# megaease/easevoice-trainer

Hardware: AMD Instinct MI355X
Metric: audio-seconds/sec trained (s2) (higher is better)
Workload: dtype bf16; 1 GPU; s2 SoVITS generator+discriminator GAN step, batch=16/GPU, 4 s 32 kHz clips (T=200 frames), configs/s2.json, random-init weights; global_batch=16, parallelism=dp1, launch=hip-graph replay (3 graphs/step)

## Files before the change

### easevoice_trainer_amd/csrc/conv1d.hip

```cpp
#include "evt_common.h"
#include "../../include/evt.h"
#include "conv_p.h"
#include "wgrad_epi.h"

extern "C" int evt_grouped_supported(const evt_conv1d_params* c);
extern "C" int evt_grouped_fwd(const evt_conv1d_params* c, const void* x, const void* w_reg, const float* bias, void* y,
                               void* stream);
extern "C" int evt_grouped_bwd_data(const evt_conv1d_params* c, const void* dy, const void* y, const void* w_reg,
                                    void* dx, void* stream);
extern "C" int evt_grouped_bwd_weight(const evt_conv1d_params* c, const void* x, const void* dy, const void* y,
                                      float* dw, void* stream);

extern "C" int evt_small_kind(const evt_conv1d_params* c);
extern "C" int evt_cout1_fwd(const evt_conv1d_params* c, const void* x, const void* w_reg, const float* bias, void* y,
                             void* stream);
extern "C" int evt_cout1_bwd_weight(const evt_conv1d_params* c, const void* x, const void* dy, const void* y, float* dw,
                                    float* dbias, float* ws, long ws_floats, void* stream);
extern "C" int evt_cin1_bwd_weight(const evt_conv1d_params* c, const void* x, const void* dy, const void* y, float* dw,
                                   float* dbias, float* ws, long ws_floats, void* stream);
extern "C" int evt_cin1_fwd(const evt_conv1d_params* c, const void* x, const void* w_reg, const float* bias, void* y,
                            void* stream);
extern "C" int evt_cin1_bwd_data(const evt_conv1d_params* c, const void* dy, const void* y, const void* w_reg,
                                 const void* gate, const void* dx_add, void* dx, void* stream);
extern "C" int evt_cout1_bwd_data(const evt_conv1d_params* c, const void* dy, const void* y, const void* w_reg,
                                  const void* gate, const void* dx_add, void* dx, void* stream);

namespace {

using evt_conv::ConvP;

template <typename T> struct Frag;
template <> struct Frag<float> {
  static constexpr int EPL = 1, KS = 4;
  typedef float type;
  static __device__ __forceinline__ f32x4 mma(float a, float b, f32x4 c) {
    return __builtin_amdgcn_mfma_f32_16x16x4f32(a, b, c, 0, 0, 0);
  }
};
template <> struct Frag<h16_t> {
  static constexpr int EPL = 8, KS = 32;
  typedef h16x8 type;
  static __device__ __forceinline__ f32x4 mma(h16x8 a, h16x8 b, f32x4 c) {
    return EVT_MFMA_16x16x32(a, b, c, 0, 0, 0);
  }
};

template <typename T, int MODE>
__device__ __forceinline__ uint4 fuse16(uint4 v, uint4 va, float act_slope, float in_slope, int act_kind) {
  if (MODE == 0) return v;
  constexpr int V = 16 / sizeof(T);
  T* h = reinterpret_cast<T*>(&v);
  const T* a = reinterpret_cast<const T*>(&va);
#pragma unroll
  for (int i = 0; i < V; ++i) {
    float t = to_f<T>(h[i]);
    if (MODE == 1) t = t > 0.f ? t : t * in_slope;
    else if (MODE == 2) t = to_f<T>(a[i]) > 0.f ? t : t * act_slope;
    else if (MODE == 3) { const float y = to_f<T>(a[i]); t *= 1.f - y * y; }
    else { t *= dact_from_out(act_kind, to_f<T>(a[i]), act_slope); t = t > 0.f ? t : t * in_slope; }
    h[i] = from_f<T>(t);
  }
  return v;
}

__device__ __forceinline__ int fuse_mode(bool has_act, int act_kind, float in_slope) {
  if (!has_act) return in_slope == 1.f ? 0 : 1;
  if (in_slope != 1.f) return 4;
  return act_kind == EVT_ACT_LRELU ? 2 : (act_kind == EVT_ACT_TANH ? 3 : 0);
}

template <typename T>
__device__ __forceinline__ uint4 fuse_load16(uint4 v, bool has_act, uint4 va, int act_kind, float act_slope,
                                             float in_slope) {
  switch (fuse_mode(has_act, act_kind, in_slope)) {
    case 0: return v;
    case 1: return fuse16<T, 1>(v, va, act_slope, in_slope, act_kind);
    case 2: return fuse16<T, 2>(v, va, act_slope, in_slope, act_kind);
    case 3: return fuse16<T, 3>(v, va, act_slope, in_slope, act_kind);
    default: return fuse16<T, 4>(v, va, act_slope, in_slope, act_kind);
  }
}

template <typename T, int CK, int WPT, int TPR>
__device__ __forceinline__ void igemm_load_w(uint4 (&wr)[WPT], const T* wg, const ConvP& p, int ch, int tg, int TG,
                                             int wrow, int wsub) {
  constexpr int SZ = sizeof(T);
  const int t0 = tg * TG;
  const int ppr = min(TG, p.KHp - t0) * CK * SZ / 16;
  const T* src = wg + ((long)(wrow * p.nchunk + ch) * p.KHp + t0) * CK;
#pragma unroll
  for (int i = 0; i < WPT; ++i) {
    const int piece = wsub + i * TPR;
    wr[i] = piece < ppr ? *reinterpret_cast<const uint4*>(src + piece * (16 / SZ)) : make_uint4(0, 0, 0, 0);
  }
}

template <typename T, int CK, int WPT, int TPR>
__device__ __forceinline__ void igemm_store_w(const uint4 (&wr)[WPT], unsigned char* ws, const ConvP& p, int tg, int TG,
                                              int WROW, int wrow, int wsub) {
  constexpr int SZ = sizeof(T);
  const int ppr = min(TG, p.KHp - tg * TG) * CK * SZ / 16;
#pragma unroll
  for (int i = 0; i < WPT; ++i) {
    const int piece = wsub + i * TPR;
    if (piece < ppr) *reinterpret_cast<uint4*>(ws + wrow * WROW + piece * 16) = wr[i];
  }
}

template <typename T, int CK, int XPT, int I0, int XPR>
__device__ __forceinline__ void igemm_load_x(uint4 (&xr)[XPT], uint4 (&ar)[XPT], const T* xg, const T* ag,
                                             const ConvP& p, int ch, int R, int row0, int lane) {
  constexpr int SZ = sizeof(T), LPR = CK * SZ / 16;
#pragma unroll
  for (int i = 0; i < XPR; ++i) {
    const int idx = lane + i * 64;
    const int r = idx / LPR, part = idx - r * LPR;
    const int in_row = row0 + r;
    const bool ok = idx < R * LPR && in_row >= 0 && in_row < p.Lin;
    const long off = ok ? (long)in_row * p.Cin + ch * CK + part * (16 / SZ) : 0;
    xr[I0 + i] = ok ? *reinterpret_cast<const uint4*>(xg + off) : make_uint4(0, 0, 0, 0);
    ar[I0 + i] = (ok && ag) ? *reinterpret_cast<const uint4*>(ag + off) : make_uint4(0, 0, 0, 0);
  }
}

template <typename T, int CK, int XPT, int I0, int XPR, int MODE>
__device__ __forceinline__ void igemm_store_x_m(const uint4 (&xr)[XPT], const uint4 (&ar)[XPT], unsigned char* xs,
                                                const ConvP& p, int R, int row0, int lane, int XROW) {
  constexpr int SZ = sizeof(T), LPR = CK * SZ / 16;
#pragma unroll
  for (int i = 0; i < XPR; ++i) {
    const int idx = lane + i * 64;
    const int r = idx / LPR, part = idx - r * LPR;
    const int in_row = row0 + r;
    if (idx < R * LPR) {
      const bool ok = in_row >= 0 && in_row < p.Lin;
      uint4 v = fuse16<T, MODE>(xr[I0 + i], ar[I0 + i], p.xact_slope, p.in_slope, p.xact_kind);
      if (!ok) v = make_uint4(0, 0, 0, 0);
      *reinterpret_cast<uint4*>(xs + r * XROW + part * 16) = v;
    }
  }
}

template <typename T, int CK, int XPT, int I0, int XPR>
__device__ __forceinline__ void igemm_store_x(const uint4 (&xr)[XPT], const uint4 (&ar)[XPT], unsigned char* xs,
                                              int mode, const ConvP& p, int R, int row0, int lane, int XROW) {
  switch (mode) {
    case 0: igemm_store_x_m<T, CK, XPT, I0, XPR, 0>(xr, ar, xs, p, R, row0, lane, XROW); break;
    case 1: igemm_store_x_m<T, CK, XPT, I0, XPR, 1>(xr, ar, xs, p, R, row0, lane, XROW); break;
    case 2: igemm_store_x_m<T, CK, XPT, I0, XPR, 2>(xr, ar, xs, p, R, row0, lane, XROW); break;
    case 3: igemm_store_x_m<T, CK, XPT, I0, XPR, 3>(xr, ar, xs, p, R, row0, lane, XROW); break;
    default: igemm_store_x_m<T, CK, XPT, I0, XPR, 4>(xr, ar, xs, p, R, row0, lane, XROW); break;
  }
}

template <typename T, int CK, int MODE>
__device__ __forceinline__ void igemm_stage_x_sync_m(unsigned char* xs, const T* xg, const T* ag, const ConvP& p, int ch,
                                                     int R, int row0, int lane, int XROW, int first_idx) {
  constexpr int SZ = sizeof(T), LPR = CK * SZ / 16;
  for (int idx = first_idx + lane; idx < R * LPR; idx += 64) {
    const int r = idx / LPR, part = idx - r * LPR;
    const int in_row = row0 + r;
    uint4 v = make_uint4(0, 0, 0, 0);
    if (in_row >= 0 && in_row < p.Lin) {
      const long off = (long)in_row * p.Cin + ch * CK + part * (16 / SZ);
      v = *reinterpret_cast<const uint4*>(xg + off);
      uint4 va = make_uint4(0, 0, 0, 0);
      if (MODE >= 2) va = *reinterpret_cast<const uint4*>(ag + off);
      v = fuse16<T, MODE>(v, va, p.xact_slope, p.in_slope, p.xact_kind);
    }
    *reinterpret_cast<uint4*>(xs + r * XROW + part * 16) = v;
  }
}

template <typename T, int CK>
__device__ __forceinline__ void igemm_stage_x_sync(unsigned char* xs, const T* xg, const T* ag, int mode, const ConvP& p,
                                                   int ch, int R, int row0, int lane, int XROW, int first_idx) {
  switch (mode) {
    case 0: igemm_stage_x_sync_m<T, CK, 0>(xs, xg, ag, p, ch, R, row0, lane, XROW, first_idx); break;
// ... 879 lines not shown
  if (c->cin % 16 || c->cout % 16) return false;
  if (c->stride > 1 && c->dil != 1) return false;
  return true;
}

int valid(const evt_conv1d_params* c) {
  if (!c || c->nseq <= 0 || c->lin <= 0 || c->cin <= 0 || c->cout <= 0 || c->k <= 0 || c->stride <= 0 ||
      c->dil <= 0 || c->groups <= 0 || c->pad < 0)
    return EVT_EINVAL;
  if (c->dtype != EVT_DT_F32 && c->dtype != EVT_DT_HALF) return EVT_EINVAL;
  if (c->cin % c->groups || c->cout % c->groups) return EVT_EINVAL;
  if (c->transposed && (c->groups != 1 || c->dil != 1)) return EVT_ENOTSUP;
  if (evt_conv1d_lout(c) <= 0) return EVT_EINVAL;
  return EVT_OK;
}

}

extern "C" {

int32_t evt_conv1d_lout(const evt_conv1d_params* c) {
  if (!c->transposed) return (c->lin + 2 * c->pad - c->dil * (c->k - 1) - 1) / c->stride + 1;
  return (c->lin - 1) * c->stride - 2 * c->pad + c->dil * (c->k - 1) + 1;
}

int32_t evt_conv1d_wants_plain_dy(const evt_conv1d_params* c) {
  if (!c || valid(c) != EVT_OK) return 0;
  if (c->impl != EVT_IMPL_AUTO || c->dtype != EVT_DT_HALF || c->transposed || !igemm_ok(c)) return 0;
  if (c->out_act == EVT_ACT_NONE || c->in_slope != 1.f) return 0;
  ConvP p{};
  p.in_slope = 1.f;
  p.nseq = c->nseq;
  p.nchunk = c->cout / 32;
  int nphase = 1;
  if (c->stride == 1) p.Q = c->lin;
  else { nphase = c->stride; p.Q = (c->lin - 1 + c->pad) / c->stride + 1; }
  if (evt_conv::deep_eligible(p, c->dtype, c->cin, c->cout, nphase)) return 1;
  {
    evt_wlayout l; evt_conv1d_layout(c, &l);
    ConvP q = p;
    q.s_in = q.s_out = 1; q.off_out = 0; q.KHp = l.alt_kp; q.nchunk = l.alt_nchunk;
    if (c->stride == 1 && evt_conv::narrow_eligible(q, c->dtype, c->cin, c->cout, 1)) return 1;
  }
  WgP w{};
  w.nseq = c->nseq; w.KH = w.KHp = c->k; w.Q = w.LA = evt_conv1d_lout(c); w.CA = c->cout; w.CB = c->cin;
  w.s = c->stride; w.dil = c->dil; w.LB = c->lin;
  w.a_slope = w.b_slope = 1.f;
  return (evt_conv::wgrad_deep_eligible(w, c->dtype) || evt_conv::wgrad_halo_eligible(w, c->dtype)) ? 1 : 0;
}

int32_t evt_conv1d_wants_plain_x(const evt_conv1d_params* c) {
  if (!c || valid(c) != EVT_OK) return 0;
  if (c->impl != EVT_IMPL_AUTO || c->dtype != EVT_DT_HALF || c->in_slope == 1.f || !igemm_ok(c)) return 0;
  if (evt_grouped_supported(c) || evt_small_kind(c) != 0) return 0;
  evt_wlayout l; evt_conv1d_layout(c, &l);
  const int lout = evt_conv1d_lout(c);
  ConvP p{};
  p.in_slope = 1.f;
  p.nseq = c->nseq;
  int nphase = 1;
  if (!c->transposed) { p.nchunk = l.reg_nchunk; p.KHp = l.reg_kp; p.Q = lout; }
  else {
    p.nchunk = l.alt_nchunk; p.KHp = l.alt_kp;
    if (c->stride == 1) p.Q = lout;
    else { nphase = c->stride; p.Q = (lout - 1 + c->pad) / c->stride + 1; }
  }
  return evt_conv::deep_eligible(p, c->dtype, c->cout, c->cin, nphase) ? 1 : 0;
}

int evt_conv1d_layout(const evt_conv1d_params* c, evt_wlayout* o) {
  if (!c || !o) return EVT_EINVAL;
  const int d0 = c->transposed ? c->cin : c->cout;
  const int d1 = c->transposed ? c->cout : c->cin / c->groups;
  o->d0 = d0; o->d1 = d1; o->k = c->k; o->stride = c->stride;
  pick_ck(c->dtype, d1, c->k, 1, &o->reg_ck, &o->reg_nchunk, &o->reg_kp);
  o->reg_elems = (int64_t)d0 * o->reg_nchunk * o->reg_kp * o->reg_ck;
  if (c->stride == 1) {
    pick_ck(c->dtype, d0, c->k, 1, &o->alt_ck, &o->alt_nchunk, &o->alt_kp);
    o->alt_nphase = 1;
  } else {
    const int J = (c->k + c->stride - 1) / c->stride;
    pick_ck(c->dtype, d0, J, 1, &o->alt_ck, &o->alt_nchunk, &o->alt_kp);
    o->alt_nphase = c->stride;
  }
  o->alt_elems = (int64_t)o->alt_nphase * d1 * o->alt_nchunk * o->alt_kp * o->alt_ck;
  return EVT_OK;
}

int evt_conv1d_fwd(const evt_conv1d_params* c, const void* x, const void* w_reg, const void* w_alt,
                   const float* bias, const void* res, void* y, void* stream) {
  int rc = valid(c);
  if (rc) return rc;
  if (!x || !y) return EVT_EINVAL;
  hipStream_t st = (hipStream_t)stream;
  const bool use_igemm = c->impl != EVT_IMPL_NAIVE && igemm_ok(c);
  if (c->impl == EVT_IMPL_IGEMM && !use_igemm) return EVT_ENOTSUP;
  const int lout = evt_conv1d_lout(c);
  evt_wlayout l; evt_conv1d_layout(c, &l);
  if (w_reg && evt_conv::rows16_eligible(c, c->nseq * c->lin, c->cout, c->cin,
                                         res || c->in_slope != 1.f || c->out_act != EVT_ACT_NONE))
    return evt_conv::launch_rows16(x, w_reg, bias, y, c->nseq * c->lin, c->cout, c->cin, st);
  evt_set_last_tag("conv_naive_fwd");
  if (c->impl != EVT_IMPL_NAIVE && !res && evt_grouped_supported(c)) {
    if (!w_reg) return EVT_EINVAL;
    evt_set_last_tag("grouped_fwd");
    return evt_grouped_fwd(c, x, w_reg, bias, y, stream);
  }
  if (c->impl != EVT_IMPL_NAIVE && !res && evt_small_kind(c) == 1) {
    if (!w_reg) return EVT_EINVAL;
    return evt_cout1_fwd(c, x, w_reg, bias, y, stream);
  }
  if (c->impl != EVT_IMPL_NAIVE && !res && evt_small_kind(c) == 2) {
    if (!w_reg) return EVT_EINVAL;
    return evt_cin1_fwd(c, x, w_reg, bias, y, stream);
  }
  if (!use_igemm) {
    if (!w_reg) return EVT_EINVAL;
    NvP p = make_nvp(c);
    p.x = x; p.w = w_reg; p.bias = bias; p.res = res; p.y = y;
    const long total = (long)c->nseq * lout * c->cout;
    const int blocks = (int)((total + 255) / 256 > 65535 * 8 ? 65535 * 8 : (total + 255) / 256);
    if (c->dtype == EVT_DT_HALF) hipLaunchKernelGGL(conv_naive_fwd<h16_t>, dim3(blocks), dim3(256), 0, st, p);
    else hipLaunchKernelGGL(conv_naive_fwd<float>, dim3(blocks), dim3(256), 0, st, p);
    return evt_check_launch();
  }
  const void* w = c->transposed ? w_alt : w_reg;
  if (!w) return EVT_EINVAL;
  ConvP p{};
  p.x = x; p.xact = nullptr; p.w = w; p.bias = bias; p.res = res; p.gate = nullptr; p.y = y;
  p.nseq = c->nseq; p.Lin = c->lin; p.Lout = lout; p.Cin = c->cin; p.Cout = c->cout;
  p.in_slope = c->in_slope; p.xact_kind = 0; p.xact_slope = 1.f; p.out_act = c->out_act; p.out_slope = c->out_slope;
  p.gate_slope = 1.f;
  int nphase = 1;
  if (!c->transposed) {
    p.KHp = l.reg_kp; p.nchunk = l.reg_nchunk;
    p.s_in = c->stride; p.dil = c->dil; p.off_in = -c->pad;
    p.s_out = 1; p.off_out = 0; p.off_out_phase = 0; p.Q = lout; p.w_phase_stride = 0;
  } else {
    p.KHp = l.alt_kp; p.nchunk = l.alt_nchunk; p.dil = 1; p.s_in = 1;
    if (c->stride == 1) {
      p.off_in = c->pad - (c->k - 1); p.s_out = 1; p.off_out = 0; p.off_out_phase = 0; p.Q = lout;
      p.w_phase_stride = 0;
    } else {
      const int J = (c->k + c->stride - 1) / c->stride;
      nphase = c->stride;
      p.off_in = -(J - 1); p.s_out = c->stride; p.off_out = -c->pad; p.off_out_phase = 1;
      p.Q = (lout - 1 + c->pad) / c->stride + 1;
      p.w_phase_stride = (long)c->cout * l.alt_nchunk * l.alt_kp * l.alt_ck;
    }
  }
  return launch_igemm(c->dtype, p, c->cout, c->cin, nphase, st, c->impl == EVT_IMPL_AUTO);
}

int evt_conv1d_bwd_data(const evt_conv1d_params* c, const void* dy, const void* y, const void* w_reg,
                        const void* w_alt, const void* x, const void* dx_add, void* dx, void* stream) {
  int rc = valid(c);
  if (rc) return rc;
  if (!dy || !dx) return EVT_EINVAL;
  if (c->out_act != EVT_ACT_NONE && !y) return EVT_EINVAL;
  if (c->in_slope != 1.f && !x) return EVT_EINVAL;
  hipStream_t st = (hipStream_t)stream;
  const bool use_igemm = c->impl != EVT_IMPL_NAIVE && igemm_ok(c);
  if (c->impl == EVT_IMPL_IGEMM && !use_igemm) return EVT_ENOTSUP;
  const int lout = evt_conv1d_lout(c);
  evt_wlayout l; evt_conv1d_layout(c, &l);
  const void* ysv = c->out_act != EVT_ACT_NONE ? y : nullptr;
  const void* gate = c->in_slope != 1.f ? x : nullptr;
  if (w_alt && evt_conv::rows16_eligible(c, c->nseq * c->lin, c->cin, c->cout, ysv || gate || dx_add))
    return evt_conv::launch_rows16(dy, w_alt, nullptr, dx, c->nseq * c->lin, c->cin, c->cout, st);
  evt_set_last_tag("conv_naive_bwd_data");
  if (c->impl != EVT_IMPL_NAIVE && !gate && !dx_add && evt_grouped_supported(c)) {
    if (!w_reg) return EVT_EINVAL;
    evt_set_last_tag("grouped_bwd_data");
    return evt_grouped_bwd_data(c, dy, y, w_reg, dx, stream);
  }
  if (c->impl != EVT_IMPL_NAIVE && evt_small_kind(c) != 0) {
    if (!w_reg) return EVT_EINVAL;
    rc = evt_small_kind(c) == 1 ? evt_cout1_bwd_data(c, dy, y, w_reg, gate, dx_add, dx, stream)
                                : evt_cin1_bwd_data(c, dy, y, w_reg, gate, dx_add, dx, stream);
    if (rc != EVT_ENOTSUP) return rc;
  }
  if (!use_igemm) {
    if (!w_reg) return EVT_EINVAL;
    NvP p = make_nvp(c);
    p.x = dy; p.y_in = ysv; p.w = w_reg; p.gate = gate; p.res = dx_add; p.y = dx;
    const long total = (long)c->nseq * c->lin * c->cin;
    const int blocks = (int)((total + 255) / 256 > 65535 * 8 ? 65535 * 8 : (total + 255) / 256);
    if (c->dtype == EVT_DT_HALF) hipLaunchKernelGGL(conv_naive_bwd_data<h16_t>, dim3(blocks), dim3(256), 0, st, p);
    else hipLaunchKernelGGL(conv_naive_bwd_data<float>, dim3(blocks), dim3(256), 0, st, p);
    return evt_check_launch();
  }
  const void* w = c->transposed ? w_reg : w_alt;
  if (!w) return EVT_EINVAL;
  ConvP p{};
  p.x = dy; p.xact = ysv; p.w = w; p.bias = nullptr; p.res = dx_add; p.gate = gate; p.y = dx;
  p.nseq = c->nseq; p.Lin = lout; p.Lout = c->lin; p.Cin = c->cout; p.Cout = c->cin;
  p.in_slope = 1.f; p.xact_kind = c->out_act; p.xact_slope = c->out_slope; p.out_act = EVT_ACT_NONE;
  p.out_slope = 1.f; p.gate_slope = c->in_slope;
  int nphase = 1;
  if (!c->transposed) {
    p.KHp = l.alt_kp; p.nchunk = l.alt_nchunk;
    if (c->stride == 1) {
      p.s_in = 1; p.dil = c->dil; p.off_in = c->pad - (c->k - 1) * c->dil;
      p.s_out = 1; p.off_out = 0; p.off_out_phase = 0; p.Q = c->lin; p.w_phase_stride = 0;
    } else {
      const int J = (c->k + c->stride - 1) / c->stride;
      nphase = c->stride;
      p.s_in = 1; p.dil = 1; p.off_in = -(J - 1);
      p.s_out = c->stride; p.off_out = -c->pad; p.off_out_phase = 1;
      p.Q = (c->lin - 1 + c->pad) / c->stride + 1;
      p.w_phase_stride = (long)c->cin * l.alt_nchunk * l.alt_kp * l.alt_ck;
    }
  } else {
    p.KHp = l.reg_kp; p.nchunk = l.reg_nchunk;
    p.s_in = c->stride; p.dil = 1; p.off_in = -c->pad;
    p.s_out = 1; p.off_out = 0; p.off_out_phase = 0; p.Q = c->lin; p.w_phase_stride = 0;
  }
  return launch_igemm(c->dtype, p, c->cin, c->cout, nphase, st, c->impl == EVT_IMPL_AUTO);
}

int evt_conv1d_bwd_weight(const evt_conv1d_params* c, const void* x, const void* dy, const void* y, float* dw,
                          float* dbias, void* stream) {
  return evt_conv1d_bwd_weight_parts(c, x, dy, y, dw, dbias, nullptr, stream);
}

int evt_conv1d_bwd_weight_parts(const evt_conv1d_params* c, const void* x, const void* dy, const void* y, float* dw,
                                float* dbias, evt_wgrad_parts* sp, void* stream) {
  int rc = valid(c);
  if (rc) return rc;
  if (!x || !dy || !dw) return EVT_EINVAL;
  int used_host = 0;
  if (sp) {
    sp->used = 0;
    if (sp->parts < 1 || !sp->used_dev || sp->prev_used < 0 || sp->prev_used > sp->parts) return EVT_EINVAL;
    if (sp->parts > 1 && (!sp->dw_extra || sp->part_stride <= 0)) return EVT_EINVAL;
    if (sp->ws && sp->ws_floats <= 0) return EVT_EINVAL;
  }
  if (c->out_act != EVT_ACT_NONE && !y) return EVT_EINVAL;
  hipStream_t st = (hipStream_t)stream;
  const int lout = evt_conv1d_lout(c);
  const void* ysv = c->out_act != EVT_ACT_NONE ? y : nullptr;
  evt_wlayout l; evt_conv1d_layout(c, &l);
  const bool grouped = c->impl != EVT_IMPL_NAIVE && evt_grouped_supported(c);
  const bool igemm_path = !grouped && c->impl != EVT_IMPL_NAIVE && igemm_ok(c) && l.reg_kp <= 64;
  WgP p{};
  p.dw = dw; p.nseq = c->nseq; p.KH = c->k; p.KHp = l.reg_kp; p.s = c->stride; p.dil = c->dil; p.off = -c->pad;
  if (!c->transposed) {
    p.A = dy; p.Aact = ysv; p.aact_kind = c->out_act; p.aact_slope = c->out_slope; p.a_slope = 1.f;
    p.B = x; p.Bact = nullptr; p.bact_kind = 0; p.bact_slope = 1.f; p.b_slope = c->in_slope;
    p.LA = lout; p.CA = c->cout; p.LB = c->lin; p.CB = c->cin; p.Q = lout;
  } else {
    p.A = x; p.Aact = nullptr; p.aact_kind = 0; p.aact_slope = 1.f; p.a_slope = c->in_slope;
    p.B = dy; p.Bact = ysv; p.bact_kind = c->out_act; p.bact_slope = c->out_slope; p.b_slope = 1.f;
    p.LA = c->lin; p.CA = c->cin; p.LB = lout; p.CB = c->cout; p.Q = c->lin;
  }
  p.dbias = nullptr;
  if (sp) {
    p.dw_extra = sp->dw_extra; p.part_stride = sp->part_stride; p.parts = sp->parts; p.prev_used = sp->prev_used;
    p.db_part = sp->db_part; p.used = sp->used_dev; p.used_host = &used_host; p.dirty0 = sp->dirty0 || sp->prev_used > 0;
  }
  const bool gemm_w = igemm_path && c->impl == EVT_IMPL_AUTO && !c->transposed && evt_conv::wgrad_gemm_eligible(p, c->dtype);
  const bool halo_w = !gemm_w && igemm_path && c->impl == EVT_IMPL_AUTO && evt_conv::wgrad_halo_eligible(p, c->dtype);
  const bool deep_w = !gemm_w && !halo_w && igemm_path && c->impl == EVT_IMPL_AUTO && evt_conv::wgrad_deep_eligible(p, c->dtype);
  const bool ring_w = !deep_w && !halo_w && igemm_path && c->impl == EVT_IMPL_AUTO && evt_conv::wgrad_ring_eligible(p, c->dtype);
  const bool cin1 = !grouped && c->impl != EVT_IMPL_NAIVE && evt_small_kind(c) == 2;
  const bool cout1 = !grouped && c->impl != EVT_IMPL_NAIVE && evt_small_kind(c) == 1;
  const bool fuse_bias = dbias && ((igemm_path && c->dtype == EVT_DT_HALF && !c->transposed) || cin1 || cout1);
  float* ws = sp ? sp->ws : nullptr;
  const long ws_floats = sp ? (long)sp->ws_floats : 0;
  if (dbias && !fuse_bias) {
    const long rows = (long)c->nseq * lout;
    const int V = c->dtype == EVT_DT_HALF ? 8 : 4;
    int blocks;
    float* wsb = nullptr;
    if (c->cout % V == 0 && c->cout / V <= 256) {
      long rpb = (rows + 255) / 256;
      if (rpb < 16) rpb = 16;
      blocks = (int)((rows + rpb - 1) / rpb);
      if (ws && blocks >= 2 && (long)blocks * c->cout <= ws_floats) wsb = ws;
      if (c->dtype == EVT_DT_HALF)
        hipLaunchKernelGGL(colsum_act2<h16_t>, dim3(blocks), dim3(256), 0, st, (const h16_t*)dy, (const h16_t*)ysv,
                           dbias, rows, c->cout, c->out_act, c->out_slope, (int)rpb, wsb);
      else
        hipLaunchKernelGGL(colsum_act2<float>, dim3(blocks), dim3(256), 0, st, (const float*)dy, (const float*)ysv,
                           dbias, rows, c->cout, c->out_act, c->out_slope, (int)rpb, wsb);
    } else {
      const int rpb = 64;
      blocks = (int)((rows + rpb - 1) / rpb);
      if (ws && blocks >= 2 && (long)blocks * c->cout <= ws_floats) wsb = ws;
      if (c->dtype == EVT_DT_HALF)
        hipLaunchKernelGGL(colsum_act<h16_t>, dim3(blocks), dim3(256), 0, st, (const h16_t*)dy, (const h16_t*)ysv,
                           dbias, rows, c->cout, c->out_act, c->out_slope, rpb, wsb);
      else
        hipLaunchKernelGGL(colsum_act<float>, dim3(blocks), dim3(256), 0, st, (const float*)dy, (const float*)ysv,
                           dbias, rows, c->cout, c->out_act, c->out_slope, rpb, wsb);
    }
    rc = evt_check_launch();
    if (rc) return rc;
    if (wsb) {
      rc = evt_conv::launch_fold_partials(wsb, c->cout, blocks, dbias, c->cout, st);
      if (rc) return rc;
    }
  }
  evt_set_last_tag("conv_naive_bwd_weight");
  if (grouped) {
    evt_set_last_tag("grouped_bwd_weight");
    return evt_grouped_bwd_weight(c, x, dy, y, dw, stream);
  }
  if (cout1) return evt_cout1_bwd_weight(c, x, dy, y, dw, dbias, ws, ws_floats, stream);
  if (cin1) return evt_cin1_bwd_weight(c, x, dy, y, dw, dbias, ws, ws_floats, stream);
  const bool use_igemm = igemm_path;
  if (c->impl == EVT_IMPL_IGEMM && !use_igemm) return EVT_ENOTSUP;
  if (!use_igemm) {
    NvP p = make_nvp(c);
    p.x = x; p.res = dy; p.y_in = ysv; p.dw = dw;
    const int d1n = c->transposed ? c->cout : c->cin / c->groups;
    const int d0n = c->transposed ? c->cin : c->cout;
    const long elems = (long)d0n * d1n * c->k;
    const long pos = (long)c->nseq * (c->transposed ? c->lin : lout);
    long split = (4096 + elems - 1) / elems;
    const long maxsplit = (pos + 2047) / 2048;
    if (split > maxsplit) split = maxsplit;
    if (split < 1) split = 1;
    p.nsplit = (int)split;
    if (c->dtype == EVT_DT_HALF)
      hipLaunchKernelGGL(conv_naive_bwd_weight<h16_t>, dim3((unsigned)elems, p.nsplit), dim3(256), 0, st, p);
    else
      hipLaunchKernelGGL(conv_naive_bwd_weight<float>, dim3((unsigned)elems, p.nsplit), dim3(256), 0, st, p);
    return evt_check_launch();
  }
  if (gemm_w) {
    p.dbias = fuse_bias ? dbias : nullptr;
    p.parts = 0;
    return evt_conv::launch_wgrad_gemm(p, st);
  }
  if (halo_w || deep_w || ring_w) {
    p.dbias = fuse_bias ? dbias : nullptr;
    if (!p.dbias) p.db_part = nullptr;
    rc = halo_w ? evt_conv::launch_wgrad_halo(p, st) : (deep_w ? evt_conv::launch_wgrad_deep(p, st) : evt_conv::launch_wgrad_ring(p, st));
    if (sp) sp->used = used_host;
    return rc;
  }
  if (c->dtype == EVT_DT_HALF) {
    p.dbias = fuse_bias ? dbias : nullptr;
    p.ws = ws; p.ws_floats = ws_floats;
    if (p.parts < 2) p.parts = 0;
    rc = launch_wgrad_tr(p, st);
    if (sp && rc != EVT_ENOTSUP) sp->used = used_host;
    if (rc != EVT_ENOTSUP) return rc;
    p.parts = 0;
    if (fuse_bias) {
      const long rows = (long)c->nseq * lout;
      hipLaunchKernelGGL(colsum_act<h16_t>, dim3((int)((rows + 63) / 64)), dim3(256), 0, st, (const h16_t*)dy,
                         (const h16_t*)ysv, dbias, rows, c->cout, c->out_act, c->out_slope, 64, (float*)nullptr);
      rc = evt_check_launch();
      if (rc) return rc;
    }
  }
  p.dbias = nullptr;
  return launch_wgrad(c->dtype, p, st);
}

}
```

### easevoice_trainer_amd/csrc/conv_deep.hip

```cpp
#include "conv_p.h"
#include "wgrad_epi.h"

namespace evt_conv {
namespace {

__device__ __attribute__((aligned(256))) unsigned int g_zero_page[64];

typedef __attribute__((address_space(1))) const void* gptr_t;
typedef __attribute__((address_space(3))) void* lptr_t;

__device__ __forceinline__ void glds16(const void* g, void* l) {
  __builtin_amdgcn_global_load_lds((gptr_t)g, (lptr_t)l, 16, 0, 0);
}

constexpr int BM = 128, BN = 128, BK = 64;

template <int TM, int TN, int MI, int NJ>
__device__ __forceinline__ void store_tile_staged(const ConvP& p, unsigned char* smem, const f32x4 (&acc)[MI][NJ], int wr,
                                                  int wc, int n, int g, int yi, int pb, int phase, int total_units) {
  constexpr int PITCH = TM * 2 + 16;
  constexpr int CPR = TM / 8;
  constexpr int RPP = 256 / CPR;
  f32x4 bv[MI];
#pragma unroll
  for (int i = 0; i < MI; ++i)
    bv[i] = p.bias ? *reinterpret_cast<const f32x4*>(p.bias + yi * TM + wr * 16 * MI + i * 16 + g * 4) : f32x4{0.f, 0.f, 0.f, 0.f};
  asm volatile("s_waitcnt lgkmcnt(0)" ::: "memory");
  __builtin_amdgcn_s_barrier();
  asm volatile("" ::: "memory");
#pragma unroll
  for (int j = 0; j < NJ; ++j) {
    const int pl = wc * 16 * NJ + j * 16 + n;
#pragma unroll
    for (int i = 0; i < MI; ++i) {
      const int cl = wr * 16 * MI + i * 16 + g * 4;
      h16_t outv[4];
#pragma unroll
      for (int r = 0; r < 4; ++r) {
        float v = acc[i][j][r] + bv[i][r];
        if (p.out_act == EVT_ACT_LRELU) v = lrelu_f(v, p.out_slope);
        else if (p.out_act == EVT_ACT_TANH) v = tanhf(v);
        outv[r] = f2h(v);
      }
      *reinterpret_cast<uint2*>(smem + pl * PITCH + cl * 2) = *reinterpret_cast<uint2*>(outv);
    }
  }
  __syncthreads();
  h16_t* Y = reinterpret_cast<h16_t*>(p.y);
  const h16_t* R = reinterpret_cast<const h16_t*>(p.res);
  const h16_t* G = reinterpret_cast<const h16_t*>(p.gate);
  const int tid = threadIdx.x;
  const int c16 = tid % CPR, r0 = tid / CPR;
#pragma unroll
  for (int pass = 0; pass * RPP < TN; ++pass) {
    const int pl = pass * RPP + r0;
    const int u = pb * TN + pl;
    if (pl >= TN || u >= total_units) continue;
    const int seq = u / p.Q;
    const int q = u - seq * p.Q;
    const int orow = q * p.s_out + p.off_out + phase * p.off_out_phase;
    if (orow < 0 || orow >= p.Lout) continue;
    const long off = ((long)seq * p.Lout + orow) * p.Cout + yi * TM + c16 * 8;
    uint4 v = *reinterpret_cast<const uint4*>(smem + pl * PITCH + c16 * 16);
    if (G || R) {
      uint4 gv = make_uint4(0, 0, 0, 0), rv = make_uint4(0, 0, 0, 0);
      if (G) gv = *reinterpret_cast<const uint4*>(G + off);
      if (R) rv = *reinterpret_cast<const uint4*>(R + off);
      h16_t* vp = reinterpret_cast<h16_t*>(&v);
      const h16_t* gp = reinterpret_cast<const h16_t*>(&gv);
      const h16_t* rp = reinterpret_cast<const h16_t*>(&rv);
#pragma unroll
      for (int e = 0; e < 8; ++e) {
        float f = h2f(vp[e]);
        if (G) f *= (h2f(gp[e]) > 0.f ? 1.f : p.gate_slope);
        if (R) f += h2f(rp[e]);
        vp[e] = f2h(f);
      }
    }
    *reinterpret_cast<uint4*>(Y + off) = v;
  }
}


constexpr int STAGE_BYTES = (BM + BN) * BK * 2;

__global__ __launch_bounds__(256, 2) void conv_deep(ConvP p) {
  extern __shared__ __attribute__((aligned(1024))) unsigned char smem[];
  const int tid = threadIdx.x, lane = tid & 63;
  const int wave = __builtin_amdgcn_readfirstlane(tid >> 6);
  const int n = lane & 15, g = lane >> 4;
  const int wr = wave >> 1, wc = wave & 1;

  const int lin = blockIdx.x;
  const int xcd = lin & 7, slot = lin >> 3;
  const int yi = slot % p.Y;
  const int pb = xcd + 8 * (slot / p.Y);
  if (pb >= p.P) return;
  const int phase = blockIdx.y;

  const h16_t* X = reinterpret_cast<const h16_t*>(p.x);
  const h16_t* W = reinterpret_cast<const h16_t*>(p.w) + (long)phase * p.w_phase_stride;
  const int total_units = p.nseq * p.Q;

  const int rsub = lane >> 3, pslot = lane & 7;
  long aoff[4], boff[4];
  int brow[4];
#pragma unroll
  for (int i = 0; i < 4; ++i) {
    const int row = wave * 32 + i * 8 + rsub;
    const int c = pslot ^ (row & 7);
    const int co = yi * BM + row;
    aoff[i] = ((long)co * p.nchunk + (c >> 2)) * p.KHp * 32 + (c & 3) * 8;
    const int u = pb * BN + row;
    const bool ok = u < total_units;
    const int seq = ok ? u / p.Q : 0;
    const int q = ok ? u - seq * p.Q : 0;
    brow[i] = ok ? q * p.s_in + p.off_in : -(1 << 28);
    boff[i] = ((long)seq * p.Lin + brow[i]) * p.Cin + c * 8;
  }
  const h16_t* zsrc = reinterpret_cast<const h16_t*>(g_zero_page) + pslot * 8;
  unsigned char* my_a = smem + wave * 32 * 128;
  unsigned char* my_b = smem + BM * 128 + wave * 32 * 128;

  const int nch2 = p.nchunk >> 1;
  const int nst = nch2 * p.KHp;

  auto issue = [&](int st, int buf) {
    const int ch2 = st / p.KHp, tap = st - ch2 * p.KHp;
    const long wsoff = ((long)(2 * ch2) * p.KHp + tap) * 32;
    const int rshift = tap * p.dil;
    const long xsoff = (long)rshift * p.Cin + ch2 * 64;
#pragma unroll
    for (int i = 0; i < 4; ++i) glds16(W + aoff[i] + wsoff, my_a + buf * STAGE_BYTES + i * 1024);
#pragma unroll
    for (int i = 0; i < 4; ++i) {
      const bool ok = (unsigned)(brow[i] + rshift) < (unsigned)p.Lin;
      const h16_t* src = ok ? X + boff[i] + xsoff : zsrc;
      glds16(src, my_b + buf * STAGE_BYTES + i * 1024);
    }
  };

  f32x4 acc[4][4];
#pragma unroll
  for (int i = 0; i < 4; ++i)
#pragma unroll
    for (int j = 0; j < 4; ++j) acc[i][j] = f32x4{0.f, 0.f, 0.f, 0.f};

  const int sw = n & 7;
  const int a_base = (wr * 64 + n) * 128;
  const int b_base = BM * 128 + (wc * 64 + n) * 128;
  const int so0 = ((0 + g) ^ sw) * 16, so1 = ((4 + g) ^ sw) * 16;

  issue(0, 0);
  for (int st = 0; st < nst; ++st) {
    const int buf = st & 1;
    __syncthreads();
    if (st + 1 < nst) issue(st + 1, buf ^ 1);
    const unsigned char* sa = smem + buf * STAGE_BYTES + a_base;
    const unsigned char* sb = smem + buf * STAGE_BYTES + b_base;
#pragma unroll
    for (int ks = 0; ks < 2; ++ks) {
      const int so = ks ? so1 : so0;
      h16x8 a[4], b[4];
#pragma unroll
      for (int i = 0; i < 4; ++i) a[i] = *reinterpret_cast<const h16x8*>(sa + i * 16 * 128 + so);
#pragma unroll
      for (int j = 0; j < 4; ++j) b[j] = *reinterpret_cast<const h16x8*>(sb + j * 16 * 128 + so);
#pragma unroll
      for (int i = 0; i < 4; ++i)
#pragma unroll
        for (int j = 0; j < 4; ++j) acc[i][j] = EVT_MFMA_16x16x32(a[i], b[j], acc[i][j], 0, 0, 0);
    }
  }

  store_tile_staged<BM, BN, 4, 4>(p, smem, acc, wr, wc, n, g, yi, pb, phase, total_units);
}

constexpr int STAGE32 = (BM + BN) * 64;

__global__ __launch_bounds__(256, 4) void conv_deep32(ConvP p) {
  extern __shared__ __attribute__((aligned(1024))) unsigned char smem[];
  const int tid = threadIdx.x, lane = tid & 63;
  const int wave = __builtin_amdgcn_readfirstlane(tid >> 6);
  const int n = lane & 15, g = lane >> 4;
  const int wr = wave >> 1, wc = wave & 1;
  const int lin = blockIdx.x;
  const int xcd = lin & 7, slot = lin >> 3;
  const int yi = slot % p.Y;
  const int pb = xcd + 8 * (slot / p.Y);
  if (pb >= p.P) return;
  const int phase = blockIdx.y;
  const h16_t* X = reinterpret_cast<const h16_t*>(p.x);
  const h16_t* W = reinterpret_cast<const h16_t*>(p.w) + (long)phase * p.w_phase_stride;
  const int total_units = p.nseq * p.Q;

  const int rsub = lane >> 2, pslot = lane & 3;
  long aoff[2], boff[2];
  int brow[2];
#pragma unroll
  for (int i = 0; i < 2; ++i) {
    const int row = wave * 32 + i * 16 + rsub;
    const int c = pslot ^ (2 * ((row >> 3) & 1));
    aoff[i] = (long)(yi * BM + row) * p.nchunk * p.KHp * 32 + c * 8;
    const int u = pb * BN + row;
    const bool ok = u < total_units;
    const int seq = ok ? u / p.Q : 0;
    const int q = ok ? u - seq * p.Q : 0;
    brow[i] = ok ? q * p.s_in + p.off_in : -(1 << 28);
    boff[i] = ((long)seq * p.Lin + brow[i]) * p.Cin + c * 8;
  }
  const h16_t* zsrc = reinterpret_cast<const h16_t*>(g_zero_page) + pslot * 8;
  unsigned char* my_a = smem + wave * 32 * 64;
  unsigned char* my_b = smem + BM * 64 + wave * 32 * 64;
  const int nst = p.nchunk * p.KHp;

  auto issue = [&](int st, int buf) {
    const int ch = st / p.KHp, tap = st - ch * p.KHp;
    const long wsoff = ((long)ch * p.KHp + tap) * 32;
    const int rshift = tap * p.dil;
    const long xsoff = (long)rshift * p.Cin + ch * 32;
#pragma unroll
    for (int i = 0; i < 2; ++i) glds16(W + aoff[i] + wsoff, my_a + buf * STAGE32 + i * 1024);
#pragma unroll
    for (int i = 0; i < 2; ++i) {
      const bool ok = (unsigned)(brow[i] + rshift) < (unsigned)p.Lin;
      glds16(ok ? X + boff[i] + xsoff : zsrc, my_b + buf * STAGE32 + i * 1024);
    }
  };

// ... 1173 lines not shown
```

### easevoice_trainer_amd/csrc/conv_p.h

```cpp
#pragma once
#include "evt_common.h"
#include "../../include/evt.h"
#include <cstdlib>

namespace evt_conv {

struct ConvP {
  const void* x;
  const void* xact;
  const void* w;
  const float* bias;
  const void* res;
  const void* gate;
  void* y;
  int nseq, Lin, Lout, Cin, Cout;
  int KHp;
  int s_in, dil, off_in;
  int s_out, off_out, off_out_phase;
  int Q, U;
  int nchunk;
  long w_phase_stride;
  float in_slope;
  int xact_kind;
  float xact_slope;
  int out_act;
  float out_slope;
  float gate_slope;
  int P, Y;
};

struct WgP {
  const void* A;
  const void* Aact;
  const void* B;
  const void* Bact;
  float* dw;
  int nseq, LA, LB, CA, CB;
  int KH, KHp, s, dil, off, Q;
  int nchunk;
  float a_slope, b_slope;
  int aact_kind, bact_kind;
  float aact_slope, bact_slope;
  int nsplit;
  int ntapgrp;
  int xcd_order;
  float* dbias;
  float* dw_extra;
  long part_stride;
  int parts;
  int prev_used;
  int now_used;
  int dirty0;
  float* db_part;
  int* used;
  int* used_host;
  float* ws;
  long ws_floats;
};

bool deep_eligible(const ConvP& p, int dtype, int out_ch, int k_ch, int nphase);
int launch_conv_deep(const ConvP& p, int out_ch, int k_ch, int nphase, hipStream_t st);
bool narrow_eligible(const ConvP& p, int dtype, int out_ch, int k_ch, int nphase);
int launch_conv_narrow(const ConvP& p, int out_ch, int k_ch, int nphase, hipStream_t st);
bool wgrad_deep_eligible(const WgP& p, int dtype);
int launch_wgrad_deep(const WgP& p, hipStream_t st);
bool wgrad_gemm_eligible(const WgP& p, int dtype);
int launch_wgrad_gemm(const WgP& p, hipStream_t st);
bool wgrad_ring_eligible(const WgP& p, int dtype);
int launch_wgrad_ring(const WgP& p, hipStream_t st);
bool wgrad_halo_eligible(const WgP& p, int dtype);
int launch_wgrad_halo(const WgP& p, hipStream_t st);
int launch_fold_partials(const float* part, long stride, int nb, float* out, long n, hipStream_t st);
int launch_fold_partials2(const float* part, long stride, int nb, float* out, long n, float* out2, long n2, hipStream_t st);
void wgrad_pick_split(const WgP& p, long tiles, int nstages, long target, int min_stages, int* nsplit, int* per);

bool rows16_eligible(const struct evt_conv1d_params* c, int rows, int n_out, int k_red, bool fused);
int launch_rows16(const void* x, const void* w, const float* bias, void* y, int M, int N, int K, hipStream_t st);

}
```

### easevoice_trainer_amd/csrc/conv_small.hip

```cpp
#include "evt_common.h"
#include "../../include/evt.h"
#include "conv_p.h"

namespace {

struct SP {
  const void* x; const void* w; const float* bias; const void* y_in; const void* dy; void* y; float* dw;
  int nseq, lin, lout, cin, cout, k, stride, pad, dil;
  int ck, nchunk, kp;
  float in_slope; int out_act; float out_slope;
  int G;
  int pos_per_block;
  float* ws;
  long ws_row;
  float* dbias;
  int tile;
  int step_q, step_r;
};

__device__ __forceinline__ long sreg_index(const SP& p, int d0, int d1, int t) {
  const int chunk = d1 / p.ck, cc = d1 - chunk * p.ck;
  return (((long)d0 * p.nchunk + chunk) * p.kp + t) * p.ck + cc;
}

struct Walk { int seq, i; };
__device__ __forceinline__ Walk walk_at(long r, int len) {
  Walk w;
  w.seq = (int)(r / len);
  w.i = (int)(r - (long)w.seq * len);
  return w;
}
__device__ __forceinline__ void walk_add(Walk& w, int dq, int dr, int len) {
  w.seq += dq; w.i += dr;
  if (w.i >= len) { w.i -= len; ++w.seq; }
}

template <typename T> struct Raw8 { uint4 q[sizeof(T) / 2]; };
template <typename T> __device__ __forceinline__ Raw8<T> ld8(const T* s) {
  Raw8<T> r;
#pragma unroll
  for (int i = 0; i < (int)sizeof(T) / 2; ++i) r.q[i] = reinterpret_cast<const uint4*>(s)[i];
  return r;
}
template <typename T> __device__ __forceinline__ void cvt8(const Raw8<T>& r, float* f) {
  const T* pv = reinterpret_cast<const T*>(&r);
#pragma unroll
  for (int e = 0; e < 8; ++e) f[e] = to_f<T>(pv[e]);
}

template <typename T>
__global__ __launch_bounds__(256) void cout1_fwd(SP p) {
  constexpr int V = 16 / sizeof(T);
  extern __shared__ __attribute__((aligned(16))) unsigned char smem[];
  float* wl = reinterpret_cast<float*>(smem);
  const T* w = reinterpret_cast<const T*>(p.w);
  for (int i = threadIdx.x; i < p.k * p.cin; i += 256) {
    const int t = i / p.cin, c = i - t * p.cin;
    wl[i] = to_f<T>(w[sreg_index(p, 0, c, t)]);
  }
  __syncthreads();
  const int G = p.G;
  const int sub = threadIdx.x % G;
  const long gid = ((long)blockIdx.x * 256 + threadIdx.x) / G;
  const long ngroups = (long)gridDim.x * 256 / G;
  const long total = (long)p.nseq * p.lout;
  const int ppr = p.cin / V;
  const int pieces = p.k * ppr;
  const T* x = reinterpret_cast<const T*>(p.x);
  const long rounds = (total + ngroups - 1) / ngroups;
  for (long rd = 0; rd < rounds; ++rd) {
    const long o = rd * ngroups + gid;
    const bool live = o < total;
    const int q = live ? (int)(o % p.lout) : 0;
    const int seq = live ? (int)(o / p.lout) : 0;
    float acc = 0.f;
    if (live) {
      for (int pc = sub; pc < pieces; pc += G) {
        const int t = pc / ppr, c0 = (pc - t * ppr) * V;
        const int row = q * p.stride + t * p.dil - p.pad;
        if (row < 0 || row >= p.lin) continue;
        const uint4 v = *reinterpret_cast<const uint4*>(x + ((long)seq * p.lin + row) * p.cin + c0);
        const T* pv = reinterpret_cast<const T*>(&v);
        const float* wr = wl + t * p.cin + c0;
#pragma unroll
        for (int e = 0; e < V; ++e) acc += lrelu_f(to_f<T>(pv[e]), p.in_slope) * wr[e];
      }
    }
    for (int off = G >> 1; off > 0; off >>= 1) acc += __shfl_xor(acc, off, 64);
    if (live && sub == 0) {
      if (p.bias) acc += p.bias[0];
      if (p.out_act == EVT_ACT_LRELU) acc = lrelu_f(acc, p.out_slope);
      else if (p.out_act == EVT_ACT_TANH) acc = tanhf(acc);
      reinterpret_cast<T*>(p.y)[o] = from_f<T>(acc);
    }
  }
}

template <typename T>
__device__ __forceinline__ float cout1_dy_sum(const SP& p, long o0, long o1) {
  __shared__ float redb[4];
  const T* dy = reinterpret_cast<const T*>(p.dy);
  const T* ys = reinterpret_cast<const T*>(p.y_in);
  float s = 0.f;
  for (long o = o0 + threadIdx.x; o < o1; o += 256) {
    float d = to_f<T>(dy[o]);
    if (ys) d *= dact_from_out(p.out_act, to_f<T>(ys[o]), p.out_slope);
    s += d;
  }
  return block_reduce_sum_256(s, redb);
}

__device__ __forceinline__ void cout1_store_partial(const SP& p, const float* red, int npl, float bsum) {
  const int kc = p.k * p.cin;
  const int img = p.nchunk * p.kp * p.ck;
  for (int i = threadIdx.x; i < img; i += 256) {
    const int run = i / p.ck, cc = i - run * p.ck;
    const int chunk = run / p.kp, t = run - chunk * p.kp;
    const int c = chunk * p.ck + cc;
    const bool real = t < p.k && c < p.cin;
    float v = 0.f;
    if (real) {
      v = red[t * p.cin + c];
      for (int l = 1; l < npl; ++l) v += red[l * kc + t * p.cin + c];
    }
    if (p.ws) p.ws[(long)blockIdx.x * p.ws_row + i] = v;
    else if (real) atomicAdd(p.dw + i, v);
  }
  if (threadIdx.x == 0 && p.dbias) {
    if (p.ws) p.ws[(long)blockIdx.x * p.ws_row + img] = bsum;
    else atomicAdd(p.dbias, bsum);
  }
}

template <typename T>
__global__ __launch_bounds__(256) void cout1_bwd_weight(SP p) {
  constexpr int V = 16 / sizeof(T);
  extern __shared__ __attribute__((aligned(16))) unsigned char smem[];
  float* red = reinterpret_cast<float*>(smem);
  const int ppr = p.cin / V;
  const int pieces = p.k * ppr;
  int pp = 1;
  while (pp < pieces && pp < 256) pp <<= 1;
  const int npl = 256 / pp;
  const int pl = threadIdx.x / pp, pc0 = threadIdx.x % pp;
  constexpr int NA = 4;
  float acc[NA][V];
#pragma unroll
  for (int a = 0; a < NA; ++a)
#pragma unroll
    for (int e = 0; e < V; ++e) acc[a][e] = 0.f;
  const T* x = reinterpret_cast<const T*>(p.x);
  const T* dy = reinterpret_cast<const T*>(p.dy);
  const T* ys = reinterpret_cast<const T*>(p.y_in);
  const long total = (long)p.nseq * p.lout;
  const long p0 = (long)blockIdx.x * p.pos_per_block;
  const long p1 = min(total, p0 + p.pos_per_block);
  constexpr int UP = 4;
  for (long ob = p0 + pl; ob < p1; ob += (long)npl * UP) {
    uint4 v[UP][NA];
    float d[UP];
#pragma unroll
    for (int u = 0; u < UP; ++u) {
      const long o = ob + (long)u * npl;
      const bool live = o < p1;
      const int q = live ? (int)(o % p.lout) : 0, seq = live ? (int)(o / p.lout) : 0;
      d[u] = live ? to_f<T>(dy[o]) : 0.f;
      if (live && ys) d[u] *= dact_from_out(p.out_act, to_f<T>(ys[o]), p.out_slope);
#pragma unroll
      for (int a = 0; a < NA; ++a) {
        const int pc = pc0 + a * pp;
// ... 162 lines not shown
        }
      }
    }
  }
  __syncthreads();
  T* dx = reinterpret_cast<T*>(p.y) + (long)seq * p.lin;
  const T* gt = gate ? reinterpret_cast<const T*>(gate) + (long)seq * p.lin : nullptr;
  const T* ad = dx_add ? reinterpret_cast<const T*>(dx_add) + (long)seq * p.lin : nullptr;
  for (int ii = threadIdx.x; ii < ni; ii += 256) {
    const int i = i0 + ii;
    float acc = 0.f;
    for (int t = 0; t < p.k; ++t) {
      const int j = i + p.pad - t * p.dil;
      if (j < 0) break;
      const int q = j / p.stride;
      if (q * p.stride != j || q > qhi || q < qlo) continue;
      const float* pr = pl + (long)(q - qlo) * CG * p.k + t;
      float s = pr[0];
      for (int g = 1; g < CG; ++g) s += pr[g * p.k];
      acc += s;
    }
    if (gt) acc *= (to_f<T>(gt[i]) > 0.f ? 1.f : p.in_slope);
    if (ad) acc += to_f<T>(ad[i]);
    dx[i] = from_f<T>(acc);
  }
}

constexpr int C1_TQ = 256;

template <typename T, int KM>
__global__ __launch_bounds__(256) void cin1_bwd_weight(SP p, float* dbias) {
  extern __shared__ __attribute__((aligned(16))) unsigned char smem[];
  float* xl = reinterpret_cast<float*>(smem);
  __shared__ float red[4][4][(KM + 1) * 8];
  const int CG = p.cout >> 3, ppp = 256 / CG;
  const int cg = threadIdx.x & (CG - 1), c0 = cg * 8, ql = threadIdx.x / CG;
  const int lane = threadIdx.x & 63, wave = threadIdx.x >> 6;
  const int tiles = (p.lout + C1_TQ - 1) / C1_TQ;
  const long ntiles = (long)p.nseq * tiles;
  constexpr int UP = KM <= 8 ? 4 : 2;
  for (int t0 = 0; t0 < p.k; t0 += KM) {
    float acc[KM][8], bacc[8];
#pragma unroll
    for (int e = 0; e < 8; ++e) {
      bacc[e] = 0.f;
#pragma unroll
      for (int t = 0; t < KM; ++t) acc[t][e] = 0.f;
    }
    Walk wk = walk_at(blockIdx.x, tiles);
    for (long tile = blockIdx.x; tile < ntiles; tile += gridDim.x) {
      const int q0 = wk.i * C1_TQ;
      const int nq = min(C1_TQ, p.lout - q0);
      const int seg = (nq - 1) * p.stride + (p.k - 1) * p.dil + 1;
      const int r0 = q0 * p.stride - p.pad;
      const T* x = reinterpret_cast<const T*>(p.x) + (long)wk.seq * p.lin;
      const T* dy = reinterpret_cast<const T*>(p.dy) + ((long)wk.seq * p.lout + q0) * p.cout + c0;
      const T* ys = p.y_in ? reinterpret_cast<const T*>(p.y_in) + ((long)wk.seq * p.lout + q0) * p.cout + c0 : nullptr;
      __syncthreads();
      for (int i = threadIdx.x; i < seg; i += 256) {
        const int r = r0 + i;
        xl[i] = (r >= 0 && r < p.lin) ? lrelu_f(to_f<T>(x[r]), p.in_slope) : 0.f;
      }
      __syncthreads();
      for (int qb = ql; qb < nq; qb += ppp * UP) {
        Raw8<T> v[UP], va[UP];
#pragma unroll
        for (int u = 0; u < UP; ++u) {
          const int q = qb + u * ppp;
          if (q < nq) {
            v[u] = ld8<T>(dy + (long)q * p.cout);
            if (ys) va[u] = ld8<T>(ys + (long)q * p.cout);
          }
        }
#pragma unroll
        for (int u = 0; u < UP; ++u) {
          const int q = qb + u * ppp;
          if (q < nq) {
            float d[8], a[8];
            cvt8<T>(v[u], d);
            if (ys) {
              cvt8<T>(va[u], a);
#pragma unroll
              for (int e = 0; e < 8; ++e) d[e] *= dact_from_out(p.out_act, a[e], p.out_slope);
            }
            if (t0 == 0) {
#pragma unroll
              for (int e = 0; e < 8; ++e) bacc[e] += d[e];
            }
            const float* xr = xl + q * p.stride + t0 * p.dil;
#pragma unroll
            for (int t = 0; t < KM; ++t) {
              if (t0 + t < p.k) {
                const float xv = xr[t * p.dil];
#pragma unroll
                for (int e = 0; e < 8; ++e) acc[t][e] += d[e] * xv;
              }
            }
          }
        }
      }
      walk_add(wk, p.step_q, p.step_r, tiles);
    }
    for (int off = CG; off < 64; off <<= 1) {
#pragma unroll
      for (int e = 0; e < 8; ++e) {
        bacc[e] += __shfl_xor(bacc[e], off, 64);
#pragma unroll
        for (int t = 0; t < KM; ++t) acc[t][e] += __shfl_xor(acc[t][e], off, 64);
      }
    }
    __syncthreads();
    if (lane < CG) {
#pragma unroll
      for (int e = 0; e < 8; ++e) {
        red[wave][cg][KM * 8 + e] = bacc[e];
#pragma unroll
        for (int t = 0; t < KM; ++t) red[wave][cg][t * 8 + e] = acc[t][e];
      }
    }
    __syncthreads();
    for (int i = threadIdx.x; i < (KM + 1) * p.cout; i += 256) {
      const int t = i / p.cout, co = i - t * p.cout;
      const int g = co >> 3, e = co & 7;
      const float v = ((red[0][g][t * 8 + e] + red[1][g][t * 8 + e]) + red[2][g][t * 8 + e]) + red[3][g][t * 8 + e];
      if (t < KM) {
        if (t0 + t < p.k) {
          const long idx = (long)co * p.kp + t0 + t;
          if (p.ws) p.ws[(long)blockIdx.x * p.ws_row + idx] = v;
          else atomicAdd(p.dw + idx, v);
        }
      } else if (t0 == 0) {
        if (p.ws) p.ws[(long)blockIdx.x * p.ws_row + (p.ws_row - p.cout) + co] = v;
        else if (dbias) atomicAdd(dbias + co, v);
      }
    }
  }
}

template <typename T>
__global__ __launch_bounds__(256) void cout1_bwd_data(SP p, const void* gate, const void* dx_add) {
  constexpr int V = 16 / sizeof(T);
  extern __shared__ __attribute__((aligned(16))) unsigned char smem[];
  float* wl = reinterpret_cast<float*>(smem);
  const T* w = reinterpret_cast<const T*>(p.w);
  for (int i = threadIdx.x; i < p.k * p.cin; i += 256) {
    const int t = i / p.cin, c = i - t * p.cin;
    wl[i] = to_f<T>(w[sreg_index(p, 0, c, t)]);
  }
  __syncthreads();
  const int ppr = p.cin / V;
  const long total = (long)p.nseq * p.lin * ppr;
  const T* dy = reinterpret_cast<const T*>(p.dy);
  const T* ys = reinterpret_cast<const T*>(p.y_in);
  for (long idx = (long)blockIdx.x * 256 + threadIdx.x; idx < total; idx += (long)gridDim.x * 256) {
    const long row = idx / ppr;
    const int c0 = (int)(idx - row * ppr) * V;
    const int seq = (int)(row / p.lin), i = (int)(row - (long)seq * p.lin);
    float acc[V];
#pragma unroll
    for (int e = 0; e < V; ++e) acc[e] = 0.f;
    for (int t = 0; t < p.k; ++t) {
      const int j = i + p.pad - t * p.dil;
      if (j < 0) break;
      const int q = j / p.stride;
      if (q * p.stride != j || q >= p.lout) continue;
      const long o = (long)seq * p.lout + q;
      float d = to_f<T>(dy[o]);
      if (ys) d *= dact_from_out(p.out_act, to_f<T>(ys[o]), p.out_slope);
      const float* wr = wl + t * p.cin + c0;
#pragma unroll
      for (int e = 0; e < V; ++e) acc[e] += d * wr[e];
    }
    const long off = row * p.cin + c0;
    T outv[V];
    uint4 gv = make_uint4(0, 0, 0, 0), av = make_uint4(0, 0, 0, 0);
    if (gate) gv = *reinterpret_cast<const uint4*>(reinterpret_cast<const T*>(gate) + off);
    if (dx_add) av = *reinterpret_cast<const uint4*>(reinterpret_cast<const T*>(dx_add) + off);
    const T* pg = reinterpret_cast<const T*>(&gv);
    const T* pa = reinterpret_cast<const T*>(&av);
#pragma unroll
    for (int e = 0; e < V; ++e) {
      float v = acc[e];
      if (gate) v *= (to_f<T>(pg[e]) > 0.f ? 1.f : p.in_slope);
      if (dx_add) v += to_f<T>(pa[e]);
      outv[e] = from_f<T>(v);
    }
    *reinterpret_cast<uint4*>(reinterpret_cast<T*>(p.y) + off) = *reinterpret_cast<uint4*>(outv);
  }
}

SP make_sp(const evt_conv1d_params* c) {
  SP p{};
  p.nseq = c->nseq; p.lin = c->lin; p.lout = evt_conv1d_lout(c); p.cin = c->cin; p.cout = c->cout; p.k = c->k;
  p.stride = c->stride; p.pad = c->pad; p.dil = c->dil; p.in_slope = c->in_slope; p.out_act = c->out_act;
  p.out_slope = c->out_slope;
  evt_wlayout l; evt_conv1d_layout(c, &l);
  p.ck = l.reg_ck; p.nchunk = l.reg_nchunk; p.kp = l.reg_kp;
  return p;
}

inline void set_step(SP& p, long step, int len) {
  p.step_q = (int)(step / len);
  p.step_r = (int)(step - (long)p.step_q * len);
}

constexpr int CI1_WG_BLOCKS = 512;

template <typename T, int K>
__global__ __launch_bounds__(256) void cout1_bwd_weight_xs(SP p, int rows_per_block) {
  constexpr int V = 16 / sizeof(T);
  extern __shared__ __attribute__((aligned(16))) unsigned char smem[];
  float* red = reinterpret_cast<float*>(smem);
  const int ppr = p.cin / V;
  int pp = 1;
  while (pp < ppr) pp <<= 1;
  const int npl = 256 / pp;
  const int rl = threadIdx.x / pp, pc = threadIdx.x % pp;
  float acc[K][V];
#pragma unroll
  for (int t = 0; t < K; ++t)
#pragma unroll
    for (int e = 0; e < V; ++e) acc[t][e] = 0.f;
  const T* x = reinterpret_cast<const T*>(p.x);
  const T* dy = reinterpret_cast<const T*>(p.dy);
  const T* ys = reinterpret_cast<const T*>(p.y_in);
  const long total = (long)p.nseq * p.lin;
  const long r0 = (long)blockIdx.x * rows_per_block;
  const long r1 = min(total, r0 + rows_per_block);
  constexpr int UP = 4;
  if (pc < ppr) {
    for (long rb = r0 + rl; rb < r1; rb += (long)npl * UP) {
      uint4 v[UP];
      float d[UP][K];
#pragma unroll
      for (int u = 0; u < UP; ++u) {
        const long r = rb + (long)u * npl;
        const bool live = r < r1;
        const long seq = live ? r / p.lin : 0;
        const int i = live ? (int)(r - seq * p.lin) : 0;
        v[u] = live ? *reinterpret_cast<const uint4*>(x + r * p.cin + pc * V) : make_uint4(0, 0, 0, 0);
#pragma unroll
        for (int t = 0; t < K; ++t) {
          const int q = i + p.pad - t;
          const bool ok = live && q >= 0 && q < p.lout;
          const long o = seq * p.lout + (ok ? q : 0);
          float dv = ok ? to_f<T>(dy[o]) : 0.f;
          if (ok && ys) dv *= dact_from_out(p.out_act, to_f<T>(ys[o]), p.out_slope);
          d[u][t] = dv;
        }
      }
#pragma unroll
      for (int u = 0; u < UP; ++u) {
        const T* pv = reinterpret_cast<const T*>(&v[u]);
#pragma unroll
        for (int e = 0; e < V; ++e) {
          const float xv = lrelu_f(to_f<T>(pv[e]), p.in_slope);
#pragma unroll
          for (int t = 0; t < K; ++t) acc[t][e] += d[u][t] * xv;
        }
      }
    }
  }
  const int kc = K * p.cin;
  if (pc < ppr) {
#pragma unroll
    for (int t = 0; t < K; ++t)
#pragma unroll
      for (int e = 0; e < V; ++e) red[rl * kc + t * p.cin + pc * V + e] = acc[t][e];
  }
  const long nout = (long)p.nseq * p.lout;
  const long o0 = min(nout, (long)blockIdx.x * p.pos_per_block);
  const float bsum = p.dbias ? cout1_dy_sum<T>(p, o0, min(nout, o0 + p.pos_per_block)) : 0.f;
  __syncthreads();
  cout1_store_partial(p, red, npl, bsum);
}

}

extern "C" int evt_small_kind(const evt_conv1d_params* c) {
  if (c->transposed || c->groups != 1) return 0;
  const int V = c->dtype == EVT_DT_HALF ? 8 : 4;
  if (c->cout == 1 && c->cin % V == 0 && (long)c->k * c->cin <= 4096) return 1;
  if (c->cin == 1 && c->cout % 8 == 0 && c->cout <= 32 && 256 % c->cout == 0 && c->cout * (c->k + 1) <= 256)
    return 2;
  return 0;
}

extern "C" int evt_cout1_fwd(const evt_conv1d_params* c, const void* x, const void* w_reg, const float* bias, void* y,
                             void* stream) {
  SP p = make_sp(c);
  p.x = x; p.w = w_reg; p.bias = bias; p.y = y;
  const int V = c->dtype == EVT_DT_HALF ? 8 : 4;
  const int pieces = c->k * (c->cin / V);
  int G = 1;
  while (G < pieces && G < 64) G <<= 1;
  p.G = G;
  const long total = (long)p.nseq * p.lout;
  long blocks = (total * G + 255) / 256;
  constexpr long cap = 4096;
  if (blocks > cap) blocks = cap;
  const size_t lds = (size_t)c->k * c->cin * sizeof(float);
  hipStream_t st = (hipStream_t)stream;
  evt_set_last_tag("cout1_fwd");
  if (c->dtype == EVT_DT_HALF) hipLaunchKernelGGL(cout1_fwd<h16_t>, dim3((int)blocks), dim3(256), lds, st, p);
  else hipLaunchKernelGGL(cout1_fwd<float>, dim3((int)blocks), dim3(256), lds, st, p);
  return evt_check_launch();
}

extern "C" int evt_cout1_bwd_weight(const evt_conv1d_params* c, const void* x, const void* dy, const void* y, float* dw,
                                    float* dbias, float* ws, long ws_floats, void* stream) {
  SP p = make_sp(c);
  p.x = x; p.dy = dy; p.y_in = c->out_act != EVT_ACT_NONE ? y : nullptr; p.dw = dw; p.dbias = dbias;
  const long total = (long)p.nseq * p.lout;
  long ppb = (total + 255) / 256;
  if (ppb < 16) ppb = 16;
  const long img = (long)p.nchunk * p.kp * p.ck;
  const long row = img + 1;
  if (ws && row * 2 <= ws_floats) {
    constexpr long tgt = 1024, minp = 16;
    ppb = (total + tgt - 1) / tgt;
    if (ppb < minp) ppb = minp;
    const long maxb = ws_floats / row;
    if ((total + ppb - 1) / ppb > maxb) ppb = (total + maxb - 1) / maxb;
    p.ws = ws; p.ws_row = row;
  }
  p.pos_per_block = (int)ppb;
  int blocks = (int)((total + ppb - 1) / ppb);
  const int V = c->dtype == EVT_DT_HALF ? 8 : 4;
  hipStream_t st = (hipStream_t)stream;
  int ppr2 = 1;
  while (ppr2 < c->cin / V) ppr2 <<= 1;
  const size_t lds_xs = (size_t)(256 / ppr2) * c->k * c->cin * sizeof(float);
  if (p.stride == 1 && p.dil == 1 && (c->k == 3 || c->k == 7) && ppr2 <= 256 && lds_xs <= (60u << 10)) {
    const long rows = (long)p.nseq * p.lin;
    long rpb = (rows + blocks - 1) / blocks;
    if (rpb < 16) rpb = 16;
    blocks = (int)((rows + rpb - 1) / rpb);
    p.pos_per_block = (int)((total + blocks - 1) / blocks);
    evt_set_last_tag("cout1_bwd_weight_xs<k%d>", c->k);
#define XS(T, K_) hipLaunchKernelGGL((cout1_bwd_weight_xs<T, K_>), dim3(blocks), dim3(256), lds_xs, st, p, (int)rpb)
    if (c->dtype == EVT_DT_HALF) { if (c->k == 3) XS(h16_t, 3); else XS(h16_t, 7); }
    else { if (c->k == 3) XS(float, 3); else XS(float, 7); }
#undef XS
  } else {
    int pp = 1;
    while (pp < c->k * (c->cin / V) && pp < 256) pp <<= 1;
    const size_t lds = (size_t)(256 / pp) * c->k * c->cin * sizeof(float);
    evt_set_last_tag("cout1_bwd_weight");
    if (c->dtype == EVT_DT_HALF) hipLaunchKernelGGL(cout1_bwd_weight<h16_t>, dim3(blocks), dim3(256), lds, st, p);
    else hipLaunchKernelGGL(cout1_bwd_weight<float>, dim3(blocks), dim3(256), lds, st, p);
  }
  int rc = evt_check_launch();
  if (rc || !p.ws) return rc;
  return evt_conv::launch_fold_partials2(p.ws, row, blocks, dw, img, dbias, dbias ? 1 : 0, st);
}

extern "C" int evt_cin1_bwd_weight(const evt_conv1d_params* c, const void* x, const void* dy, const void* y, float* dw,
                                   float* dbias, float* ws, long ws_floats, void* stream) {
  if (c->cout != 8 && c->cout != 16 && c->cout != 32) return EVT_ENOTSUP;
  SP p = make_sp(c);
  p.x = x; p.dy = dy; p.y_in = c->out_act != EVT_ACT_NONE ? y : nullptr; p.dw = dw;
  const int tiles = (p.lout + C1_TQ - 1) / C1_TQ;
  const long ntiles = (long)p.nseq * tiles;
  const long img = (long)p.cout * p.nchunk * p.kp * p.ck;
  const long row = img + p.cout;
  int blocks = (int)(ntiles < 256 ? ntiles : 256);
  if (ws && ntiles >= 2 && row * 2 <= ws_floats) {
    const long maxb = ws_floats / row < CI1_WG_BLOCKS ? ws_floats / row : CI1_WG_BLOCKS;
    blocks = (int)(ntiles < maxb ? ntiles : maxb);
    p.ws = ws; p.ws_row = row;
  }
  set_step(p, blocks, tiles);
  const int seg = (C1_TQ - 1) * c->stride + (c->k - 1) * c->dil + 1;
  const size_t lds = (size_t)seg * sizeof(float);
  hipStream_t st = (hipStream_t)stream;
  evt_set_last_tag("cin1_bwd_weight");
#define WG(T) do { if (c->k <= 8) hipLaunchKernelGGL((cin1_bwd_weight<T, 8>), dim3(blocks), dim3(256), lds, st, p, dbias); \
                   else hipLaunchKernelGGL((cin1_bwd_weight<T, 16>), dim3(blocks), dim3(256), lds, st, p, dbias); } while (0)
  if (c->dtype == EVT_DT_HALF) WG(h16_t); else WG(float);
#undef WG
  int rc = evt_check_launch();
  if (rc || !p.ws) return rc;
  return evt_conv::launch_fold_partials2(p.ws, row, blocks, dw, img, dbias, dbias ? p.cout : 0, st);
}

extern "C" int evt_cin1_fwd(const evt_conv1d_params* c, const void* x, const void* w_reg, const float* bias, void* y,
                            void* stream) {
  SP p = make_sp(c);
  p.x = x; p.w = w_reg; p.bias = bias; p.y = y;
  const int blocks = p.nseq * ((p.lout + C1_TP - 1) / C1_TP);
  const int seg = (C1_TP - 1) * c->stride + (c->k - 1) * c->dil + 1;
  const size_t lds = ((size_t)c->k * c->cout + seg) * sizeof(float);
  hipStream_t st = (hipStream_t)stream;
  evt_set_last_tag("cin1_fwd");
  if (c->dtype == EVT_DT_HALF) hipLaunchKernelGGL(cin1_fwd<h16_t>, dim3(blocks), dim3(256), lds, st, p);
  else hipLaunchKernelGGL(cin1_fwd<float>, dim3(blocks), dim3(256), lds, st, p);
  return evt_check_launch();
}

extern "C" int evt_cin1_bwd_data(const evt_conv1d_params* c, const void* dy, const void* y, const void* w_reg,
                                 const void* gate, const void* dx_add, void* dx, void* stream) {
  if (c->cout != 8 && c->cout != 16 && c->cout != 32) return EVT_ENOTSUP;
  SP p = make_sp(c);
  p.dy = dy; p.y_in = c->out_act != EVT_ACT_NONE ? y : nullptr; p.w = w_reg; p.y = dx;
  const int CG = c->cout >> 3;
  int TI = C1_TI;
  size_t lds;
  for (;; TI >>= 1) {
    const int rows = (TI + (c->k - 1) * c->dil) / c->stride + 2;
    lds = ((size_t)c->k * c->cout + (size_t)rows * CG * c->k) * sizeof(float);
    if (lds <= 48 * 1024 || TI <= 32) break;
  }
  if (lds > 64 * 1024) return EVT_ENOTSUP;
  p.tile = TI;
  const int blocks = p.nseq * ((p.lin + TI - 1) / TI);
  hipStream_t st = (hipStream_t)stream;
  evt_set_last_tag("cin1_bwd_data");
#define BWD(T) do { if (c->k <= 8) hipLaunchKernelGGL((cin1_bwd_data<T, 8>), dim3(blocks), dim3(256), lds, st, p, gate, dx_add); \
                    else hipLaunchKernelGGL((cin1_bwd_data<T, 16>), dim3(blocks), dim3(256), lds, st, p, gate, dx_add); } while (0)
  if (c->dtype == EVT_DT_HALF) BWD(h16_t); else BWD(float);
#undef BWD
  return evt_check_launch();
}

extern "C" int evt_cout1_bwd_data(const evt_conv1d_params* c, const void* dy, const void* y, const void* w_reg,
                                  const void* gate, const void* dx_add, void* dx, void* stream) {
  SP p = make_sp(c);
  p.dy = dy; p.y_in = c->out_act != EVT_ACT_NONE ? y : nullptr; p.w = w_reg; p.y = dx;
  const int V = c->dtype == EVT_DT_HALF ? 8 : 4;
  const long total = (long)p.nseq * p.lin * (p.cin / V);
  long blocks = (total + 255) / 256;
  if (blocks > 2048) blocks = 2048;
  const size_t lds = (size_t)c->k * c->cin * sizeof(float);
  hipStream_t st = (hipStream_t)stream;
  evt_set_last_tag("cout1_bwd_data");
  if (c->dtype == EVT_DT_HALF) hipLaunchKernelGGL(cout1_bwd_data<h16_t>, dim3((int)blocks), dim3(256), lds, st, p, gate, dx_add);
  else hipLaunchKernelGGL(cout1_bwd_data<float>, dim3((int)blocks), dim3(256), lds, st, p, gate, dx_add);
  return evt_check_launch();
}
```

### easevoice_trainer_amd/csrc/elementwise.hip

```cpp
#include "evt_common.h"
#include "../../include/evt.h"

namespace {

__device__ __forceinline__ void store_w(void* base, long idx, float w, int dtype) {
  if (dtype == EVT_DT_HALF) reinterpret_cast<h16_t*>(base)[idx] = f2h(w);
  else reinterpret_cast<float*>(base)[idx] = w;
}

__device__ __forceinline__ long reg_idx(const evt_wlayout& L, int d0, int d1, int kk) {
  const int chunk = d1 / L.reg_ck, cc = d1 - chunk * L.reg_ck;
  return (((long)d0 * L.reg_nchunk + chunk) * L.reg_kp + kk) * L.reg_ck + cc;
}

__device__ __forceinline__ long alt_idx(const evt_wlayout& L, int d0, int d1, int kk) {
  const int chunk = d0 / L.alt_ck, cc = d0 - chunk * L.alt_ck;
  if (L.stride == 1) {
    const int t = L.k - 1 - kk;
    return (((long)d1 * L.alt_nchunk + chunk) * L.alt_kp + t) * L.alt_ck + cc;
  }
  const int J = (L.k + L.stride - 1) / L.stride;
  const int ph = kk % L.stride, j = kk / L.stride;
  const int jp = J - 1 - j;
  return ((((long)ph * L.d1 + d1) * L.alt_nchunk + chunk) * L.alt_kp + jp) * L.alt_ck + cc;
// ... 184 lines not shown
      const int row_floats = L.reg_nchunk * L.reg_kp * L.reg_ck;
      const long ro = (long)d0 * row_floats;
      fold_slabs_row(const_cast<float*>(it.dw) + ro, it.dw_extra + ro, it.dw_part_stride, nu, row_floats);
    }
    if (nb > 0 && it.db_part && it.db && threadIdx.x == 0) {
      float s = 0.f;
      for (int k = 0; k < nb; ++k) s += it.db_part[(long)k * L.d0 + d0];
      it.db[d0] += s;
    }
  }
  if (!it.g) {
    for (int e = threadIdx.x; e < n; e += 256) {
      const int d1 = e / L.k, kk = e - d1 * L.k;
      dv[e] += it.dw[reg_idx(L, d0, d1, kk)];
    }
    return;
  }
  float ss = 0.f, dot = 0.f;
  for (int e = threadIdx.x; e < n; e += 256) {
    const int d1 = e / L.k, kk = e - d1 * L.k;
    const float x = v[e];
    ss += x * x;
    dot += x * it.dw[reg_idx(L, d0, d1, kk)];
  }
  ss = block_reduce_sum_256(ss, red);
  dot = block_reduce_sum_256(dot, red);
  const float norm = sqrtf(ss);
  const float gval = it.g[d0];
  if (threadIdx.x == 0) it.dg[d0] += dot / norm;
  const float s1 = gval / norm, s2 = dot / ss;
  for (int e = threadIdx.x; e < n; e += 256) {
    const int d1 = e / L.k, kk = e - d1 * L.k;
    dv[e] += s1 * (it.dw[reg_idx(L, d0, d1, kk)] - v[e] * s2);
  }
}

template <typename T>
__global__ void add3_scale_kernel(const T* a, const T* b, const T* c, float scale, T* out, long n) {
  for (long i = blockIdx.x * (long)blockDim.x + threadIdx.x; i < n; i += (long)gridDim.x * blockDim.x) {
    float v = to_f<T>(a[i]);
    if (b) v += to_f<T>(b[i]);
    if (c) v += to_f<T>(c[i]);
    out[i] = from_f<T>(v * scale);
  }
}

template <typename T>
__global__ void dact_mul_kernel(const T* dy, const T* y, int kind, float slope, T* out, long n) {
  constexpr int V = 16 / sizeof(T);
  const long nv = n / V;
  for (long i = blockIdx.x * (long)blockDim.x + threadIdx.x; i < nv; i += (long)gridDim.x * blockDim.x) {
    uint4 d = reinterpret_cast<const uint4*>(dy)[i];
    const uint4 a = reinterpret_cast<const uint4*>(y)[i];
    T* dh = reinterpret_cast<T*>(&d);
    const T* ah = reinterpret_cast<const T*>(&a);
#pragma unroll
    for (int e = 0; e < V; ++e) dh[e] = from_f<T>(to_f<T>(dh[e]) * dact_from_out(kind, to_f<T>(ah[e]), slope));
    reinterpret_cast<uint4*>(out)[i] = d;
  }
  if (blockIdx.x == 0 && threadIdx.x < n - nv * V) {
    const long i = nv * V + threadIdx.x;
    out[i] = from_f<T>(to_f<T>(dy[i]) * dact_from_out(kind, to_f<T>(y[i]), slope));
  }
}

template <typename T>
__global__ void lrelu_kernel(const T* x, float slope, T* out, long n) {
  constexpr int V = 16 / sizeof(T);
  const long nv = n / V;
  for (long i = blockIdx.x * (long)blockDim.x + threadIdx.x; i < nv; i += (long)gridDim.x * blockDim.x) {
    uint4 v = reinterpret_cast<const uint4*>(x)[i];
    T* h = reinterpret_cast<T*>(&v);
#pragma unroll
    for (int e = 0; e < V; ++e) h[e] = from_f<T>(lrelu_f(to_f<T>(h[e]), slope));
    reinterpret_cast<uint4*>(out)[i] = v;
  }
  if (blockIdx.x == 0 && threadIdx.x < n - nv * V) {
    const long i = nv * V + threadIdx.x;
    out[i] = from_f<T>(lrelu_f(to_f<T>(x[i]), slope));
  }
}

__device__ __forceinline__ float sigmoid_f(float x) { return 1.f / (1.f + __expf(-x)); }

template <typename T>
__global__ void gated_fwd_kernel(const T* xin, const T* g, T* acts, int nseq, int len, int H) {
  const long total = (long)nseq * len * H;
  for (long i = blockIdx.x * (long)blockDim.x + threadIdx.x; i < total; i += (long)gridDim.x * blockDim.x) {
    const int h = (int)(i % H);
    const long nt = i / H;
    const int s = (int)(nt / len);
    float a = to_f<T>(xin[nt * 2 * H + h]), b = to_f<T>(xin[nt * 2 * H + H + h]);
    if (g) { a += to_f<T>(g[(long)s * 2 * H + h]); b += to_f<T>(g[(long)s * 2 * H + H + h]); }
    acts[i] = from_f<T>(tanhf(a) * sigmoid_f(b));
  }
}

template <typename T>
__global__ void gated_bwd_kernel(const T* xin, const T* g, const T* dacts, T* dxin, float* dg, int nseq, int len,
                                 int H) {
  const long total = (long)nseq * len * H;
  for (long i = blockIdx.x * (long)blockDim.x + threadIdx.x; i < total; i += (long)gridDim.x * blockDim.x) {
    const int h = (int)(i % H);
    const long nt = i / H;
    const int s = (int)(nt / len);
    float a = to_f<T>(xin[nt * 2 * H + h]), b = to_f<T>(xin[nt * 2 * H + H + h]);
    if (g) { a += to_f<T>(g[(long)s * 2 * H + h]); b += to_f<T>(g[(long)s * 2 * H + H + h]); }
    const float t = tanhf(a), sg = sigmoid_f(b), d = to_f<T>(dacts[i]);
    const float da = d * sg * (1.f - t * t), db = d * t * sg * (1.f - sg);
    dxin[nt * 2 * H + h] = from_f<T>(da);
    dxin[nt * 2 * H + H + h] = from_f<T>(db);
    if (dg) { atomicAdd(dg + (long)s * 2 * H + h, da); atomicAdd(dg + (long)s * 2 * H + H + h, db); }
  }
}

template <typename T>
__global__ __launch_bounds__(256) void gated_bwd_dg_kernel(const T* xin, const T* g, const T* dacts, T* dxin, float* dg,
                                                           int nseq, int len, int H, int tch) {
  const int per_seq = (len + tch - 1) / tch;
  const int s = blockIdx.x / per_seq;
  const int t0 = (blockIdx.x - s * per_seq) * tch, t1 = min(len, t0 + tch);
  for (int h = threadIdx.x; h < H; h += 256) {
    const float ga = to_f<T>(g[(long)s * 2 * H + h]), gb = to_f<T>(g[(long)s * 2 * H + H + h]);
    float sa = 0.f, sb = 0.f;
    for (int t = t0; t < t1; ++t) {
      const long nt = (long)s * len + t;
      const float a = to_f<T>(xin[nt * 2 * H + h]) + ga, b = to_f<T>(xin[nt * 2 * H + H + h]) + gb;
      const float th = tanhf(a), sg = sigmoid_f(b), d = to_f<T>(dacts[nt * H + h]);
      const float da = d * sg * (1.f - th * th), db = d * th * sg * (1.f - sg);
      dxin[nt * 2 * H + h] = from_f<T>(da);
      dxin[nt * 2 * H + H + h] = from_f<T>(db);
      sa += da;
      sb += db;
    }
    atomicAdd(dg + (long)s * 2 * H + h, sa);
    atomicAdd(dg + (long)s * 2 * H + H + h, sb);
  }
}

constexpr int SEG_MAX = 64;

template <typename T, int MODE>
__device__ __forceinline__ float seg_term(float a, float b, float target) {
  if (MODE == 0) return fabsf(a - b);
  const float d = target - a;
  return d * d;
}
template <typename T, int MODE>
__device__ __forceinline__ float seg_grad(float a, float b, float target, float dl) {
  if (MODE == 0) { const float d = a - b; return d > 0.f ? dl : (d < 0.f ? -dl : 0.f); }
  return -2.f * (target - a) * dl;
}

template <typename T, int MODE, bool BWD>
__global__ __launch_bounds__(256) void seg_flat_kernel(const evt_seg* segs, int nseg, float target, float* out,
                                                       const float* dloss) {
  constexpr int V = 16 / sizeof(T);
  __shared__ float red[4];
  __shared__ long pre[SEG_MAX + 1];
  if (threadIdx.x == 0) {
    long acc = 0;
    for (int i = 0; i < nseg; ++i) { pre[i] = acc; acc += segs[i].n; }
    pre[nseg] = acc;
  }
  __syncthreads();
  const long total = pre[nseg];
  long chunk = (total + gridDim.x - 1) / gridDim.x;
  chunk = (chunk + 2047) / 2048 * 2048;
  const long lo = (long)blockIdx.x * chunk, hi = min(total, lo + chunk);
  float acc = 0.f;
  for (int si = 0; si < nseg; ++si) {
    const long s0 = pre[si], s1 = pre[si + 1];
    if (s1 <= lo || s0 >= hi) continue;
    const evt_seg s = segs[si];
    if (BWD && !s.da) continue;
    const T* a = reinterpret_cast<const T*>(s.a);
    const T* b = reinterpret_cast<const T*>(s.b);
    T* da = reinterpret_cast<T*>(s.da);
    const long i0 = max(lo, s0) - s0, i1 = min(hi, s1) - s0;
    const float dl = BWD ? dloss[0] * s.scale : 0.f;
    float part = 0.f;
    const long v0 = min(i1, (i0 + V - 1) / V * V), v1 = v0 + (i1 - v0) / V * V;
    const bool vec_ok = ((((uintptr_t)a) | (MODE == 0 ? (uintptr_t)b : 0) | (BWD ? (uintptr_t)da : 0)) & 15) == 0;
    if (vec_ok) {
      for (long i = i0 + threadIdx.x; i < v0; i += 256) {
        const float av = to_f<T>(a[i]), bv = MODE == 0 ? to_f<T>(b[i]) : 0.f;
        if (BWD) da[i] = from_f<T>(seg_grad<T, MODE>(av, bv, target, dl)); else part += seg_term<T, MODE>(av, bv, target);
      }
      for (long i = v0 + (long)threadIdx.x * V; i < v1; i += 256L * V) {
        const uint4 va = *reinterpret_cast<const uint4*>(a + i);
        uint4 vb = make_uint4(0, 0, 0, 0);
        if (MODE == 0) vb = *reinterpret_cast<const uint4*>(b + i);
        const T* pa = reinterpret_cast<const T*>(&va);
        const T* pb = reinterpret_cast<const T*>(&vb);
        uint4 vo;
        T* po = reinterpret_cast<T*>(&vo);
#pragma unroll
        for (int e = 0; e < V; ++e) {
          const float av = to_f<T>(pa[e]), bv = MODE == 0 ? to_f<T>(pb[e]) : 0.f;
          if (BWD) po[e] = from_f<T>(seg_grad<T, MODE>(av, bv, target, dl)); else part += seg_term<T, MODE>(av, bv, target);
        }
        if (BWD) *reinterpret_cast<uint4*>(da + i) = vo;
      }
      for (long i = v1 + threadIdx.x; i < i1; i += 256) {
        const float av = to_f<T>(a[i]), bv = MODE == 0 ? to_f<T>(b[i]) : 0.f;
        if (BWD) da[i] = from_f<T>(seg_grad<T, MODE>(av, bv, target, dl)); else part += seg_term<T, MODE>(av, bv, target);
      }
    } else {
      for (long i = i0 + threadIdx.x; i < i1; i += 256) {
        const float av = to_f<T>(a[i]), bv = MODE == 0 ? to_f<T>(b[i]) : 0.f;
        if (BWD) da[i] = from_f<T>(seg_grad<T, MODE>(av, bv, target, dl)); else part += seg_term<T, MODE>(av, bv, target);
      }
    }
    acc += part * s.scale;
  }
  if (!BWD) {
    acc = block_reduce_sum_256(acc, red);
    if (threadIdx.x == 0 && acc != 0.f) atomicAdd(out, acc);
  }
}

__global__ void adamw_flat_kernel(float* p, const float* g, float* m, float* v, const evt_adamw_seg* segs, int nseg,
                                  float b1, float b2, float eps, float bc1, float bc2_sqrt, float gscale,
                                  long lo, long hi) {
  for (long i = lo + blockIdx.x * (long)blockDim.x + threadIdx.x; i < hi; i += (long)gridDim.x * blockDim.x) {
    int si = -1;
    for (int s = 0; s < nseg; ++s)
      if (i >= segs[s].begin && i < segs[s].end) { si = s; break; }
    if (si < 0) continue;
    const float lr = segs[si].lr, wd = segs[si].weight_decay;
    const float gr = g[i] * gscale;
    float pv = p[i];
    pv *= 1.f - lr * wd;
    const float mv = b1 * m[i] + (1.f - b1) * gr;
    const float vv = b2 * v[i] + (1.f - b2) * gr * gr;
    m[i] = mv; v[i] = vv;
    const float denom = sqrtf(vv) / bc2_sqrt + eps;
    pv -= (lr / bc1) * (mv / denom);
    p[i] = pv;
  }
}

__global__ void counter_inc_kernel(int* c, const float* skip) {
  if (skip && *skip != 0.f) return;
  *c += 1;
}

__global__ void adamw_flat_dev_kernel(float* p, const float* g, float* m, float* v, const evt_adamw_seg* segs, int nseg,
                                      float b1, float b2, float eps, const int* stepp, float gscale, long lo, long hi,
                                      const float* skip) {
  if (skip && *skip != 0.f) return;
  const float stepf = (float)*stepp;
  const float bc1 = 1.f - powf(b1, stepf);
  const float bc2_sqrt = sqrtf(1.f - powf(b2, stepf));
  for (long i = lo + blockIdx.x * (long)blockDim.x + threadIdx.x; i < hi; i += (long)gridDim.x * blockDim.x) {
    int si = -1;
    for (int s = 0; s < nseg; ++s)
      if (i >= segs[s].begin && i < segs[s].end) { si = s; break; }
    if (si < 0) continue;
    const float lr = segs[si].lr, wd = segs[si].weight_decay;
    const float gr = g[i] * gscale;
    float pv = p[i];
    pv *= 1.f - lr * wd;
    const float mv = b1 * m[i] + (1.f - b1) * gr;
    const float vv = b2 * v[i] + (1.f - b2) * gr * gr;
    m[i] = mv; v[i] = vv;
    const float denom = sqrtf(vv) / bc2_sqrt + eps;
    pv -= (lr / bc1) * (mv / denom);
    p[i] = pv;
  }
}

__global__ __launch_bounds__(256) void unscale_check_kernel(float* g, long n, const float* scale, float* found) {
  const float inv = (float)(1.0 / (double)*scale);
  bool bad = false;
  const long n4 = n >> 2;
  float4* g4 = reinterpret_cast<float4*>(g);
  for (long i = blockIdx.x * 256L + threadIdx.x; i < n4; i += (long)gridDim.x * 256) {
    float4 v = g4[i];
    bad |= !(isfinite(v.x) && isfinite(v.y) && isfinite(v.z) && isfinite(v.w));
    v.x *= inv; v.y *= inv; v.z *= inv; v.w *= inv;
    g4[i] = v;
  }
  for (long i = (n4 << 2) + blockIdx.x * 256L + threadIdx.x; i < n; i += (long)gridDim.x * 256) {
    const float v = g[i];
    bad |= !isfinite(v);
    g[i] = v * inv;
  }
  if (bad) *found = 1.f;
}

struct ScalerFlags { float* f[4]; };
__global__ void scaler_update_kernel(float* scale, int* tracker, ScalerFlags fl, int nflags, float growth, float backoff,
                                     int interval) {
  bool found = false;
  for (int i = 0; i < nflags; ++i) {
    found |= *fl.f[i] != 0.f;
    *fl.f[i] = 0.f;
  }
  if (found) {
    *scale = *scale * backoff;
    *tracker = 0;
  } else {
    const int ok = *tracker + 1;
    if (ok == interval) {
      const float ns = *scale * growth;
      if (isfinite(ns)) *scale = ns;
      *tracker = 0;
    } else {
      *tracker = ok;
    }
  }
}

__global__ __launch_bounds__(256) void sumsq_kernel(const float* x, long n, float* out) {
  __shared__ float red[4];
  float acc = 0.f;
  for (long i = blockIdx.x * 256L + threadIdx.x; i < n; i += (long)gridDim.x * 256) acc += x[i] * x[i];
  acc = block_reduce_sum_256(acc, red);
  if (threadIdx.x == 0) atomicAdd(out, acc);
}

inline int grid_for(long n, int cap = 8192) {
  long b = (n + 255) / 256;
  if (b > cap) b = cap;
  if (b < 1) b = 1;
  return (int)b;
}

}

#include <stdarg.h>
#include <stdio.h>
static bool g_tags_on = false;
static thread_local char g_last_tag[128] = "";
extern "C" void evt_set_last_tag(const char* fmt, ...) {
  if (!g_tags_on) return;
  va_list ap;
  va_start(ap, fmt);
  vsnprintf(g_last_tag, sizeof(g_last_tag), fmt, ap);
  va_end(ap);
}

extern "C" {

const char* evt_last_kernel_tag(void) { return g_last_tag; }
void evt_debug_kernel_tags(int32_t enable) { g_tags_on = enable != 0; }

#ifndef EVT_SRC_HASH
#define EVT_SRC_HASH "unknown"
#endif
const char* evt_version(void) { return "evt-hip 0.3 (gfx950, half = " EVT_HALF_NAME ") src=" EVT_SRC_HASH; }
int32_t evt_half_dtype(void) { return EVT_DT_HALF; }

int evt_wn_fold_multi(const evt_wprep_item* items, const int32_t* row_index, int32_t nrows, void* stream) {
  if (!items || !row_index || nrows <= 0) return EVT_EINVAL;
  const int nblocks = ((nrows + 255) / 256) * 256;
  hipLaunchKernelGGL(wn_fold_kernel, dim3(nblocks), dim3(256), 0, (hipStream_t)stream, items, row_index, nrows);
  return evt_check_launch();
}

int evt_wn_fold_groups(const evt_wprep_item* items, const int32_t* group_index, int32_t ngroups, void* stream) {
  if (!items || !group_index || ngroups <= 0) return EVT_EINVAL;
  const int nblocks = ((ngroups + 31) / 32) * 32;
// ... 208 lines not shown
```

### easevoice_trainer_amd/hip/conv.py

```python
import ctypes as C
import os
import math

import torch
from torch import nn

from . import lib as L


class ConvSlot:

    __slots__ = ("module", "layout", "reg", "alt", "dw", "bank", "_pcache", "packed_member", "parts", "dw_extra",
                 "db_part", "used", "wg_used", "wg_dirty", "_wgp")

    def __init__(self, module, layout, bank):
        self.module, self.layout, self.bank = module, layout, bank
        self.reg = self.alt = self.dw = None
        self._pcache = {}
        self.packed_member = False
        self.parts, self.dw_extra, self.db_part, self.used, self.wg_used, self._wgp = 1, None, None, None, 0, None
        self.wg_dirty = False

    def params(self, nseq, lin, in_slope, out_act, out_slope):
        key = (nseq, lin, in_slope, out_act, out_slope, self.bank.impl)
# ... 355 lines not shown

class FrozenConv:
    weight_norm, kdims, transposed, groups, dil = False, 1, False, 1, 1

    def __init__(self, weight_fn, bias_fn, cin, cout, k=1, stride=1, padding=0):
        self.weight_fn, self.bias_fn = weight_fn, bias_fn
        self.cin, self.cout, self.k, self.stride, self.pad = cin, cout, k, stride, padding
        self._slot = None

    @property
    def v(self):
        w = self.weight_fn()
        return w if w.dim() == 3 else w.unsqueeze(-1)

    @property
    def bias(self):
        return self.bias_fn() if self.bias_fn is not None else None

    def lout(self, lin):
        return (lin + 2 * self.pad - (self.k - 1) - 1) // self.stride + 1


class FrozenBank:
    weight_grads = False

    def __init__(self, convs, device, impl=L.IMPL_AUTO):
        self.dt, self.dtype, self.device, self.impl = L.DT_F32, torch.float32, torch.device(device), impl
        self.slots, offs, reg_n, alt_n = [], [], 0, 0
        for m in convs:
            lay = conv_layout(self.dt, m.cin, m.cout, m.k, m.stride, m.pad, m.dil, m.groups, m.transposed)
            s = ConvSlot(m, lay, self)
            m._slot = s
            self.slots.append(s)
            offs.append((reg_n, alt_n))
            reg_n += (lay.reg_elems + 127) // 128 * 128
            alt_n += (lay.alt_elems + 127) // 128 * 128
        self.reg_arena = torch.zeros(max(reg_n, 1), dtype=torch.float32, device=device)
        self.alt_arena = torch.zeros(max(alt_n, 1), dtype=torch.float32, device=device)
        for s, (ro, ao) in zip(self.slots, offs):
            s.reg = self.reg_arena[ro: ro + s.layout.reg_elems]
            s.alt = self.alt_arena[ao: ao + s.layout.alt_elems]
        self._stamp = self._items = None

    def prepare(self):
        vs = [s.module.v for s in self.slots]
        stamp = tuple((v.data_ptr(), v._version) for v in vs)
        if stamp == self._stamp:
            return
        items, rows = [], []
        for i, (s, v) in enumerate(zip(self.slots, vs)):
            if v.dtype != torch.float32 or not v.is_contiguous() or v.device != self.device:
                raise L.EvtError("FrozenBank: contiguous fp32 weights on the bank's device expected")
            it = L.WPrepItem()
            it.v, it.g, it.reg, it.alt = v.data_ptr(), None, s.reg.data_ptr(), s.alt.data_ptr()
            it.dw = it.dv = it.dg = None
            it.lay, it.dtype = s.layout, self.dt
            items.append(it)
            rows.extend((i, r) for r in range(s.layout.d0))
        self._items = L.struct_to_device(items, self.device)
        self._rows = torch.tensor(rows, dtype=torch.int32, device=self.device).contiguous()
        L.check(L.lib().evt_wn_fold_multi(L.ptr(self._items), L.ptr(self._rows), len(rows), L.stream_ptr()),
                "evt_wn_fold_multi")
        self._stamp = stamp


PLAIN_X = os.environ.get("EVT_CONV_PLAIN_X", "1") != "0"
TRACE = None


TRACE_RANGES = False


def set_trace(rec, ranges=False):
    global TRACE, TRACE_RANGES
    TRACE = rec
    TRACE_RANGES = bool(ranges) and rec is not None
    L.lib().evt_debug_kernel_tags(1 if rec is not None else 0)


def _t0():
    if TRACE is None:
        return None
    rf = None
    if TRACE_RANGES:
        rf = torch.profiler.record_function(f"evt#{len(TRACE)}")
        rf.__enter__()
    e = torch.cuda.Event(enable_timing=True)
    e.record()
    return e, rf


def _t1(e0, kind, m, nseq, lin, extra_elems):
    e0, rf = e0
    e1 = torch.cuda.Event(enable_timing=True)
    e1.record()
    if rf is not None:
        rf.__exit__(None, None, None)
    lq = lin if m.transposed else m.lout(lin)
    macs = nseq * lq * m.cin * m.cout * m.k // m.groups
    sz = 2 if L.is_half(m._slot.bank.dtype) else 4
    act = nseq * (lin * m.cin + m.lout(lin) * m.cout) + extra_elems
    wbytes = m.v.numel() * (4 if kind == "bwd_weight" else sz)
    shape = (f"{'T' if m.transposed else ''}{m.cin}>{m.cout} k{m.k} s{m.stride} d{m.dil} g{m.groups} "
             f"n{nseq} L{lin}")
    TRACE.append((L.lib().evt_last_kernel_tag().decode(), kind, 2 * macs, act * sz + wbytes, e0, e1, shape, m))


def _t1_elt(e0, name, nbytes, owner):
    e0, rf = e0
    e1 = torch.cuda.Event(enable_timing=True)
    e1.record()
    if rf is not None:
        rf.__exit__(None, None, None)
    TRACE.append((name, "elt", 0, nbytes, e0, e1, name, owner))


def _fwd(slot, x, res, in_slope, out_act, out_slope, out=None):
    m = slot.module
    if x.dim() != 3 or x.size(2) != m.cin or x.dtype != slot.bank.dtype or not x.is_contiguous():
        raise L.EvtError(f"conv input must be contiguous [nseq, L, {m.cin}] {slot.bank.dtype}, got "
                         f"{tuple(x.shape)} {x.dtype} contiguous={x.is_contiguous()}")
    nseq, lin = x.size(0), x.size(1)
    y = out if out is not None else torch.empty((nseq, m.lout(lin), m.cout), dtype=x.dtype, device=x.device)
    if y.shape != (nseq, m.lout(lin), m.cout) or y.dtype != x.dtype or not y.is_contiguous():
        raise L.EvtError("conv output buffer must be contiguous [nseq, Lout, Cout] in the compute dtype")
    if res is not None and (res.shape != y.shape or not res.is_contiguous() or res.dtype != x.dtype):
        raise L.EvtError("residual must match the output")
    p = slot.params(nseq, lin, in_slope, out_act, out_slope)
    bias = m.bias
    e0 = _t0()
    L.check(L.lib().evt_conv1d_fwd(C.byref(p), L.ptr(x), L.ptr(slot.reg), L.ptr(slot.alt),
                                   L.ptr(bias.data if bias is not None else None), L.ptr(res), L.ptr(y),
                                   L.stream_ptr()), "evt_conv1d_fwd")
    if e0 is not None:
        _t1(e0, "fwd", m, nseq, lin, y.numel() if res is not None else 0)
    return y


def _bwd_data(slot, dy, y, x, dx_add, nseq, lin, in_slope, out_act, out_slope):
    m = slot.module
    dx = torch.empty((nseq, lin, m.cin), dtype=dy.dtype, device=dy.device)
    p = slot.params(nseq, lin, in_slope, out_act, out_slope)
    e0 = _t0()
    L.check(L.lib().evt_conv1d_bwd_data(C.byref(p), L.ptr(dy), L.ptr(y if out_act != L.ACT_NONE else None),
                                        L.ptr(slot.reg), L.ptr(slot.alt), L.ptr(x if in_slope != 1.0 else None),
                                        L.ptr(dx_add), L.ptr(dx), L.stream_ptr()), "evt_conv1d_bwd_data")
    if e0 is not None:
        extra = (dy.numel() if out_act != L.ACT_NONE else 0) + (dx.numel() if in_slope != 1.0 else 0) + \
                (dx.numel() if dx_add is not None else 0)
        _t1(e0, "bwd_data", m, nseq, lin, extra)
    return dx


def _bwd_weight(slot, x, dy, y, nseq, lin, in_slope, out_act, out_slope):
    bank = slot.bank
    if slot.packed_member:
        raise L.EvtError("weight gradient of a packed projection member requested on its own: inside a bf16 runtime the "
                         "q / k / v projections of a windowed attention layer run (and are differentiated) as one pack")
    if bank.defer_n > 0 and TRACE is None:
        bank._deferred.append((slot, x, dy, y, nseq, lin, in_slope, out_act, out_slope))
        bank._deferred_on.add(torch.cuda.current_stream(bank.device))
        bank._deferred_bytes += x.numel() * x.element_size() + dy.numel() * dy.element_size()
        if len(bank._deferred) >= bank.defer_n or bank._deferred_bytes >= bank.defer_bytes:
            bank.flush_deferred()
        return
    _bwd_weight_now(slot, x, dy, y, nseq, lin, in_slope, out_act, out_slope)


def _bwd_weight_now(slot, x, dy, y, nseq, lin, in_slope, out_act, out_slope):
    m = slot.module
    p = slot.params(nseq, lin, in_slope, out_act, out_slope)
    dbias = None
    if m.bias is not None:
        if m.bias.grad is None:
            m.bias.grad = torch.zeros_like(m.bias)
        dbias = m.bias.grad
    e0 = _t0()
    if slot.bank.parts_on:
        sp = slot._wgp
        if sp is None:
            sp = slot._wgp = L.WgradParts()
            sp.dw_extra = slot.dw_extra.data_ptr() if slot.parts > 1 else None
            sp.part_stride = (slot.layout.reg_elems + 127) // 128 * 128
            sp.db_part = slot.db_part.data_ptr() if (dbias is not None and not m.transposed) else None
            sp.used_dev = slot.used.data_ptr()
            sp.parts = slot.parts
        sp.prev_used, sp.dirty0 = slot.wg_used, int(slot.wg_dirty)
        ws = slot.bank.scratch()
        sp.ws, sp.ws_floats = ws.data_ptr(), ws.numel()
        L.check(L.lib().evt_conv1d_bwd_weight_parts(C.byref(p), L.ptr(x), L.ptr(dy),
                                                    L.ptr(y if out_act != L.ACT_NONE else None), L.ptr(slot.dw),
                                                    L.ptr(dbias), C.byref(sp), L.stream_ptr()),
                "evt_conv1d_bwd_weight_parts")
        slot.wg_used, slot.wg_dirty = max(slot.wg_used, int(sp.used)), True
    else:
        L.check(L.lib().evt_conv1d_bwd_weight(C.byref(p), L.ptr(x), L.ptr(dy),
                                              L.ptr(y if out_act != L.ACT_NONE else None), L.ptr(slot.dw), L.ptr(dbias),
                                              L.stream_ptr()), "evt_conv1d_bwd_weight")
    if e0 is not None:
        _t1(e0, "bwd_weight", m, nseq, lin, dy.numel() if out_act != L.ACT_NONE else 0)


class ConvFn(torch.autograd.Function):

    @staticmethod
    def forward(ctx, x, anchor, res, slot, in_slope, out_act, out_slope):
        ctx.pre = False
        if in_slope != 1.0 and x.is_cuda and x.dim() == 3 and PLAIN_X and L.lib().evt_conv1d_wants_plain_x(
                C.byref(slot.params(x.size(0), x.size(1), in_slope, out_act, out_slope))):
            xa = torch.empty_like(x)
            e0 = _t0()
            L.check(L.lib().evt_leaky_relu(L.dt_of(x), L.ptr(x), C.c_float(in_slope), L.ptr(xa), C.c_int64(x.numel()),
                                           L.stream_ptr()), "evt_leaky_relu")
            if e0 is not None:
                _t1_elt(e0, "lrelu_kernel", 2 * x.numel() * x.element_size(), slot.module)
            y = _fwd(slot, xa, res, 1.0, out_act, out_slope)
            x, ctx.pre = xa, True
        else:
            y = _fwd(slot, x, res, in_slope, out_act, out_slope)
        ctx.slot, ctx.cfg = slot, (in_slope, out_act, out_slope)
        ctx.has_res = res is not None
        ctx.save_for_backward(x, y if out_act != L.ACT_NONE else None)
        return y

    @staticmethod
    def backward(ctx, dy):
        x, y = ctx.saved_tensors
        slot = ctx.slot
        in_slope, out_act, out_slope = ctx.cfg
        dy = dy.contiguous()
        nseq, lin = x.size(0), x.size(1)
        if out_act != L.ACT_NONE and L.lib().evt_conv1d_wants_plain_dy(
                C.byref(slot.params(nseq, lin, in_slope, out_act, out_slope))):
            dy_eff = torch.empty_like(dy)
            e0 = _t0()
            L.check(L.lib().evt_dact_mul(L.dt_of(dy), L.ptr(dy), L.ptr(y), int(out_act), C.c_float(out_slope),
                                         L.ptr(dy_eff), C.c_int64(dy.numel()), L.stream_ptr()), "evt_dact_mul")
            if e0 is not None:
                _t1_elt(e0, "dact_mul_kernel", 3 * dy.numel() * dy.element_size(), slot.module)
            dy, y, out_act, out_slope = dy_eff, None, L.ACT_NONE, 1.0
        if slot.bank.weight_grads:
            _bwd_weight(slot, x, dy, y, nseq, lin, 1.0 if ctx.pre else in_slope, out_act, out_slope)
        dx = None
        if ctx.needs_input_grad[0]:
            dx = _bwd_data(slot, dy, y, x, None, nseq, lin, in_slope, out_act, out_slope)
        dres = dy if (ctx.has_res and ctx.needs_input_grad[2]) else None
        if dres is not None and out_act != L.ACT_NONE:
            raise L.EvtError("residual + output activation: residual is added after the activation, "
                             "its gradient is dy (supported), but was not expected here")
        return dx, None, dres, None, None, None, None


def _resunit_params(s1, s2, x, slope):
    m1, m2 = s1.module, s2.module
    if (not L.is_half(x.dtype) or not x.is_cuda or not x.is_contiguous() or x.dim() != 3 or m1.cin != m1.cout
            or m2.cin != m2.cout or m1.cin != m2.cin or m1.k != m2.k or m2.dil != 1 or m1.stride != 1 or m2.stride != 1
            or m1.groups != 1 or m2.groups != 1 or m1.transposed or m2.transposed
            or m1.pad != m1.dil * (m1.k - 1) // 2 or m2.pad != (m2.k - 1) // 2 or s1.bank.impl != L.IMPL_AUTO):
        return None
    p = L.ResUnitParams(L.dt_code(x.dtype), x.size(0), x.size(1), m1.cin, m1.k, m1.dil, float(slope))
    return p if L.lib().evt_resunit_supported(C.byref(p)) else None


def _resunit_wide_params(s1, s2, x, slope):
    m1, m2 = s1.module, s2.module
    if (not L.is_half(x.dtype) or not x.is_cuda or not x.is_contiguous() or x.dim() != 3 or m1.cin != m1.cout
            or m2.cin != m2.cout or m1.cin != m2.cin or m1.k != m2.k or m2.dil != 1 or m1.stride != 1 or m2.stride != 1
            or m1.groups != 1 or m2.groups != 1 or m1.transposed or m2.transposed
            or m1.pad != m1.dil * (m1.k - 1) // 2 or m2.pad != (m2.k - 1) // 2 or s1.bank.impl != L.IMPL_AUTO):
        return None
    p = L.ResUnitParams(L.dt_code(x.dtype), x.size(0), x.size(1), m1.cin, m1.k, m1.dil, float(slope))
    return p if L.lib().evt_resunit_wide_supported(C.byref(p)) else None


def _t1_unit(e0, m1, m2, x):
    e0, rf = e0
    e1 = torch.cuda.Event(enable_timing=True)
    e1.record()
    if rf is not None:
        rf.__exit__(None, None, None)
    n, ln, c = x.shape
    macs = n * ln * c * c * (m1.k + m2.k)
    TRACE.append((L.lib().evt_last_kernel_tag().decode(), "fwd", 2 * macs, 4 * x.numel() * 2 + (m1.v.numel() + m2.v.numel()) * 2,
                  e0, e1, f"unit {c}>{c} k{m1.k} d{m1.dil} n{n} L{ln}", m1))


def _lrelu(x, slope, owner=None):
    out = torch.empty_like(x)
    e0 = _t0()
    L.check(L.lib().evt_leaky_relu(L.dt_of(x), L.ptr(x), C.c_float(slope), L.ptr(out), C.c_int64(x.numel()),
                                   L.stream_ptr()), "evt_leaky_relu")
    if e0 is not None:
        _t1_elt(e0, "lrelu_kernel", 2 * x.numel() * x.element_size(), owner)
    return out


def _add3(a, b, c, scale, out, owner):
    e0 = _t0()
    L.check(L.lib().evt_add3_scale(L.dt_of(a), L.ptr(a), L.ptr(b), L.ptr(c), C.c_float(scale), L.ptr(out),
                                   C.c_int64(a.numel()), L.stream_ptr()), "evt_add3_scale")
    if e0 is not None:
        _t1_elt(e0, "add3_scale_kernel", (2 + (b is not None) + (c is not None)) * a.numel() * a.element_size(), owner)
    return out


class ResUnitFn(torch.autograd.Function):

    @staticmethod
    def forward(ctx, x, anchor, s1, s2, slope):
        fused = _resunit_params(s1, s2, x, slope)
        if fused is not None:
            m1, m2 = s1.module, s2.module
            xa, mid_a, y = torch.empty_like(x), torch.empty_like(x), torch.empty_like(x)
            e0 = _t0()
            L.check(L.lib().evt_resunit_fwd(C.byref(fused), L.ptr(x), L.ptr(s1.reg), L.ptr(s2.reg),
                                            L.ptr(m1.bias.data if m1.bias is not None else None),
                                            L.ptr(m2.bias.data if m2.bias is not None else None), L.ptr(xa), L.ptr(mid_a),
                                            L.ptr(y), L.stream_ptr()), "evt_resunit_fwd")
            if e0 is not None:
                _t1_unit(e0, m1, m2, x)
            ctx.s1, ctx.s2, ctx.slope = s1, s2, slope
            ctx.save_for_backward(xa, mid_a)
            return y
        wide = _resunit_wide_params(s1, s2, x, slope)
        if wide is not None:
            m1, m2 = s1.module, s2.module
            xa, mid_a, y = torch.empty_like(x), torch.empty_like(x), torch.empty_like(x)
            e0 = _t0()
            L.check(L.lib().evt_resunit_wide_fwd(C.byref(wide), L.ptr(x), L.ptr(s1.reg), L.ptr(s2.reg),
                                                 L.ptr(m1.bias.data if m1.bias is not None else None),
                                                 L.ptr(m2.bias.data if m2.bias is not None else None), L.ptr(xa),
                                                 L.ptr(mid_a), L.ptr(y), L.stream_ptr()), "evt_resunit_wide_fwd")
            if e0 is not None:
                _t1_unit(e0, m1, m2, x)
            ctx.s1, ctx.s2, ctx.slope = s1, s2, slope
            ctx.save_for_backward(xa, mid_a)
            return y
        xa = _lrelu(x, slope, s1.module)
        mid_a = _fwd(s1, xa, None, 1.0, L.ACT_LRELU, slope)
        y = _fwd(s2, mid_a, x, 1.0, L.ACT_NONE, 1.0)
        ctx.s1, ctx.s2, ctx.slope = s1, s2, slope
        ctx.save_for_backward(xa, mid_a)
        return y

    @staticmethod
    def backward(ctx, dy):
        xa, mid_a = ctx.saved_tensors
        s1, s2, slope = ctx.s1, ctx.s2, ctx.slope
        dy = dy.contiguous()
        nseq, lin = xa.size(0), xa.size(1)
        if ctx.needs_input_grad[0]:
            dx = resunit_bwd(s1, s2, dy, xa, mid_a, slope, 1.0)
            if dx is not None:
                return dx, None, None, None, None
            wide = _resunit_wide_params(s1, s2, xa, slope)
            if wide is not None:
                m1, m2 = s1.module, s2.module
                dmid, dx = torch.empty_like(dy), torch.empty_like(dy)
                e0 = _t0()
                L.check(L.lib().evt_resunit_wide_bwd_data(C.byref(wide), L.ptr(dy), C.c_float(1.0), L.ptr(xa), L.ptr(mid_a),
                                                          L.ptr(s1.alt), L.ptr(s2.alt), L.ptr(dmid), L.ptr(dx),
                                                          L.stream_ptr()), "evt_resunit_wide_bwd_data")
                if e0 is not None:
                    _t1_unit_bwd(e0, m1, m2, xa, False)
                if s2.bank.weight_grads:
                    _bwd_weight(s2, mid_a, dy, None, nseq, lin, 1.0, L.ACT_NONE, 1.0)
                    _bwd_weight(s1, xa, dmid, None, nseq, lin, 1.0, L.ACT_NONE, 1.0)
                return dx, None, None, None, None
        if s2.bank.weight_grads:
            _bwd_weight(s2, mid_a, dy, None, nseq, lin, 1.0, L.ACT_NONE, 1.0)
        dmid = _bwd_data(s2, dy, None, mid_a, None, nseq, lin, slope, L.ACT_NONE, 1.0)
        if s1.bank.weight_grads:
            _bwd_weight(s1, xa, dmid, None, nseq, lin, 1.0, L.ACT_NONE, 1.0)
        dx = None
        if ctx.needs_input_grad[0]:
            dx = _bwd_data(s1, dmid, None, xa, dy, nseq, lin, slope, L.ACT_NONE, 1.0)
        return dx, None, None, None, None


def _t1_unit_bwd(e0, m1, m2, xa, wg):
    e0, rf = e0
    e1 = torch.cuda.Event(enable_timing=True)
    e1.record()
    if rf is not None:
        rf.__exit__(None, None, None)
    n, ln, c = xa.shape
    macs = n * ln * c * c * (m1.k + m2.k) * (2 if wg else 1)
    wb = (m1.v.numel() + m2.v.numel()) * (2 + (4 if wg else 0))
    TRACE.append((L.lib().evt_last_kernel_tag().decode(), "bwd_unit", 2 * macs, 4 * xa.numel() * 2 + wb, e0, e1,
                  f"unit {c}>{c} k{m1.k} d{m1.dil} n{n} L{ln}", m1))


def resunit_bwd(s1, s2, dy, xa, mid_a, slope, dy_scale=1.0):
# ... 232 lines not shown
```

### easevoice_trainer_amd/hip/disc.py

```python
import ctypes as C
import os

import torch

from . import conv as HC
from . import lib as L

_ALL = os.environ.get("EVT_BRANCH_STREAMS", "1") != "0"
MPD_STREAMS = int(os.environ.get("EVT_MPD_STREAMS", "2")) if _ALL else 1
_side = {}


def _new_stream(dev, k):
    return L.role_stream(dev, f"lane{k}", ring=1)


def _branches(dev, n_items):
    n = MPD_STREAMS if (dev.type == "cuda" and HC.TRACE is None) else 1
    if n <= 1:
        return [None] * n_items, []
    pool = _side.setdefault(dev, [])
    while len(pool) < n - 1:
        pool.append(_new_stream(dev, len(pool)))
    lanes = [None] + pool[: n - 1]
    per = [lanes[i % n] for i in range(n_items)]
    return per, pool[: n - 1]


ENC_STREAM = _ALL and os.environ.get("EVT_ENC_STREAM", "1") != "0"


def enc_lane(dev):
    if not ENC_STREAM or dev.type != "cuda" or HC.TRACE is not None:
        return None
    pool = _side.setdefault(dev, [])
    if not pool:
        pool.append(_new_stream(dev, 0))
    return pool[0]


DEC_STREAM = _ALL and os.environ.get("EVT_DEC_STREAM", "1") != "0"


def dec_lane(dev):
    if not DEC_STREAM or dev.type != "cuda" or HC.TRACE is not None:
        return None
    pool = _side.setdefault(dev, [])
    while len(pool) < 2:
        pool.append(_new_stream(dev, len(pool)))
    return pool[1]


class _On:

    def __init__(self, s):
        self.cm = torch.cuda.stream(s) if s is not None else None

    def __enter__(self):
        if self.cm is not None:
            self.cm.__enter__()

    def __exit__(self, *a):
        if self.cm is not None:
            self.cm.__exit__(*a)


def mpd_fold(periods, cd, src0, src1=None):
    src0 = src0.contiguous()
    n0, T = src0.shape
    n1, dt1 = 0, L.dt_of(src0)
    if src1 is not None:
        src1 = src1.contiguous()
        n1, dt1 = src1.size(0), L.dt_of(src1)
    outs = [torch.empty(((n0 + n1) * p, (T + p - 1) // p, 1), dtype=cd, device=src0.device) for p in periods]
    per = (C.c_int32 * len(periods))(*periods)
    ptrs = (C.c_void_p * len(periods))(*[o.data_ptr() for o in outs])
    L.check(L.lib().evt_mpd_fold(L.dt_of(src0), L.ptr(src0), n0, dt1, L.ptr(src1), n1, T, per, len(periods), ptrs,
                                 L.dt_of(outs[0]), L.stream_ptr()), "evt_mpd_fold")
    return outs


def mpd_unfold(periods, grads, b0, n, T, dtype):
    grads = [g.contiguous() for g in grads]
    out = torch.empty((n, T), dtype=dtype, device=grads[0].device)
    per = (C.c_int32 * len(periods))(*periods)
    ptrs = (C.c_void_p * len(periods))(*[g.data_ptr() for g in grads])
    L.check(L.lib().evt_mpd_unfold(L.dt_of(grads[0]), ptrs, per, len(periods), b0, n, T, L.dt_of(out), L.ptr(out),
                                   L.stream_ptr()), "evt_mpd_unfold")
    return out


class MPDFoldFn(torch.autograd.Function):

    @staticmethod
    def forward(ctx, x, periods, cd):
        ctx.periods, ctx.shape, ctx.dtype = periods, tuple(x.shape), x.dtype
        return tuple(mpd_fold(periods, cd, x))

    @staticmethod
    def backward(ctx, *grads):
        n, T = ctx.shape
        gs = []
        for g, p in zip(grads, ctx.periods):
            gs.append(g if g is not None else torch.zeros((n * p, (T + p - 1) // p, 1), dtype=grads[0].dtype,
                                                          device=grads[0].device))
        return mpd_unfold(ctx.periods, gs, 0, n, T, ctx.dtype), None, None


def _seg_table(a, b, da, scales, device):
    segs = [L.Seg(x.data_ptr(), y.data_ptr() if y is not None else None, g.data_ptr() if g is not None else None,
                  x.numel(), sc, 0) for x, y, g, sc in zip(a, b, da, scales)]
    return L.struct_to_device(segs, device)


class MPDGenLossFn(torch.autograd.Function):
    @staticmethod
    def forward(ctx, anchor, plan, periods, y_hat, y_real):
        nd = len(plan)
        n_items, T = y_hat.shape
        dev = y_hat.device
        cd = plan[0][0][0].bank.dtype
        dt = L.dt_code(cd)
        both = mpd_fold(periods, cd, y_real, y_hat)
        maps, saved = [], []
        lanes, sides = _branches(dev, nd)
        main = torch.cuda.current_stream(dev) if sides else None
        for st in sides:
            st.wait_stream(main)
        for (slots, acts), x, lane in zip(plan, both, lanes):
            ys = []
            with _On(lane):
                for s, (act, slope) in zip(slots, acts):
                    x = HC._fwd(s, x, None, 1.0, act, slope)
                    ys.append(x)
            if lane is not None:
                for y in ys:
                    y.record_stream(main)
            maps.append(ys)
        for st in sides:
            main.wait_stream(st)
        fa, fb, fs, la, ls = [], [], [], [], []
        for ys in maps:
            for y in ys:
                h = y.size(0) // 2
                fa.append(y[h:])
                fb.append(y[:h])
                fs.append(2.0 / y[h:].numel())
            lg = ys[-1][ys[-1].size(0) // 2:]
            la.append(lg)
            ls.append(1.0 / lg.numel())
        out = torch.zeros(2, dtype=torch.float32, device=dev)
        L.check(L.lib().evt_l1_multi_fwd(dt, L.ptr(_seg_table(fa, fb, [None] * len(fa), fs, dev)), len(fa),
                                         L.ptr(out[1:]), L.stream_ptr()), "evt_l1_multi_fwd")
        L.check(L.lib().evt_lsgan_multi_fwd(dt, L.ptr(_seg_table(la, [None] * nd, [None] * nd, ls, dev)), nd,
                                            C.c_float(1.0), L.ptr(out[:1]), L.stream_ptr()), "evt_lsgan_multi_fwd")
        ctx.plan, ctx.dt = plan, dt
        ctx.counts = [len(ys) for ys in maps]
        ctx.in_shapes = [(x.size(0) // 2, x.size(1), 1) for x in both]
        ctx.periods, ctx.wav = periods, (n_items, T, y_hat.dtype)
        ctx.save_for_backward(*[y for ys in maps for y in ys])
        logits = [lg.reshape(n_items, -1).detach() for lg in la]
        ctx.mark_non_differentiable(*logits)
        return (out[0], out[1], *logits)

    @staticmethod
    def backward(ctx, dgen, dfm, *_unused):
        plan, dt = ctx.plan, ctx.dt
        flat = list(ctx.saved_tensors)
        maps, at = [], 0
        for c in ctx.counts:
            maps.append(flat[at: at + c])
            at += c
        dev = flat[0].device
        nd = len(plan)
        fa, fb, fs, fg, la, ls, lgr = [], [], [], [], [], [], []
        for ys in maps:
            for y in ys:
                h = y.size(0) // 2
                fa.append(y[h:])
                fb.append(y[:h])
                fs.append(2.0 / y[h:].numel())
                fg.append(torch.empty_like(y[h:]))
            lg = ys[-1][ys[-1].size(0) // 2:]
            la.append(lg)
            ls.append(1.0 / lg.numel())
            lgr.append(torch.empty_like(lg))
        dl = torch.stack([dgen.reshape(()).float(), dfm.reshape(()).float()]).contiguous()
        L.check(L.lib().evt_l1_multi_bwd(dt, L.ptr(_seg_table(fa, fb, fg, fs, dev)), len(fa), L.ptr(dl[1:]),
                                         L.stream_ptr()), "evt_l1_multi_bwd")
        L.check(L.lib().evt_lsgan_multi_bwd(dt, L.ptr(_seg_table(la, [None] * nd, lgr, ls, dev)), nd, C.c_float(1.0),
                                            L.ptr(dl[:1]), L.stream_ptr()), "evt_lsgan_multi_bwd")
        grads, gi = [], 0
        lanes, sides = _branches(dev, nd)
        main = torch.cuda.current_stream(dev) if sides else None
        for st in sides:
            st.wait_stream(main)
        for (slots, acts), ys, lg_grad, in_shape, lane in zip(plan, maps, lgr, ctx.in_shapes, lanes):
            nl = len(slots)
            mg = fg[gi: gi + nl]
            gi += nl
            with _On(lane):
                dy = _branch_bwd(slots, acts, ys, mg, lg_grad, in_shape, dt)
            if lane is not None:
                dy.record_stream(main)
            grads.append(dy)
        for st in sides:
            main.wait_stream(st)
        n_items, T, wdt = ctx.wav
        return None, None, None, mpd_unfold(ctx.periods, grads, 0, n_items, T, wdt), None


def _branch_bwd(slots, acts, ys, mg, lg_grad, in_shape, dt):
    nl = len(slots)
    dy = mg[-1] + lg_grad
    for l in reversed(range(nl)):
        s, (act, slope) = slots[l], acts[l]
        y_act = ys[l][ys[l].size(0) // 2:]
        half = y_act.size(0)
        lin = ys[l - 1].size(1) if l > 0 else in_shape[1]
        add = mg[l - 1] if l > 0 else None
        a_kind, a_slope, y_arg = act, slope, (y_act if act != L.ACT_NONE else None)
        if act != L.ACT_NONE and L.lib().evt_conv1d_wants_plain_dy(C.byref(s.params(half, lin, 1.0, act, slope))):
            dy_eff = torch.empty_like(dy)
            L.check(L.lib().evt_dact_mul(dt, L.ptr(dy), L.ptr(y_act), int(act), C.c_float(slope), L.ptr(dy_eff),
                                         C.c_int64(dy.numel()), L.stream_ptr()), "evt_dact_mul")
            dy, y_arg, a_kind, a_slope = dy_eff, None, L.ACT_NONE, 1.0
        if add is not None and s.module.groups > 1:
            dy = HC._bwd_data(s, dy.contiguous(), y_arg, None, None, half, lin, 1.0, a_kind, a_slope)
            dy.add_(add)
        else:
            dy = HC._bwd_data(s, dy.contiguous(), y_arg, None, add, half, lin, 1.0, a_kind, a_slope)
    return dy
```

### easevoice_trainer_amd/hip/lib.py

```python
import ctypes as C
import os

import torch

_HERE = os.path.dirname(os.path.abspath(__file__))
LIB_PATH = os.path.join(os.path.dirname(_HERE), "libevt_hip.so")
LIB_PATH_F16 = os.path.join(os.path.dirname(_HERE), "libevt_hip_f16.so")

DT_F32, DT_BF16, DT_F16 = 0, 1, 2
HALF_DTYPES = (torch.bfloat16, torch.float16)
ACT_NONE, ACT_LRELU, ACT_TANH = 0, 1, 2
IMPL_AUTO, IMPL_NAIVE, IMPL_IGEMM = 0, 1, 2


class EvtError(RuntimeError):
    pass


class ConvParams(C.Structure):
    _fields_ = [
        ("dtype", C.c_int32), ("nseq", C.c_int32), ("lin", C.c_int32), ("cin", C.c_int32), ("cout", C.c_int32),
        ("k", C.c_int32), ("stride", C.c_int32), ("pad", C.c_int32), ("dil", C.c_int32), ("groups", C.c_int32),
        ("transposed", C.c_int32), ("in_slope", C.c_float), ("out_act", C.c_int32), ("out_slope", C.c_float),
        ("impl", C.c_int32),
    ]


class ResUnitParams(C.Structure):
    _fields_ = [("dtype", C.c_int32), ("nseq", C.c_int32), ("L", C.c_int32), ("C", C.c_int32), ("k", C.c_int32),
                ("dil", C.c_int32), ("slope", C.c_float)]


class ResUnitFwdJob(C.Structure):
    _fields_ = [("p", ResUnitParams), ("x", C.c_void_p), ("w1_reg", C.c_void_p), ("w2_reg", C.c_void_p),
                ("b1", C.c_void_p), ("b2", C.c_void_p), ("xa", C.c_void_p), ("mid_a", C.c_void_p), ("y", C.c_void_p)]


class ResUnitBwdJob(C.Structure):
    _fields_ = [("p", ResUnitParams), ("dy_scale", C.c_float), ("dy", C.c_void_p), ("xa", C.c_void_p),
                ("mid_a", C.c_void_p), ("w1_alt", C.c_void_p), ("w2_alt", C.c_void_p), ("dx", C.c_void_p),
                ("dmid", C.c_void_p), ("dw1", C.c_void_p), ("dw2", C.c_void_p), ("db1", C.c_void_p), ("db2", C.c_void_p)]


class WLayout(C.Structure):
    _fields_ = [
        ("d0", C.c_int32), ("d1", C.c_int32), ("k", C.c_int32), ("stride", C.c_int32),
        ("reg_ck", C.c_int32), ("reg_nchunk", C.c_int32), ("reg_kp", C.c_int32),
        ("alt_ck", C.c_int32), ("alt_nchunk", C.c_int32), ("alt_kp", C.c_int32), ("alt_nphase", C.c_int32),
        ("reg_elems", C.c_int64), ("alt_elems", C.c_int64),
    ]


class WPrepItem(C.Structure):
    _fields_ = [
        ("v", C.c_void_p), ("g", C.c_void_p), ("reg", C.c_void_p), ("alt", C.c_void_p),
        ("dw", C.c_void_p), ("dv", C.c_void_p), ("dg", C.c_void_p),
        ("lay", WLayout), ("dtype", C.c_int32), ("src_d1", C.c_int32),
        ("dw_extra", C.c_void_p), ("dw_part_stride", C.c_int64), ("db_part", C.c_void_p), ("db", C.c_void_p),
        ("used", C.c_void_p),
    ]


class FragItem(C.Structure):
    _fields_ = [("src", C.c_void_p), ("dst", C.c_void_p), ("rows", C.c_int32), ("ktot", C.c_int32)]


class WgradParts(C.Structure):
    _fields_ = [("dw_extra", C.c_void_p), ("part_stride", C.c_int64), ("db_part", C.c_void_p), ("used_dev", C.c_void_p),
                ("parts", C.c_int32), ("prev_used", C.c_int32), ("used", C.c_int32), ("dirty0", C.c_int32),
                ("ws", C.c_void_p), ("ws_floats", C.c_int64)]


class Seg(C.Structure):
    _fields_ = [("a", C.c_void_p), ("b", C.c_void_p), ("da", C.c_void_p), ("n", C.c_int64),
                ("scale", C.c_float), ("pad_", C.c_int32)]


class KlParams(C.Structure):
    _fields_ = [("B", C.c_int32), ("T", C.c_int32), ("C", C.c_int32), ("time_inner", C.c_int32),
                ("dt_z_p", C.c_int32), ("dt_logs_q", C.c_int32), ("dt_m_p", C.c_int32), ("dt_logs_p", C.c_int32)]


class AdamWSeg(C.Structure):
    _fields_ = [("begin", C.c_int64), ("end", C.c_int64), ("lr", C.c_float), ("weight_decay", C.c_float)]


class AttnParams(C.Structure):
    _fields_ = [
        ("dtype", C.c_int32), ("B", C.c_int32), ("L", C.c_int32), ("H", C.c_int32), ("D", C.c_int32),
        ("x_len", C.c_int32),
        ("q_stride_b", C.c_int64), ("q_stride_l", C.c_int64), ("q_stride_h", C.c_int64),
        ("o_stride_b", C.c_int64), ("o_stride_l", C.c_int64), ("o_stride_h", C.c_int64),
        ("dropout_p", C.c_float), ("seed", C.c_uint32),
    ]


class SampleParams(C.Structure):
    _fields_ = [("V", C.c_int32), ("eos", C.c_int32), ("top_k", C.c_int32), ("no_eos_steps", C.c_int32),
                ("ymax", C.c_int32), ("top_p", C.c_float), ("temperature", C.c_float),
                ("repetition_penalty", C.c_float), ("seed", C.c_uint32), ("noise_rows", C.c_int32)]


class RowSample(C.Structure):
    _fields_ = [("top_k", C.c_int32), ("top_p", C.c_float), ("temperature", C.c_float),
                ("repetition_penalty", C.c_float)]


DEC_POS, DEC_IDX, DEC_YCOUNT, DEC_YLEN, DEC_SEED = 0, 1, 2, 3, 4


class SAChunk(C.Structure):
    _fields_ = [("begin", C.c_int64), ("end", C.c_int64), ("tensor", C.c_int32), ("pad_", C.c_int32)]


class ScaledAdamHP(C.Structure):
    _fields_ = [("lr", C.c_float), ("beta1", C.c_float), ("beta2", C.c_float), ("eps", C.c_float),
                ("scalar_lr_scale", C.c_float), ("scalar_max", C.c_float), ("step", C.c_int32), ("pad_", C.c_int32)]


class MhaParams(C.Structure):
    _fields_ = [("dtype", C.c_int32), ("B", C.c_int32), ("H", C.c_int32), ("D", C.c_int32), ("Tq", C.c_int32),
                ("Tk", C.c_int32), ("window", C.c_int32), ("n_heads_rel", C.c_int32), ("ldq", C.c_int64),
                ("ldk", C.c_int64), ("ldo", C.c_int64), ("scale", C.c_float), ("dropout_p", C.c_float),
                ("site", C.c_uint32), ("pad_", C.c_uint32), ("seed_dev", C.c_void_p)]


_libs = {}
_half = torch.bfloat16


def set_half(dtype) -> None:
    global _half
    if dtype in HALF_DTYPES:
        _half = dtype


def half():
    return _half


def is_half(dtype) -> bool:
    return dtype in HALF_DTYPES


def dt_code(dtype) -> int:
    if dtype == torch.float32:
        return DT_F32
    if dtype in HALF_DTYPES:
        if dtype != _half:
            raise EvtError(f"{dtype} data while the {_half} build of the library is selected: call hip.lib.set_half({dtype}) "
                           "(the engines do, at the top of a step)")
        return DT_BF16 if dtype == torch.bfloat16 else DT_F16
    raise EvtError(f"unsupported dtype {dtype}")


def _check_fresh(handle, LIB_PATH=LIB_PATH):
    csrc = os.path.join(os.path.dirname(_HERE), "csrc")
    if os.environ.get("EVT_ALLOW_STALE_LIB") == "1" or not os.path.isdir(csrc):
        return
    from ..build import source_hash

    have = handle.evt_version().decode()
    want = source_hash()
    if f"src={want}" not in have:
        raise EvtError(f"{LIB_PATH} is stale: built from sources {have.split('src=')[-1]!r}, the tree has {want!r}; "
                       "rebuild with `python -m easevoice_trainer_amd.build` (EVT_ALLOW_STALE_LIB=1 overrides)")


def lib():
    _lib = _libs.get(_half)
    if _lib is None:
        path = LIB_PATH if _half == torch.bfloat16 else LIB_PATH_F16
        if not os.path.exists(path):
            raise EvtError(
                f"{path} not found: build it with `python -m easevoice_trainer_amd.build` "
                "(or __graft_entry__.build()). There is no fallback path.")
        _lib = C.CDLL(path)
        _lib.evt_version.restype = C.c_char_p
        _check_fresh(_lib, path)
        _lib.evt_half_dtype.restype = C.c_int32
        if _lib.evt_half_dtype() != (DT_BF16 if _half == torch.bfloat16 else DT_F16):
            raise EvtError(f"{path} serves half code {_lib.evt_half_dtype()}: not the {_half} build")
        _libs[_half] = _lib
        _lib.evt_conv1d_lout.restype = C.c_int32
        _lib.evt_mel_workspace_floats.restype = C.c_int64
        _lib.evt_workspace_bytes.restype = C.c_int64
        _lib.evt_last_kernel_tag.restype = C.c_char_p
        _lib.evt_resunit_bwd_ws_floats.restype = C.c_int64
        _lib.evt_debug_kernel_tags.restype = None
    return _lib


def check(rc: int, what: str) -> None:
    if rc != 0:
        raise EvtError(f"{what} failed with code {rc}")


def dt_of(t: torch.Tensor) -> int:
    return dt_code(t.dtype)


def torch_dtype(dt: int) -> torch.dtype:
    return {DT_F32: torch.float32, DT_BF16: torch.bfloat16, DT_F16: torch.float16}[dt]


def ptr(t):
    if t is None:
        return C.c_void_p(0)
    if not t.is_contiguous():
        raise EvtError("non-contiguous tensor passed to the C ABI")
    return C.c_void_p(t.data_ptr())


_hip_rt = None
_role_pools = {}


def own_stream(device):
    global _hip_rt
    device = torch.device(device)
    if _hip_rt is None:
        path = "libamdhip64.so"
        try:
            with open("/proc/self/maps") as f:
                for line in f:
                    if "libamdhip64.so" in line:
                        path = line.split(None, 5)[-1].strip()
                        break
        except OSError:
            pass
        _hip_rt = C.CDLL(path)
        _hip_rt.hipStreamCreateWithFlags.argtypes = [C.POINTER(C.c_void_p), C.c_uint]
        _hip_rt.hipStreamCreateWithFlags.restype = C.c_int
    h = C.c_void_p()
    with torch.cuda.device(device):
        rc = _hip_rt.hipStreamCreateWithFlags(C.byref(h), 1)
    if rc != 0 or not h.value:
        raise EvtError(f"hipStreamCreateWithFlags failed ({rc})")
    return torch.cuda.ExternalStream(h.value, device=device)


def role_stream(device, role: str, ring: int = 4):
    device = torch.device(device)
    if device.index is None:
        device = torch.device("cuda", torch.cuda.current_device())
    pool = _role_pools.setdefault((device.index, role), [[], 0])
    if len(pool[0]) < ring:
        pool[0].append(own_stream(device))
        return pool[0][-1]
    st = pool[0][pool[1] % ring]
    pool[1] += 1
    return st


def stream_ptr():
    return C.c_void_p(torch.cuda.current_stream().cuda_stream)


_PINNED_KEEP = []


def struct_to_device(items, device) -> torch.Tensor:
    if not items:
        raise EvtError("empty table")
    arr = (type(items[0]) * len(items))(*items)
    buf = bytes(arr)
    device = torch.device(device)
    if device.type != "cuda":
        return torch.frombuffer(bytearray(buf), dtype=torch.uint8).to(device)
    host = torch.empty(len(buf), dtype=torch.uint8, pin_memory=True)
    host.copy_(torch.frombuffer(bytearray(buf), dtype=torch.uint8))
    dev = torch.empty(len(buf), dtype=torch.uint8, device=device)
    dev.copy_(host, non_blocking=True)
    if torch.cuda.is_current_stream_capturing():
        _PINNED_KEEP.append(host)
    else:
        dev._evt_host = host
    return dev
```

### easevoice_trainer_amd/module/models.py

```python

import os

import torch
from torch import nn
from torch.nn import functional as F

from ..hip import lib as L
from ..hip.conv import Add3ScaleFn, EvtConv1d, GatedActFn, res_stage, res_unit
from ..hip.enc import new_site, rel_self_attention, unbind_rows, wn_residual, wn_residual_last
from ..hip.frontend import RvqEncoder, ncl_to_nlc
from ..hip.wn import wn_stack
from . import commons
from .attentions import Encoder, MultiHeadAttention, PointwiseEvtConv, linear_rows, pointwise

LRELU_SLOPE = 0.1
N_SYMBOLS = 732


def get_padding(kernel_size, dilation=1):
    return (kernel_size * dilation - dilation) // 2


class _ComputeDtype:
    cd = torch.float32
# ... 441 lines not shown
            x = self.ups[i](x, in_slope=LRELU_SLOPE)
            blocks = [self.resblocks[i * self.num_kernels + j] for j in range(self.num_kernels)]
            if x.is_cuda:
                xs = res_stage(x, blocks, LRELU_SLOPE, 1.0 / self.num_kernels)
                if xs is not None:
                    x = xs
                    continue
            lane = None
            if x.is_cuda and len(blocks) == 3:
                from ..hip.disc import _On, dec_lane

                lane = dec_lane(x.device)
            if lane is not None:
                main = torch.cuda.current_stream(x.device)
                lane.wait_stream(main)
                with _On(lane):
                    r0, r1 = blocks[0](x), blocks[1](x)
                x.record_stream(lane)
                r2 = blocks[2](x)
                main.wait_stream(lane)
                r0.record_stream(main)
                r1.record_stream(main)
                rs = [r0, r1, r2]
            else:
                rs = [b(x) for b in blocks]
            while len(rs) < 3:
                rs.append(None)
            x = Add3ScaleFn.apply(rs[0], rs[1], rs[2], 1.0 / self.num_kernels, self)
        return self.conv_post(x, in_slope=0.01, out_act=L.ACT_TANH)


class DiscriminatorP(nn.Module, _ComputeDtype):

    def __init__(self, period, kernel_size=5, stride=3, use_spectral_norm=False):
        super().__init__()
        if use_spectral_norm:
            raise L.EvtError("spectral_norm discriminators are not used by configs/s2.json")
        self.period = period
        chans = [1, 32, 128, 512, 1024, 1024]
        self.convs = nn.ModuleList([
            EvtConv1d(chans[i], chans[i + 1], kernel_size, stride=(stride if i < 4 else 1),
                      padding=get_padding(kernel_size, 1), weight_norm=True, kdims=2) for i in range(5)])
        self.conv_post = EvtConv1d(1024, 1, 3, padding=1, weight_norm=True, kdims=2)

    def prepare(self, x):
        n, t = x.shape
        p = self.period
        if t % p != 0:
            x = F.pad(x.unsqueeze(1), (0, p - (t % p)), "reflect").squeeze(1)
            t = x.size(1)
        return x.view(n, t // p, p).transpose(1, 2).reshape(n * p, t // p, 1).to(self.cd).contiguous()

    def plan(self):
        convs = list(self.convs) + [self.conv_post]
        return (tuple(c._slot for c in convs),
                tuple([(L.ACT_LRELU, LRELU_SLOPE)] * len(self.convs) + [(L.ACT_NONE, 1.0)]))

    def forward(self, x):
        return self.forward_prepared(self.prepare(x))

    def forward_prepared(self, x):
        n = x.size(0) // self.period
        fmap = []
        for l in self.convs:
            x = l(x, out_act=L.ACT_LRELU, out_slope=LRELU_SLOPE)
            fmap.append(x)
        x = self.conv_post(x)
        fmap.append(x)
        return x.view(n, -1), fmap


class DiscriminatorS(nn.Module, _ComputeDtype):

    def __init__(self, use_spectral_norm=False):
        super().__init__()
        if use_spectral_norm:
            raise L.EvtError("spectral_norm discriminators are not used by configs/s2.json")
        spec = [(1, 16, 15, 1, 1, 7), (16, 64, 41, 4, 4, 20), (64, 256, 41, 4, 16, 20), (256, 1024, 41, 4, 64, 20),
                (1024, 1024, 41, 4, 256, 20), (1024, 1024, 5, 1, 1, 2)]
        self.convs = nn.ModuleList([EvtConv1d(ci, co, k, stride=s, groups=g, padding=p, weight_norm=True)
                                    for ci, co, k, s, g, p in spec])
        self.conv_post = EvtConv1d(1024, 1, 3, padding=1, weight_norm=True)

    def prepare(self, x):
        return x.unsqueeze(-1).to(self.cd).contiguous()

    def plan(self):
        convs = list(self.convs) + [self.conv_post]
        return (tuple(c._slot for c in convs),
                tuple([(L.ACT_LRELU, LRELU_SLOPE)] * len(self.convs) + [(L.ACT_NONE, 1.0)]))

    def forward(self, x):
        return self.forward_prepared(self.prepare(x))

    def forward_prepared(self, x):
        fmap = []
        for l in self.convs:
            x = l(x, out_act=L.ACT_LRELU, out_slope=LRELU_SLOPE)
            fmap.append(x)
        x = self.conv_post(x)
        fmap.append(x)
        return x.view(x.size(0), -1), fmap


class MultiPeriodDiscriminator(nn.Module):

    def __init__(self, use_spectral_norm=False):
        super().__init__()
        periods = [2, 3, 5, 7, 11]
        self.discriminators = nn.ModuleList([DiscriminatorS(use_spectral_norm)] +
                                            [DiscriminatorP(p, use_spectral_norm=use_spectral_norm) for p in periods])

    def periods(self):
        return tuple(getattr(d, "period", 1) for d in self.discriminators)

    def _prepared(self, y, y2=None):
        if y.is_cuda:
            from ..hip.disc import MPDFoldFn, mpd_fold

            cd = self.discriminators[0].cd
            if y2 is None and y.requires_grad:
                return list(MPDFoldFn.apply(y, self.periods(), cd))
            if y2 is None or not (y.requires_grad or y2.requires_grad):
                return mpd_fold(self.periods(), cd, y, y2)
        x = y if y2 is None else torch.cat([y.float(), y2.float()], dim=0)
        return [d.prepare(x.float()) for d in self.discriminators]

    def forward_single(self, y):
        y = y.reshape(y.size(0), -1)
        outs, fmaps = [], []
        for d, x in zip(self.discriminators, self._prepared(y)):
            o, f = d.forward_prepared(x)
            outs.append(o)
            fmaps.append(f)
        return outs, fmaps

    def generator_losses(self, y, y_hat):
        from ..hip.disc import MPDGenLossFn

        n = y.size(0)
        plan = tuple(d.plan() for d in self.discriminators)
        if any(s is None for slots, _ in plan for s in slots):
            raise L.EvtError("MultiPeriodDiscriminator used before WeightBank.attach(); there is no eager fallback")
        anchor = plan[0][0][0].bank.anchor
        out = MPDGenLossFn.apply(anchor, plan, self.periods(), y_hat.reshape(n, -1).contiguous(),
                                 y.reshape(n, -1).detach().contiguous())
        return out[0], out[1], list(out[2:])

    def forward_batched(self, y, y_hat):
        n = y.size(0)
        xs = self._prepared(y.reshape(n, -1), y_hat.reshape(n, -1))
        if not y.is_cuda:
            return [d.forward_prepared(x)[0] for d, x in zip(self.discriminators, xs)]
        from ..hip.disc import _On, _branches

        bank = self.discriminators[0].convs[0]._slot.bank if self.discriminators[0].convs[0]._slot is not None else None
        lanes, sides = _branches(y.device, len(self.discriminators)) if (bank is not None and bank.defer_n > 0) \
            else ([None] * len(self.discriminators), [])
        main = torch.cuda.current_stream(y.device) if sides else None
        for st in sides:
            st.wait_stream(main)
        outs = []
        for d, x, lane in zip(self.discriminators, xs, lanes):
            with _On(lane):
                o = d.forward_prepared(x)[0]
            if lane is not None:
                x.record_stream(lane)
                o.record_stream(main)
            outs.append(o)
        for st in sides:
            main.wait_stream(st)
        return outs

    def forward(self, y, y_hat):
        n = y.size(0)
        y_d_rs, y_d_gs, fmap_rs, fmap_gs = [], [], [], []
        for d, x in zip(self.discriminators, self._prepared(y.reshape(n, -1), y_hat.reshape(n, -1))):
            o, f = d.forward_prepared(x)
            y_d_rs.append(o[:n])
            y_d_gs.append(o[n:])
            fmap_rs.append([t[: t.size(0) // 2] for t in f])
            fmap_gs.append([t[t.size(0) // 2:] for t in f])
        return y_d_rs, y_d_gs, fmap_rs, fmap_gs


class SynthesizerTrn(nn.Module, _ComputeDtype):

    def __init__(self, spec_channels, segment_size, inter_channels, hidden_channels, filter_channels, n_heads,
                 n_layers, kernel_size, p_dropout, resblock, resblock_kernel_sizes, resblock_dilation_sizes,
                 upsample_rates, upsample_initial_channel, upsample_kernel_sizes, n_speakers=0, gin_channels=0,
                 use_sdp=True, semantic_frame_rate=None, freeze_quantizer=None, version="v2", **kwargs):
        super().__init__()
        self.spec_channels, self.segment_size, self.inter_channels = spec_channels, segment_size, inter_channels
        self.gin_channels, self.version = gin_channels, version
        self.upsample_rates = upsample_rates
        self.enc_p = TextEncoder(inter_channels, hidden_channels, filter_channels, n_heads, n_layers, kernel_size,
                                 p_dropout, version=version)
        self.dec = Generator(inter_channels, resblock, resblock_kernel_sizes, resblock_dilation_sizes, upsample_rates,
                             upsample_initial_channel, upsample_kernel_sizes, gin_channels=gin_channels)
        self.enc_q = PosteriorEncoder(spec_channels, inter_channels, hidden_channels, 5, 1, 16,
                                      gin_channels=gin_channels)
        self.flow = ResidualCouplingBlock(inter_channels, hidden_channels, 5, 1, 4, gin_channels=gin_channels)
        self.ref_enc = MelStyleEncoder(spec_channels if version == "v1" else 704, style_vector_dim=gin_channels)
        ssl_dim = 768
        assert semantic_frame_rate in ["25hz", "50hz"]
        self.semantic_frame_rate = semantic_frame_rate
        if semantic_frame_rate == "25hz":
            self.ssl_proj = nn.Conv1d(ssl_dim, ssl_dim, 2, stride=2)
        else:
            self.ssl_proj = nn.Conv1d(ssl_dim, ssl_dim, 1, stride=1)
        self.quantizer = ResidualVectorQuantizer(dimension=ssl_dim, n_q=1, bins=1024)
        self.freeze_quantizer = freeze_quantizer
        self.split_backward = False
        self._cut = None
        self._cut2 = None

    def _rvq(self):
        enc = getattr(self, "_rvq_enc", None)
        cb = self.quantizer.vq.layers[0]._codebook
        if enc is None or enc.bank.device != cb.embed.device:
            k = 2 if self.semantic_frame_rate == "25hz" else 1
            enc = RvqEncoder(lambda: self.ssl_proj.weight, lambda: self.ssl_proj.bias, lambda: cb.embed,
                             cb.embed.size(1), cb.codebook_size, k, k, cb.embed.device)
            object.__setattr__(self, "_rvq_enc", enc)
        return enc

    def _quantize(self, ssl):
        with torch.no_grad(), torch.autocast("cuda", enabled=False):
            return rvq_encode(self._rvq(), self.quantizer, ssl, 2 if self.semantic_frame_rate == "25hz" else 1)

    @torch.no_grad()
    def extract_latent(self, x):
        _q, codes = self._quantize(x)
        return codes.transpose(0, 1)

    @torch.no_grad()
    def decode(self, codes, text, refer, noise_scale=0.5, speed=1, noise=None):
        amp = self.cd in (torch.bfloat16, torch.float16)
        with torch.autocast("cuda", dtype=self.cd if amp else torch.bfloat16, enabled=amp):
            ges = []
            for r in (refer if isinstance(refer, (list, tuple)) else [refer]):
                r_cl = r.transpose(1, 2)
                r_cl = r_cl if self.version == "v1" else r_cl[..., :704]
                ges.append(self.ref_enc(r_cl, torch.ones(r_cl.size(0), r_cl.size(1), 1, device=r.device)))
            ge = torch.stack(ges, 0).mean(0)
            B, Tc = codes.size(1), codes.size(2)
            T = Tc * 2 if self.semantic_frame_rate == "25hz" else Tc
            y_lengths = torch.full((B,), T, dtype=torch.long, device=codes.device)
            text_lengths = torch.full((B,), text.size(-1), dtype=torch.long, device=text.device)
            quantized = self.quantizer.decode(codes)
            if self.semantic_frame_rate == "25hz":
                quantized = quantized.repeat_interleave(2, dim=1)
            y_mask = torch.ones(B, T, 1, device=codes.device)
            text_mask = torch.ones(B, text.size(1), 1, device=text.device)
            enc = self.enc_p(quantized, y_mask, text, text_mask, ge, y_lengths, text_lengths, speed=speed)
            if speed != 1:
                _x, m_p, logs_p, y_mask = enc
                y_lengths = torch.full((B,), y_mask.size(1), dtype=torch.long, device=codes.device)
            else:
                _x, m_p, logs_p = enc
            if noise is None:
                noise = torch.randn(B, m_p.size(2), m_p.size(1), device=m_p.device)
            eps = noise[:, :, :m_p.size(1)].transpose(1, 2).to(m_p.dtype)
            z_p = m_p + eps * torch.exp(logs_p) * noise_scale
            ym = y_mask.to(self.cd)
            z = self.flow(z_p, ym, g=ge, reverse=True, lens=y_lengths.to(torch.int32))
            o = self.dec(z * ym, g=ge)
        return o.transpose(1, 2)

    def forward(self, ssl, y, y_lengths, text, text_lengths, eps=None, ids_slice=None):
        dev = y.device
        T = y.size(2)
        y_mask = commons.sequence_mask(y_lengths, T).unsqueeze(-1).to(torch.float32)
        text_mask = commons.sequence_mask(text_lengths, text.size(1)).unsqueeze(-1).to(torch.float32)
        amp = self.cd in (torch.bfloat16, torch.float16)
        with torch.autocast("cuda", dtype=self.cd if amp else torch.bfloat16, enabled=amp):
            lens32 = y_lengths.to(torch.int32)
            y_cl = ncl_to_nlc(y.float(), self.enc_q.pre.cin, self.cd)
            ref_in = y_cl[..., :self.spec_channels] if self.version == "v1" else y_cl[..., :704]
            split = self.split_backward and torch.is_grad_enabled()
            lane = None
            if y.is_cuda and not split:
                from ..hip.disc import _On, enc_lane

                lane = enc_lane(dev)
            if lane is not None and os.environ.get("EVT_QUANT_LANE", "1") != "0":
                main = torch.cuda.current_stream(dev)
                lane.wait_stream(main)
                with _On(lane):
                    quantized, _codes = self._quantize(ssl)
                ssl.record_stream(lane)
                ge = self.ref_enc(ref_in * y_mask.to(self.cd), y_mask, lens32)
            else:
                ge = self.ref_enc(ref_in * y_mask.to(self.cd), y_mask, lens32)
                quantized, _codes = self._quantize(ssl)
            if lane is not None:
                main = torch.cuda.current_stream(dev)
                lane.wait_stream(main)
                with _On(lane):
                    x, m_p, logs_p = self.enc_p(quantized, y_mask, text, text_mask, ge, y_lengths, text_lengths)
                for t in (quantized, y_mask, text, text_mask, ge, y_lengths, text_lengths):
                    t.record_stream(lane)
            else:
                x, m_p, logs_p = self.enc_p(quantized, y_mask, text, text_mask, ge, y_lengths, text_lengths)
            eps_cl = eps.transpose(1, 2) if eps is not None else None
            ym = y_mask.to(self.cd)
            ge_fq = ge
            if split:
                ge_fq = ge.detach().requires_grad_(True)
                m_p_cut, logs_p_cut = m_p.detach().requires_grad_(True), logs_p.detach().requires_grad_(True)
                self._cut2 = ((ge, ge_fq), (m_p, m_p_cut), (logs_p, logs_p_cut))
                m_p, logs_p = m_p_cut, logs_p_cut
            z, m_q, logs_q = self.enc_q(y_cl, ym, g=ge_fq, eps=eps_cl, lens=lens32)
            z_p = self.flow(z, ym, g=ge_fq, lens=lens32)
            if ids_slice is None:
                z_slice, ids_slice = commons.rand_slice_segments(z, y_lengths, self.segment_size)
            else:
                z_slice = commons.slice_segments(z, ids_slice, self.segment_size)
# ... 16 lines not shown
```

### include/evt.h

```cpp
#ifndef EVT_H
#define EVT_H
#include <stddef.h>
#include <stdint.h>

#ifdef __cplusplus
extern "C" {
#endif
#pragma GCC visibility push(default)

#define EVT_DT_F32 0
#define EVT_DT_BF16 1
#define EVT_DT_F16 2
#define EVT_ACT_NONE 0
#define EVT_ACT_LRELU 1
#define EVT_ACT_TANH 2
#define EVT_IMPL_AUTO 0
#define EVT_IMPL_NAIVE 1
#define EVT_IMPL_IGEMM 2

const char* evt_version(void);
int32_t evt_half_dtype(void);
void evt_debug_kernel_tags(int32_t enable);
const char* evt_last_kernel_tag(void);

#define EVT_WS_NONE 0
#define EVT_WS_MEL 1
#define EVT_WS_ATTN_BWD 2
#define EVT_WS_MHA_BWD 3
#define EVT_WS_MASKED_KL 4
int64_t evt_workspace_bytes(int32_t op, const int64_t* dims, int32_t ndims);

typedef struct evt_conv1d_params {
  int32_t dtype;
  int32_t nseq;
  int32_t lin;
  int32_t cin, cout;
  int32_t k, stride, pad, dil, groups;
  int32_t transposed;
  float in_slope;
  int32_t out_act;
  float out_slope;
  int32_t impl;
} evt_conv1d_params;

int32_t evt_conv1d_wants_plain_dy(const evt_conv1d_params* c);

int32_t evt_conv1d_wants_plain_x(const evt_conv1d_params* c);

int32_t evt_conv1d_lout(const evt_conv1d_params* p);

typedef struct evt_wlayout {
  int32_t d0, d1, k, stride;
  int32_t reg_ck, reg_nchunk, reg_kp;
  int32_t alt_ck, alt_nchunk, alt_kp, alt_nphase;
  int64_t reg_elems, alt_elems;
} evt_wlayout;
int evt_conv1d_layout(const evt_conv1d_params* p, evt_wlayout* out);

typedef struct evt_wprep_item {
  const float* v;
  const float* g;
  void* reg;
  void* alt;
  const float* dw;
  float* dv;
  float* dg;
  evt_wlayout lay;
  int32_t dtype;
  int32_t src_d1;
  const float* dw_extra;
  int64_t dw_part_stride;
  const float* db_part;
  float* db;
  const int32_t* used;
} evt_wprep_item;
int evt_wn_fold_multi(const evt_wprep_item* items, const int32_t* row_index, int32_t nrows, void* stream);
int evt_wn_fold_groups(const evt_wprep_item* items, const int32_t* group_index, int32_t ngroups, void* stream);
int evt_wn_grad_multi(const evt_wprep_item* items, const int32_t* row_index, int32_t nrows, void* stream);

int evt_conv1d_fwd(const evt_conv1d_params* p, const void* x, const void* w_reg, const void* w_alt,
                   const float* bias, const void* res, void* y, void* stream);

int evt_conv1d_bwd_data(const evt_conv1d_params* p, const void* dy, const void* y, const void* w_reg,
                        const void* w_alt, const void* x, const void* dx_add, void* dx, void* stream);

int evt_conv1d_bwd_weight(const evt_conv1d_params* p, const void* x, const void* dy, const void* y,
                          float* dw, float* dbias, void* stream);

typedef struct evt_wgrad_parts {
  float* dw_extra;
  int64_t part_stride;
  float* db_part;
  int32_t* used_dev;
  int32_t parts;
  int32_t prev_used;
  int32_t used;
  int32_t dirty0;
  float* ws;
  int64_t ws_floats;
} evt_wgrad_parts;
int evt_conv1d_bwd_weight_parts(const evt_conv1d_params* p, const void* x, const void* dy, const void* y,
                                float* dw, float* dbias, evt_wgrad_parts* sp, void* stream);

typedef struct evt_resunit_params {
  int32_t dtype, nseq, L, C, k, dil;
  float slope;
} evt_resunit_params;
int32_t evt_resunit_supported(const evt_resunit_params* p);
int evt_resunit_fwd(const evt_resunit_params* p, const void* x, const void* w1_reg, const void* w2_reg, const float* b1,
                    const float* b2, void* xa, void* mid_a, void* y, void* stream);

typedef struct evt_resunit_fwd_job {
  evt_resunit_params p;
  const void* x; const void* w1_reg; const void* w2_reg; const float* b1; const float* b2;
  void* xa; void* mid_a; void* y;
} evt_resunit_fwd_job;
int evt_resunit_fwd_multi(const evt_resunit_fwd_job* jobs, int32_t njobs, void* stream);

int32_t evt_resunit_bwd_supported(const evt_resunit_params* p, int32_t with_weight_grads);
int64_t evt_resunit_bwd_ws_floats(const evt_resunit_params* p);
int evt_resunit_bwd(const evt_resunit_params* p, const void* dy, float dy_scale, const void* xa, const void* mid_a,
                    const void* w1_alt, const void* w2_alt, void* dx, void* dmid, float* dw1, float* dw2, float* db1,
                    float* db2, float* ws, int64_t ws_floats, void* stream);
typedef struct evt_resunit_bwd_job {
  evt_resunit_params p;
  float dy_scale;
  const void* dy; const void* xa; const void* mid_a; const void* w1_alt; const void* w2_alt;
  void* dx; void* dmid;
  float* dw1; float* dw2; float* db1; float* db2;
} evt_resunit_bwd_job;
int evt_resunit_bwd_multi(const evt_resunit_bwd_job* jobs, int32_t njobs, float* ws, int64_t ws_floats, void* stream);

int32_t evt_resunit_wide_supported(const evt_resunit_params* p);
int evt_resunit_wide_fwd(const evt_resunit_params* p, const void* x, const void* w1_reg, const void* w2_reg, const float* b1,
                         const float* b2, void* xa, void* mid_a, void* y, void* stream);
int evt_resunit_wide_bwd_data(const evt_resunit_params* p, const void* dy, float dy_scale, const void* xa, const void* mid_a,
                              const void* w1_alt, const void* w2_alt, void* dmid, void* dx, void* stream);

typedef struct evt_frag_item {
  const void* src;
  void* dst;
  int32_t rows, ktot;
} evt_frag_item;
int evt_frag_pack(const evt_frag_item* items, int32_t nitems, void* stream);
int evt_wn_layer_bwd_data(int32_t dtype, const void* dx_next, const void* dacc, const void* x_in, const void* g,
                          const void* w_rs_alt_frag, const void* w_in_alt_frag, const int32_t* lens, void* drs, void* dx_in,
                          void* dx, float* dg, int32_t nseq, int32_t L, int32_t H, int32_t k, int32_t last, void* stream);
int32_t evt_wn_layer_supported(int32_t dtype, int32_t H, int32_t k, int32_t dil);
int evt_wn_layer_fwd(int32_t dtype, const void* x, const void* w_in_frag, const float* b_in, const void* w_rs_frag,
                     const float* b_rs, const void* g, const void* acc_in, const int32_t* lens, void* x_in, void* acts,
                     void* x_out, void* acc_out, int32_t nseq, int32_t L, int32_t H, int32_t k, int32_t last, void* stream);

int evt_add3_scale(int32_t dtype, const void* a, const void* b, const void* c, float scale, void* out,
                   int64_t n, void* stream);

int evt_leaky_relu(int32_t dtype, const void* x, float slope, void* out, int64_t n, void* stream);

int evt_dact_mul(int32_t dtype, const void* dy, const void* y, int32_t act_kind, float slope, void* out, int64_t n,
                 void* stream);

int evt_gated_act_fwd(int32_t dtype, const void* xin, const void* g, void* acts, int32_t nseq, int32_t len,
                      int32_t H, void* stream);
int evt_gated_act_bwd(int32_t dtype, const void* xin, const void* g, const void* dacts, void* dxin, float* dg,
                      int32_t nseq, int32_t len, int32_t H, void* stream);


int evt_mel_fwd(const float* wav, const float* window, const float* mel_basis, float* spec_out, float* mel_out,
                float* ws_spec_re_im, int32_t nseq, int32_t wav_len, int32_t n_fft, int32_t hop, int32_t n_mels,
                void* stream);
int evt_mel_bwd(const float* dmel, const float* window, const float* mel_basis, const float* ws_spec_re_im,
                float* dwav, int32_t nseq, int32_t wav_len, int32_t n_fft, int32_t hop, int32_t n_mels, void* stream);
int64_t evt_mel_workspace_floats(int32_t nseq, int32_t wav_len, int32_t n_fft, int32_t hop, int32_t n_mels);

int evt_ncl_to_nlc(int32_t dtype, const float* src, void* dst, int32_t B, int32_t C, int32_t T, int32_t Cp, void* stream);

int evt_rvq_norms(const float* embed, float* ee, int32_t K, int32_t D, void* stream);
int evt_rvq_select(const float* h, const float* dots, const float* embed, const float* ee, int64_t* codes, float* q_out,
                   int32_t N, int32_t D, int32_t K, int32_t rep, void* stream);

int evt_spec_to_mel(const float* spec, const float* basis, const int64_t* starts, float* out, int32_t B, int32_t F,
                    int32_t T, int32_t M, int32_t nfr, void* stream);

typedef struct evt_seg { const void* a; const void* b; void* da; int64_t n; float scale; int32_t pad_; } evt_seg;
int evt_l1_multi_fwd(int32_t dtype, const evt_seg* segs, int32_t nseg, float* out, void* stream);
int evt_l1_multi_bwd(int32_t dtype, const evt_seg* segs, int32_t nseg, const float* dloss, void* stream);
int evt_lsgan_multi_fwd(int32_t dtype, const evt_seg* segs, int32_t nseg, float target, float* out, void* stream);
int evt_lsgan_multi_bwd(int32_t dtype, const evt_seg* segs, int32_t nseg, float target, const float* dloss,
                        void* stream);

typedef struct evt_kl_params {
  int32_t B, T, C, time_inner;
  int32_t dt_z_p, dt_logs_q, dt_m_p, dt_logs_p;
} evt_kl_params;
int evt_masked_kl_fwd(const evt_kl_params* p, const void* z_p, const void* logs_q, const void* m_p, const void* logs_p,
                      const int32_t* lens, float* out2, void* stream);
int evt_masked_kl_bwd(const evt_kl_params* p, const void* z_p, const void* logs_q, const void* m_p, const void* logs_p,
                      const int32_t* lens, const float* dloss, const float* count, void* dz_p, void* dlogs_q, void* dm_p,
                      void* dlogs_p, void* stream);

typedef struct evt_adamw_seg { int64_t begin, end; float lr; float weight_decay; } evt_adamw_seg;
int evt_adamw_flat(float* param, const float* grad, float* exp_avg, float* exp_avg_sq, int64_t n,
                   const evt_adamw_seg* segs, int32_t nseg, float beta1, float beta2, float eps, int32_t step,
                   float grad_scale, void* stream);
int evt_adamw_flat_dev(float* param, const float* grad, float* exp_avg, float* exp_avg_sq, int64_t n,
                       const evt_adamw_seg* segs, int32_t nseg, float beta1, float beta2, float eps,
                       int32_t* step_counter, float grad_scale, void* stream);
int evt_adamw_flat_dev_range(float* param, const float* grad, float* exp_avg, float* exp_avg_sq, int64_t lo, int64_t hi,
                             const evt_adamw_seg* segs, int32_t nseg, float beta1, float beta2, float eps,
                             int32_t* step_counter, int32_t bump, float grad_scale, void* stream);
int evt_mpd_fold(int32_t src0_dtype, const void* src0, int32_t n0, int32_t src1_dtype, const void* src1, int32_t n1, int32_t T,
                 const int32_t* periods, int32_t nper, void* const* outs, int32_t out_dtype, void* stream);
int evt_mpd_unfold(int32_t grad_dtype, const void* const* douts, const int32_t* periods, int32_t nper, int32_t b0, int32_t n,
                   int32_t T, int32_t dsrc_dtype, void* dsrc, void* stream);

int evt_sumsq(const float* x, int64_t n, float* out, void* stream);

int evt_scaler_unscale(float* grad, int64_t n, const float* scale, float* found_inf, void* stream);
int evt_adamw_flat_dev_guarded(float* param, const float* grad, float* exp_avg, float* exp_avg_sq, int64_t n,
                               const evt_adamw_seg* segs, int32_t nseg, float beta1, float beta2, float eps,
                               int32_t* step_counter, float grad_scale, const float* skip, void* stream);
int evt_scaler_update(float* scale, int32_t* growth_tracker, float* const* found_inf, int32_t nflags, float growth_factor,
                      float backoff_factor, int32_t growth_interval, void* stream);

typedef struct evt_gemm_params {
  int32_t dtype;
  int32_t M, N, K;
  int32_t relu;
} evt_gemm_params;
int evt_gemm_bf16_layout(const evt_gemm_params* g, evt_wlayout* out);
int evt_gemm_bf16_fwd(const evt_gemm_params* g, const void* x, const void* w_reg, const void* w_alt, const float* bias,
                      void* y, void* stream);
int evt_gemm_bf16_bwd_data(const evt_gemm_params* g, const void* dy, const void* w_reg, const void* w_alt, void* dx,
                           void* stream);
int evt_gemm_bf16_bwd_weight(const evt_gemm_params* g, const void* x, const void* dy, float* dw, float* dbias,
                             void* stream);

typedef struct evt_gemm_epilogue {
  float dropout_p;
  uint32_t site;
  const uint32_t* seed_dev;
  const void* gate;
  float gate_pos;
  uint32_t pad_;
  const void* add;
} evt_gemm_epilogue;
int32_t evt_gemm_bf16_fused_supported(const evt_gemm_params* g, int32_t backward_data);
int evt_gemm_bf16_fwd_ex(const evt_gemm_params* g, const void* x, const void* w_reg, const void* w_alt, const float* bias,
                         const evt_gemm_epilogue* epi, void* y, void* stream);
int evt_gemm_bf16_bwd_data_ex(const evt_gemm_params* g, const void* dy, const void* w_reg, const void* w_alt,
                              const evt_gemm_epilogue* epi, void* dx, void* stream);

typedef struct evt_attn_params {
  int32_t dtype, B, L, H, D;
  int32_t x_len;
  int64_t q_stride_b, q_stride_l, q_stride_h;
  int64_t o_stride_b, o_stride_l, o_stride_h;
  float dropout_p;
  uint32_t seed;
} evt_attn_params;
int evt_attn_prefixlm_fwd(const evt_attn_params* p, const void* q, const void* k, const void* v,
                          const int32_t* x_lens, const int32_t* y_lens, void* o, float* lse, void* stream);
int evt_attn_prefixlm_bwd(const evt_attn_params* p, const void* q, const void* k, const void* v, const void* o,
                          const void* d_o, const float* lse, const int32_t* x_lens, const int32_t* y_lens,
                          void* dq, void* dk, void* dv, float* delta_ws, void* stream);

int evt_add_layernorm_fwd(int32_t dtype, const void* x, const void* r, const float* gamma, const float* beta,
                          void* y, float* mean, float* rstd, int64_t rows, int32_t C, float eps, void* stream);
int evt_add_layernorm_bwd(int32_t dtype, const void* x, const void* r, const float* gamma, const void* dy,
                          const float* mean, const float* rstd, void* dxr, float* dgamma, float* dbeta,
                          int64_t rows, int32_t C, void* stream);

int evt_counter_inc(uint32_t* counter, uint32_t inc, void* stream);

int evt_res_dropout_ln_fwd(int32_t dtype, const void* x, const void* y, const float* gamma, const float* beta,
                           const int32_t* lens, int32_t rows_per_seq, float p, const uint32_t* seed_dev, uint32_t site,
                           void* out, float* mean, float* rstd, int64_t rows, int32_t C, float eps, void* stream);
int evt_res_dropout_ln_bwd(int32_t dtype, const void* x, const void* y, const float* gamma, const void* dout,
                           const float* mean, const float* rstd, const int32_t* lens, int32_t rows_per_seq, float p,
                           const uint32_t* seed_dev, uint32_t site, void* dx, void* dy, float* dgamma, float* dbeta,
                           int64_t rows, int32_t C, void* stream);

int evt_relu_dropout_fwd(int32_t dtype, const void* x, float p, const uint32_t* seed_dev, uint32_t site,
                         const int32_t* lens, int32_t rows_per_seq, int32_t C, void* y, int64_t n, void* stream);
int evt_relu_dropout_bwd(int32_t dtype, const void* x, const void* dy, float p, const uint32_t* seed_dev, uint32_t site,
                         const int32_t* lens, int32_t rows_per_seq, int32_t C, void* dx, int64_t n, void* stream);

int evt_wn_residual_fwd(int32_t dtype, const void* x, const void* rs, const void* acc, const int32_t* lens,
                        int32_t rows_per_seq, void* x_out, void* acc_out, int64_t rows, int32_t H, int32_t last,
                        void* stream);
int evt_mish_dropout_fwd(int32_t dtype, int32_t wide_dtype, const void* x, float p, const uint32_t* seed_dev, uint32_t site,
                         void* y, int64_t n, void* stream);
int evt_mish_dropout_bwd(int32_t dtype, int32_t wide_dtype, const void* x, const void* dy, float p, const uint32_t* seed_dev,
                         uint32_t site, void* dx, int64_t n, void* stream);
int evt_glu_dropout_res_fwd(int32_t dtype, int32_t wide_dtype, const void* h, const void* res, float p,
                            const uint32_t* seed_dev, uint32_t site, void* y, int64_t rows, int32_t C, void* stream);
int evt_glu_dropout_res_bwd(int32_t dtype, int32_t wide_dtype, const void* h, const void* dy, float p,
                            const uint32_t* seed_dev, uint32_t site, void* dh, int64_t rows, int32_t C, void* stream);
int evt_reparam_fwd(int32_t dtype, const void* stats, const float* eps, const int32_t* lens, int32_t rows_per_seq,
                    int64_t rows, int32_t C, float* z, float* m, float* logs, void* stream);
int evt_reparam_bwd(int32_t dtype, const float* dz, const float* dm, const float* dlogs, const float* eps, const float* logs,
                    const int32_t* lens, int32_t rows_per_seq, int64_t rows, int32_t C, void* dstats, void* stream);
int evt_coupling_flip_fwd(int32_t dtype, const float* x, const void* stats, const int32_t* lens, int32_t rows_per_seq,
                          int64_t rows, int32_t h, float* y, void* x0n, void* stream);
int evt_coupling_flip_bwd(int32_t dtype, const float* dy, const void* dx0n, const int32_t* lens, int32_t rows_per_seq,
                          int64_t rows, int32_t h, float* dx, void* dstats, void* stream);
int evt_wn_residual_bwd(int32_t dtype, const void* dx_out, const void* dacc_out, const int32_t* lens,
                        int32_t rows_per_seq, void* dx, void* drs, int64_t rows, int32_t H, int32_t last, void* stream);

typedef struct evt_mha_params {
  int32_t dtype;
  int32_t B, H, D;
  int32_t Tq, Tk;
  int32_t window;
  int32_t n_heads_rel;
  int64_t ldq, ldk, ldo;
  float scale;
  float dropout_p;
  uint32_t site;
  uint32_t pad_;
  const uint32_t* seed_dev;
} evt_mha_params;
int evt_mha_fwd(const evt_mha_params* p, const void* q, const void* k, const void* v, const float* emb_k,
                const float* emb_v, const int32_t* lens_q, const int32_t* lens_k, void* out, float* lse, void* stream);
int evt_mha_bwd(const evt_mha_params* p, const void* q, const void* k, const void* v, const void* o, const void* d_o,
                const float* lse, const float* emb_k, const float* emb_v, const int32_t* lens_q, const int32_t* lens_k,
                void* dq, void* dk, void* dv, float* demb_k, float* demb_v, float* delta_ws, void* stream);

int evt_ce_sum_fwd_bwd(int32_t dtype, const void* logits, const int64_t* targets, void* dlogits, float* loss,
                       int32_t* hits, int64_t rows, int32_t V, int32_t topk, int64_t ignore_index, float dloss,
                       void* stream);
int evt_ce_rows_fwd_bwd(int32_t dtype, const void* logits, const int64_t* targets, void* dlogits, float* row_loss,
                        int32_t* hits, int64_t rows, int32_t V, int32_t topk, int64_t ignore_index, void* stream);
int evt_ce_sum_fwd_bwd_ld(int32_t dtype, const void* logits, const int64_t* targets, void* dlogits, float* loss,
                          int32_t* hits, int64_t rows, int32_t V, int64_t ld, int32_t topk, int64_t ignore_index,
                          float dloss, void* stream);
int evt_ce_rows_fwd_bwd_ld(int32_t dtype, const void* logits, const int64_t* targets, void* dlogits, float* row_loss,
// ... 90 lines not shown
```

Baseline: 3480 audio-s/s.

## Fuse feature-matching grad and activation gating into discriminator conv backward-data epilogue

Adds a post-epilogue to the conv backward-data kernels (deep igemm and cout1 paths) that adds the feature-matching L1 gradient sign term and applies the lower layer's leaky-ReLU derivative in place. The discriminator backward chain is restructured around this: the separate fm-grad buffers, the dact_mul passes and the extra adds are skipped, and the LSGAN grad accumulates into the fm buffer. The aim is fewer elementwise kernels and less HBM traffic per discriminator layer. In exchange there is a larger API surface with probe logic, extra bf16 rounding steps in the epilogue, and an env flag that is on by default.

```diff
diff --git a/easevoice_trainer_amd/csrc/conv1d.hip b/easevoice_trainer_amd/csrc/conv1d.hip
--- a/easevoice_trainer_amd/csrc/conv1d.hip
+++ b/easevoice_trainer_amd/csrc/conv1d.hip
@@ -23,7 +23,7 @@
 extern "C" int evt_cin1_bwd_data(const evt_conv1d_params* c, const void* dy, const void* y, const void* w_reg,
                                  const void* gate, const void* dx_add, void* dx, void* stream);
 extern "C" int evt_cout1_bwd_data(const evt_conv1d_params* c, const void* dy, const void* y, const void* w_reg,
-                                  const void* gate, const void* dx_add, void* dx, void* stream);
+                                  const void* gate, const void* dx_add, const evt_bwd_post* post, void* dx, void* stream);
 
 namespace {
 
@@ -1209,13 +1209,19 @@
   return launch_igemm(c->dtype, p, c->cout, c->cin, nphase, st, c->impl == EVT_IMPL_AUTO);
 }
 
-int evt_conv1d_bwd_data(const evt_conv1d_params* c, const void* dy, const void* y, const void* w_reg,
-                        const void* w_alt, const void* x, const void* dx_add, void* dx, void* stream) {
+static int bwd_data_impl(const evt_conv1d_params* c, const void* dy, const void* y, const void* w_reg, const void* w_alt,
+                         const void* x, const void* dx_add, const evt_bwd_post* post, bool probe, void* dx, void* stream) {
   int rc = valid(c);
   if (rc) return rc;
-  if (!dy || !dx) return EVT_EINVAL;
-  if (c->out_act != EVT_ACT_NONE && !y) return EVT_EINVAL;
-  if (c->in_slope != 1.f && !x) return EVT_EINVAL;
+  if (!probe) {
+    if (!dy || !dx) return EVT_EINVAL;
+    if (c->out_act != EVT_ACT_NONE && !y) return EVT_EINVAL;
+    if (c->in_slope != 1.f && !x) return EVT_EINVAL;
+    if (post && ((post->gate || post->fm_real) && !post->act_y)) return EVT_EINVAL;
+    if (post && post->fm_real && !post->fm_dloss) return EVT_EINVAL;
+  }
+  const bool strict = post || probe;
+  if (strict && (c->dtype != EVT_DT_HALF || c->in_slope != 1.f || c->impl == EVT_IMPL_NAIVE)) return EVT_ENOTSUP;
   hipStream_t st = (hipStream_t)stream;
   const bool use_igemm = c->impl != EVT_IMPL_NAIVE && igemm_ok(c);
   if (c->impl == EVT_IMPL_IGEMM && !use_igemm) return EVT_ENOTSUP;
@@ -1223,8 +1229,12 @@
   evt_wlayout l; evt_conv1d_layout(c, &l);
   const void* ysv = c->out_act != EVT_ACT_NONE ? y : nullptr;
   const void* gate = c->in_slope != 1.f ? x : nullptr;
-  if (w_alt && evt_conv::rows16_eligible(c, c->nseq * c->lin, c->cin, c->cout, ysv || gate || dx_add))
+  if (strict) {
+    if (evt_conv::rows16_eligible(c, c->nseq * c->lin, c->cin, c->cout, dx_add || c->out_act != EVT_ACT_NONE)) return EVT_ENOTSUP;
+  } else if (w_alt && evt_conv::rows16_eligible(c, c->nseq * c->lin, c->cin, c->cout, ysv || gate || dx_add)) {
     return evt_conv::launch_rows16(dy, w_alt, nullptr, dx, c->nseq * c->lin, c->cin, c->cout, st);
+  }
+  if (strict && evt_grouped_supported(c)) return EVT_ENOTSUP;
   evt_set_last_tag("conv_naive_bwd_data");
   if (c->impl != EVT_IMPL_NAIVE && !gate && !dx_add && evt_grouped_supported(c)) {
     if (!w_reg) return EVT_EINVAL;
@@ -1232,12 +1242,15 @@
     return evt_grouped_bwd_data(c, dy, y, w_reg, dx, stream);
   }
   if (c->impl != EVT_IMPL_NAIVE && evt_small_kind(c) != 0) {
+    if (strict && evt_small_kind(c) != 1) return EVT_ENOTSUP;
+    if (probe) return EVT_OK;
     if (!w_reg) return EVT_EINVAL;
-    rc = evt_small_kind(c) == 1 ? evt_cout1_bwd_data(c, dy, y, w_reg, gate, dx_add, dx, stream)
+    rc = evt_small_kind(c) == 1 ? evt_cout1_bwd_data(c, dy, y, w_reg, gate, dx_add, post, dx, stream)
                                 : evt_cin1_bwd_data(c, dy, y, w_reg, gate, dx_add, dx, stream);
     if (rc != EVT_ENOTSUP) return rc;
   }
   if (!use_igemm) {
+    if (strict) return EVT_ENOTSUP;
     if (!w_reg) return EVT_EINVAL;
     NvP p = make_nvp(c);
     p.x = dy; p.y_in = ysv; p.w = w_reg; p.gate = gate; p.res = dx_add; p.y = dx;
@@ -1248,9 +1261,10 @@
     return evt_check_launch();
   }
   const void* w = c->transposed ? w_reg : w_alt;
-  if (!w) return EVT_EINVAL;
+  if (!w && !probe) return EVT_EINVAL;
   ConvP p{};
   p.x = dy; p.xact = ysv; p.w = w; p.bias = nullptr; p.res = dx_add; p.gate = gate; p.y = dx;
+  if (probe && c->out_act != EVT_ACT_NONE) p.xact = c;
   p.nseq = c->nseq; p.Lin = lout; p.Lout = c->lin; p.Cin = c->cout; p.Cout = c->cin;
   p.in_slope = 1.f; p.xact_kind = c->out_act; p.xact_slope = c->out_slope; p.out_act = EVT_ACT_NONE;
   p.out_slope = 1.f; p.gate_slope = c->in_slope;
@@ -1273,7 +1287,32 @@
     p.s_in = c->stride; p.dil = 1; p.off_in = -c->pad;
     p.s_out = 1; p.off_out = 0; p.off_out_phase = 0; p.Q = c->lin; p.w_phase_stride = 0;
   }
+  if (strict) {
+    if (c->impl != EVT_IMPL_AUTO || c->cin % 16 || c->cout % 16 ||
+        !evt_conv::deep_eligible(p, c->dtype, c->cin, c->cout, nphase))
+      return EVT_ENOTSUP;
+    if (probe) return EVT_OK;
+    p.post_y = post->act_y; p.fm_real = post->fm_real; p.fm_dloss = post->fm_dloss; p.fm_scale = post->fm_scale;
+    p.post_slope = post->act_slope; p.post_gate = post->gate;
+    return evt_conv::launch_conv_deep(p, c->cin, c->cout, nphase, st);
+  }
   return launch_igemm(c->dtype, p, c->cin, c->cout, nphase, st, c->impl == EVT_IMPL_AUTO);
+}
+
+int evt_conv1d_bwd_data(const evt_conv1d_params* c, const void* dy, const void* y, const void* w_reg,
+                        const void* w_alt, const void* x, const void* dx_add, void* dx, void* stream) {
+  return bwd_data_impl(c, dy, y, w_reg, w_alt, x, dx_add, nullptr, false, dx, stream);
+}
+
+int evt_conv1d_bwd_data_post(const evt_conv1d_params* c, const void* dy, const void* y, const void* w_reg,
+                             const void* w_alt, const void* dx_add, const evt_bwd_post* post, void* dx, void* stream) {
+  if (!post) return EVT_EINVAL;
+  return bwd_data_impl(c, dy, y, w_reg, w_alt, nullptr, dx_add, post, false, dx, stream);
+}
+
+int32_t evt_conv1d_bwd_data_post_ok(const evt_conv1d_params* c) {
+  if (!c) return 0;
+  return bwd_data_impl(c, nullptr, nullptr, nullptr, nullptr, nullptr, nullptr, nullptr, true, nullptr, nullptr) == EVT_OK;
 }
 
 int evt_conv1d_bwd_weight(const evt_conv1d_params* c, const void* x, const void* dy, const void* y, float* dw,
diff --git a/easevoice_trainer_amd/csrc/conv_deep.hip b/easevoice_trainer_amd/csrc/conv_deep.hip
--- a/easevoice_trainer_amd/csrc/conv_deep.hip
+++ b/easevoice_trainer_amd/csrc/conv_deep.hip
@@ -49,6 +49,9 @@
   h16_t* Y = reinterpret_cast<h16_t*>(p.y);
   const h16_t* R = reinterpret_cast<const h16_t*>(p.res);
   const h16_t* G = reinterpret_cast<const h16_t*>(p.gate);
+  const h16_t* PY = reinterpret_cast<const h16_t*>(p.post_y);
+  const h16_t* FR = PY ? reinterpret_cast<const h16_t*>(p.fm_real) : nullptr;
+  const float dl = FR ? p.fm_dloss[0] * p.fm_scale : 0.f;
   const int tid = threadIdx.x;
   const int c16 = tid % CPR, r0 = tid / CPR;
 #pragma unroll
@@ -75,6 +78,26 @@
         if (G) f *= (h2f(gp[e]) > 0.f ? 1.f : p.gate_slope);
         if (R) f += h2f(rp[e]);
         vp[e] = f2h(f);
+      }
+    }
+    if (PY) {
+      const uint4 yv = *reinterpret_cast<const uint4*>(PY + off);
+      uint4 fv = make_uint4(0, 0, 0, 0);
+      if (FR) fv = *reinterpret_cast<const uint4*>(FR + off);
+      h16_t* vp = reinterpret_cast<h16_t*>(&v);
+      const h16_t* yp = reinterpret_cast<const h16_t*>(&yv);
+      const h16_t* fp = reinterpret_cast<const h16_t*>(&fv);
+#pragma unroll
+      for (int e = 0; e < 8; ++e) {
+        const float ya = h2f(yp[e]);
+        h16_t t = vp[e];
+        if (FR) {
+          const float d = ya - h2f(fp[e]);
+          const h16_t fmv = f2h(d > 0.f ? dl : (d < 0.f ? -dl : 0.f));
+          t = f2h(h2f(t) + h2f(fmv));
+        }
+        if (p.post_gate) t = f2h(h2f(t) * (ya > 0.f ? 1.f : p.post_slope));
+        vp[e] = t;
       }
     }
     *reinterpret_cast<uint4*>(Y + off) = v;
diff --git a/easevoice_trainer_amd/csrc/conv_p.h b/easevoice_trainer_amd/csrc/conv_p.h
--- a/easevoice_trainer_amd/csrc/conv_p.h
+++ b/easevoice_trainer_amd/csrc/conv_p.h
@@ -27,6 +27,12 @@
   float out_slope;
   float gate_slope;
   int P, Y;
+  const void* post_y;
+  const void* fm_real;
+  const float* fm_dloss;
+  float fm_scale;
+  float post_slope;
+  int post_gate;
 };
 
 struct WgP {
diff --git a/easevoice_trainer_amd/csrc/conv_small.hip b/easevoice_trainer_amd/csrc/conv_small.hip
--- a/easevoice_trainer_amd/csrc/conv_small.hip
+++ b/easevoice_trainer_amd/csrc/conv_small.hip
@@ -16,6 +16,7 @@
   float* dbias;
   int tile;
   int step_q, step_r;
+  const void* post_y; const void* fm_real; const float* fm_dloss; float fm_scale, post_slope; int post_gate;
 };
 
 __device__ __forceinline__ long sreg_index(const SP& p, int d0, int d1, int t) {
@@ -484,6 +485,9 @@
   const long total = (long)p.nseq * p.lin * ppr;
   const T* dy = reinterpret_cast<const T*>(p.dy);
   const T* ys = reinterpret_cast<const T*>(p.y_in);
+  const T* PY = reinterpret_cast<const T*>(p.post_y);
+  const T* FR = PY ? reinterpret_cast<const T*>(p.fm_real) : nullptr;
+  const float dl = FR ? p.fm_dloss[0] * p.fm_scale : 0.f;
   for (long idx = (long)blockIdx.x * 256 + threadIdx.x; idx < total; idx += (long)gridDim.x * 256) {
     const long row = idx / ppr;
     const int c0 = (int)(idx - row * ppr) * V;
@@ -505,16 +509,30 @@
     }
     const long off = row * p.cin + c0;
     T outv[V];
-    uint4 gv = make_uint4(0, 0, 0, 0), av = make_uint4(0, 0, 0, 0);
+    uint4 gv = make_uint4(0, 0, 0, 0), av = make_uint4(0, 0, 0, 0), yv = make_uint4(0, 0, 0, 0), fv = make_uint4(0, 0, 0, 0);
     if (gate) gv = *reinterpret_cast<const uint4*>(reinterpret_cast<const T*>(gate) + off);
     if (dx_add) av = *reinterpret_cast<const uint4*>(reinterpret_cast<const T*>(dx_add) + off);
+    if (PY) yv = *reinterpret_cast<const uint4*>(PY + off);
+    if (FR) fv = *reinterpret_cast<const uint4*>(FR + off);
     const T* pg = reinterpret_cast<const T*>(&gv);
     const T* pa = reinterpret_cast<const T*>(&av);
+    const T* py = reinterpret_cast<const T*>(&yv);
+    const T* pf = reinterpret_cast<const T*>(&fv);
 #pragma unroll
     for (int e = 0; e < V; ++e) {
       float v = acc[e];
       if (gate) v *= (to_f<T>(pg[e]) > 0.f ? 1.f : p.in_slope);
       if (dx_add) v += to_f<T>(pa[e]);
+      if (PY) {
+        const float ya = to_f<T>(py[e]);
+        if (FR) {
+          const float d = ya - to_f<T>(pf[e]);
+          const T fmv = from_f<T>(d > 0.f ? dl : (d < 0.f ? -dl : 0.f));
+          if (dx_add) v = to_f<T>(from_f<T>(v));
+          v += to_f<T>(fmv);
+        }
+        if (p.post_gate) v = to_f<T>(from_f<T>(v)) * (ya > 0.f ? 1.f : p.post_slope);
+      }
       outv[e] = from_f<T>(v);
     }
     *reinterpret_cast<uint4*>(reinterpret_cast<T*>(p.y) + off) = *reinterpret_cast<uint4*>(outv);
@@ -756,9 +774,13 @@
 }
 
 extern "C" int evt_cout1_bwd_data(const evt_conv1d_params* c, const void* dy, const void* y, const void* w_reg,
-                                  const void* gate, const void* dx_add, void* dx, void* stream) {
+                                  const void* gate, const void* dx_add, const evt_bwd_post* post, void* dx, void* stream) {
   SP p = make_sp(c);
   p.dy = dy; p.y_in = c->out_act != EVT_ACT_NONE ? y : nullptr; p.w = w_reg; p.y = dx;
+  if (post) {
+    p.post_y = post->act_y; p.fm_real = post->fm_real; p.fm_dloss = post->fm_dloss; p.fm_scale = post->fm_scale;
+    p.post_slope = post->act_slope; p.post_gate = post->gate;
+  }
   const int V = c->dtype == EVT_DT_HALF ? 8 : 4;
   const long total = (long)p.nseq * p.lin * (p.cin / V);
   long blocks = (total + 255) / 256;
diff --git a/easevoice_trainer_amd/csrc/elementwise.hip b/easevoice_trainer_amd/csrc/elementwise.hip
--- a/easevoice_trainer_amd/csrc/elementwise.hip
+++ b/easevoice_trainer_amd/csrc/elementwise.hip
@@ -360,6 +360,12 @@
   return -2.f * (target - a) * dl;
 }
 
+template <typename T>
+__device__ __forceinline__ T seg_store(T old, float g, bool accum) {
+  const T r = from_f<T>(g);
+  return accum ? from_f<T>(to_f<T>(old) + to_f<T>(r)) : r;
+}
+
 template <typename T, int MODE, bool BWD>
 __global__ __launch_bounds__(256) void seg_flat_kernel(const evt_seg* segs, int nseg, float target, float* out,
                                                        const float* dloss) {
@@ -387,13 +393,14 @@
     T* da = reinterpret_cast<T*>(s.da);
     const long i0 = max(lo, s0) - s0, i1 = min(hi, s1) - s0;
     const float dl = BWD ? dloss[0] * s.scale : 0.f;
+    const bool acc_da = BWD && MODE == 1 && s.accum != 0;
     float part = 0.f;
     const long v0 = min(i1, (i0 + V - 1) / V * V), v1 = v0 + (i1 - v0) / V * V;
     const bool vec_ok = ((((uintptr_t)a) | (MODE == 0 ? (uintptr_t)b : 0) | (BWD ? (uintptr_t)da : 0)) & 15) == 0;
     if (vec_ok) {
       for (long i = i0 + threadIdx.x; i < v0; i += 256) {
         const float av = to_f<T>(a[i]), bv = MODE == 0 ? to_f<T>(b[i]) : 0.f;
-        if (BWD) da[i] = from_f<T>(seg_grad<T, MODE>(av, bv, target, dl)); else part += seg_term<T, MODE>(av, bv, target);
+        if (BWD) da[i] = seg_store<T>(da[i], seg_grad<T, MODE>(av, bv, target, dl), acc_da); else part += seg_term<T, MODE>(av, bv, target);
       }
       for (long i = v0 + (long)threadIdx.x * V; i < v1; i += 256L * V) {
         const uint4 va = *reinterpret_cast<const uint4*>(a + i);
@@ -401,23 +408,25 @@
         if (MODE == 0) vb = *reinterpret_cast<const uint4*>(b + i);
         const T* pa = reinterpret_cast<const T*>(&va);
         const T* pb = reinterpret_cast<const T*>(&vb);
-        uint4 vo;
+        uint4 vo = make_uint4(0, 0, 0, 0);
+        if (BWD && acc_da) vo = *reinterpret_cast<const uint4*>(da + i);
         T* po = reinterpret_cast<T*>(&vo);
 #pragma unroll
         for (int e = 0; e < V; ++e) {
           const float av = to_f<T>(pa[e]), bv = MODE == 0 ? to_f<T>(pb[e]) : 0.f;
-          if (BWD) po[e] = from_f<T>(seg_grad<T, MODE>(av, bv, target, dl)); else part += seg_term<T, MODE>(av, bv, target);
+          if (BWD) po[e] = seg_store<T>(po[e], seg_grad<T, MODE>(av, bv, target, dl), acc_da);
+          else part += seg_term<T, MODE>(av, bv, target);
         }
         if (BWD) *reinterpret_cast<uint4*>(da + i) = vo;
       }
       for (long i = v1 + threadIdx.x; i < i1; i += 256) {
         const float av = to_f<T>(a[i]), bv = MODE == 0 ? to_f<T>(b[i]) : 0.f;
-        if (BWD) da[i] = from_f<T>(seg_grad<T, MODE>(av, bv, target, dl)); else part += seg_term<T, MODE>(av, bv, target);
+        if (BWD) da[i] = seg_store<T>(da[i], seg_grad<T, MODE>(av, bv, target, dl), acc_da); else part += seg_term<T, MODE>(av, bv, target);
       }
     } else {
       for (long i = i0 + threadIdx.x; i < i1; i += 256) {
         const float av = to_f<T>(a[i]), bv = MODE == 0 ? to_f<T>(b[i]) : 0.f;
-        if (BWD) da[i] = from_f<T>(seg_grad<T, MODE>(av, bv, target, dl)); else part += seg_term<T, MODE>(av, bv, target);
+        if (BWD) da[i] = seg_store<T>(da[i], seg_grad<T, MODE>(av, bv, target, dl), acc_da); else part += seg_term<T, MODE>(av, bv, target);
       }
     }
     acc += part * s.scale;
diff --git a/easevoice_trainer_amd/hip/conv.py b/easevoice_trainer_amd/hip/conv.py
--- a/easevoice_trainer_amd/hip/conv.py
+++ b/easevoice_trainer_amd/hip/conv.py
@@ -531,6 +531,97 @@
     return dx
 
 
+DISC_FUSED_BWD = os.environ.get("EVT_DISC_FUSED_BWD", "1") != "0"
+ENOTSUP = 95
+
+
+def wants_plain_dy(slot, nseq, lin, out_act, out_slope):
+    return out_act != L.ACT_NONE and bool(
+        L.lib().evt_conv1d_wants_plain_dy(C.byref(slot.params(nseq, lin, 1.0, out_act, out_slope))))
+
+
+def bwd_post_ok(slot, nseq, lin, out_act, out_slope):
+    return bool(L.lib().evt_conv1d_bwd_data_post_ok(C.byref(slot.params(nseq, lin, 1.0, out_act, out_slope))))
+
+
+def _bwd_data_post(slot, dy, y, dx_add, nseq, lin, out_act, out_slope, act_y, act_slope, gate, fm_real=None,
+                   fm_dloss=None, fm_scale=0.0):
+    m = slot.module
+    dx = torch.empty((nseq, lin, m.cin), dtype=dy.dtype, device=dy.device)
+    p = slot.params(nseq, lin, 1.0, out_act, out_slope)
+    post = L.BwdPost(act_y.data_ptr(), fm_real.data_ptr() if fm_real is not None else None,
+                     fm_dloss.data_ptr() if fm_dloss is not None else None, fm_scale, act_slope, 1 if gate else 0, 0)
+    e0 = _t0()
+    rc = L.lib().evt_conv1d_bwd_data_post(C.byref(p), L.ptr(dy), L.ptr(y if out_act != L.ACT_NONE else None),
+                                          L.ptr(slot.reg), L.ptr(slot.alt), L.ptr(dx_add), C.byref(post), L.ptr(dx),
+                                          L.stream_ptr())
+    if rc == ENOTSUP:
+        if e0 is not None and e0[1] is not None:
+            e0[1].__exit__(None, None, None)
+        return None
+    L.check(rc, "evt_conv1d_bwd_data_post")
+    if e0 is not None:
+        extra = (dy.numel() if out_act != L.ACT_NONE else 0) + dx.numel() * (1 + (dx_add is not None) + (fm_real is not None))
+        _t1(e0, "bwd_data", m, nseq, lin, extra)
+    return dx
+
+
+def _dact_mul(dy, y, act, slope, owner):
+    out = torch.empty_like(dy)
+    e0 = _t0()
+    L.check(L.lib().evt_dact_mul(L.dt_of(dy), L.ptr(dy), L.ptr(y), int(act), C.c_float(slope), L.ptr(out),
+                                 C.c_int64(dy.numel()), L.stream_ptr()), "evt_dact_mul")
+    if e0 is not None:
+        _t1_elt(e0, "dact_mul_kernel", 3 * dy.numel() * dy.element_size(), owner)
+    return out
+
+
+class DiscChainFn(torch.autograd.Function):
+
+    @staticmethod
+    def forward(ctx, x, anchor, slots, acts):
+        ys, h = [], x
+        for s, (act, slope) in zip(slots, acts):
+            h = _fwd(s, h, None, 1.0, act, slope)
+            ys.append(h)
+        ctx.slots, ctx.acts = slots, acts
+        ctx.save_for_backward(x, *ys)
+        return ys[-1]
+
+    @staticmethod
+    def backward(ctx, dy):
+        x, *ys = ctx.saved_tensors
+        slots, acts = ctx.slots, ctx.acts
+        dy = dy.contiguous()
+        nseq = x.size(0)
+        pre, dx = False, None
+        for l in reversed(range(len(slots))):
+            s, (act, slope) = slots[l], acts[l]
+            xin = ys[l - 1] if l > 0 else x
+            lin = xin.size(1)
+            y = ys[l] if act != L.ACT_NONE else None
+            if pre:
+                y, act, slope = None, L.ACT_NONE, 1.0
+            elif wants_plain_dy(s, nseq, lin, act, slope):
+                dy = _dact_mul(dy, y, act, slope, s.module)
+                y, act, slope = None, L.ACT_NONE, 1.0
+            if s.bank.weight_grads:
+                _bwd_weight(s, xin, dy, y, nseq, lin, 1.0, act, slope)
+            pre, dx = False, None
+            if l == 0 and not ctx.needs_input_grad[0]:
+                break
+            if l > 0:
+                pact, pslope = acts[l - 1]
+                plin = (ys[l - 2] if l > 1 else x).size(1)
+                if pact == L.ACT_LRELU and wants_plain_dy(slots[l - 1], nseq, plin, pact, pslope):
+                    dx = _bwd_data_post(s, dy, y, None, nseq, lin, act, slope, xin, pslope, True)
+                    pre = dx is not None
+            if dx is None:
+                dx = _bwd_data(s, dy, y, None, None, nseq, lin, 1.0, act, slope)
+            dy = dx
+        return dx, None, None, None
+
+
 def _bwd_weight(slot, x, dy, y, nseq, lin, in_slope, out_act, out_slope):
     bank = slot.bank
     if slot.packed_member:
@@ -611,13 +702,7 @@
         nseq, lin = x.size(0), x.size(1)
         if out_act != L.ACT_NONE and L.lib().evt_conv1d_wants_plain_dy(
                 C.byref(slot.params(nseq, lin, in_slope, out_act, out_slope))):
-            dy_eff = torch.empty_like(dy)
-            e0 = _t0()
-            L.check(L.lib().evt_dact_mul(L.dt_of(dy), L.ptr(dy), L.ptr(y), int(out_act), C.c_float(out_slope),
-                                         L.ptr(dy_eff), C.c_int64(dy.numel()), L.stream_ptr()), "evt_dact_mul")
-            if e0 is not None:
-                _t1_elt(e0, "dact_mul_kernel", 3 * dy.numel() * dy.element_size(), slot.module)
-            dy, y, out_act, out_slope = dy_eff, None, L.ACT_NONE, 1.0
+            dy, y, out_act, out_slope = _dact_mul(dy, y, out_act, out_slope, slot.module), None, L.ACT_NONE, 1.0
         if slot.bank.weight_grads:
             _bwd_weight(slot, x, dy, y, nseq, lin, 1.0 if ctx.pre else in_slope, out_act, out_slope)
         dx = None
diff --git a/easevoice_trainer_amd/hip/disc.py b/easevoice_trainer_amd/hip/disc.py
--- a/easevoice_trainer_amd/hip/disc.py
+++ b/easevoice_trainer_amd/hip/disc.py
@@ -107,10 +107,24 @@
         return mpd_unfold(ctx.periods, gs, 0, n, T, ctx.dtype), None, None
 
 
-def _seg_table(a, b, da, scales, device):
+def _seg_table(a, b, da, scales, device, accum=0):
     segs = [L.Seg(x.data_ptr(), y.data_ptr() if y is not None else None, g.data_ptr() if g is not None else None,
-                  x.numel(), sc, 0) for x, y, g, sc in zip(a, b, da, scales)]
+                  x.numel(), sc, accum) for x, y, g, sc in zip(a, b, da, scales)]
     return L.struct_to_device(segs, device)
+
+
+def _bwd_plan(slots, acts, ys, in_len):
+    layers, fused = [], []
+    for l, (s, (act, slope)) in enumerate(zip(slots, acts)):
+        half = ys[l].size(0) // 2
+        lin = ys[l - 1].size(1) if l > 0 else in_len
+        plain = HC.wants_plain_dy(s, half, lin, act, slope)
+        call = (L.ACT_NONE, 1.0) if (plain or act == L.ACT_NONE) else (act, slope)
+        layers.append((half, lin, plain, call))
+        if l > 0:
+            fused.append(HC.DISC_FUSED_BWD and HC.bwd_post_ok(s, half, lin, *call))
+    fused.append(False)
+    return layers, fused
 
 
 class MPDGenLossFn(torch.autograd.Function):
@@ -161,6 +175,8 @@
         ctx.save_for_backward(*[y for ys in maps for y in ys])
         logits = [lg.reshape(n_items, -1).detach() for lg in la]
         ctx.mark_non_differentiable(*logits)
+        if HC.DISC_FUSED_BWD:
+            ctx.set_materialize_grads(False)
         return (out[0], out[1], *logits)
 
     @staticmethod
@@ -173,34 +189,44 @@
             at += c
         dev = flat[0].device
         nd = len(plan)
+        zero = None
+        if dgen is None or dfm is None:
+            zero = torch.zeros((), dtype=torch.float32, device=dev)
+        dl = torch.stack([(zero if dgen is None else dgen).reshape(()).float(),
+                          (zero if dfm is None else dfm).reshape(()).float()]).contiguous()
+        fused_on = HC.DISC_FUSED_BWD
+        plans = [_bwd_plan(slots, acts, ys, in_shape[1]) for (slots, acts), ys, in_shape in zip(plan, maps, ctx.in_shapes)]
         fa, fb, fs, fg, la, ls, lgr = [], [], [], [], [], [], []
-        for ys in maps:
-            for y in ys:
+        for ys, (_, fused) in zip(maps, plans):
+            for y, fu in zip(ys, fused):
                 h = y.size(0) // 2
                 fa.append(y[h:])
                 fb.append(y[:h])
                 fs.append(2.0 / y[h:].numel())
-                fg.append(torch.empty_like(y[h:]))
+                fg.append(None if fu else torch.empty_like(y[h:]))
             lg = ys[-1][ys[-1].size(0) // 2:]
             la.append(lg)
             ls.append(1.0 / lg.numel())
-            lgr.append(torch.empty_like(lg))
-        dl = torch.stack([dgen.reshape(()).float(), dfm.reshape(()).float()]).contiguous()
+            lgr.append(fg[-1] if fused_on else torch.empty_like(lg))
         L.check(L.lib().evt_l1_multi_bwd(dt, L.ptr(_seg_table(fa, fb, fg, fs, dev)), len(fa), L.ptr(dl[1:]),
                                          L.stream_ptr()), "evt_l1_multi_bwd")
-        L.check(L.lib().evt_lsgan_multi_bwd(dt, L.ptr(_seg_table(la, [None] * nd, lgr, ls, dev)), nd, C.c_float(1.0),
-                                            L.ptr(dl[:1]), L.stream_ptr()), "evt_lsgan_multi_bwd")
+        L.check(L.lib().evt_lsgan_multi_bwd(dt, L.ptr(_seg_table(la, [None] * nd, lgr, ls, dev, 1 if fused_on else 0)),
+                                            nd, C.c_float(1.0), L.ptr(dl[:1]), L.stream_ptr()), "evt_lsgan_multi_bwd")
         grads, gi = [], 0
         lanes, sides = _branches(dev, nd)
         main = torch.cuda.current_stream(dev) if sides else None
         for st in sides:
             st.wait_stream(main)
-        for (slots, acts), ys, lg_grad, in_shape, lane in zip(plan, maps, lgr, ctx.in_shapes, lanes):
+        for (slots, acts), ys, lg_grad, in_shape, lane, bp in zip(plan, maps, lgr, ctx.in_shapes, lanes, plans):
             nl = len(slots)
             mg = fg[gi: gi + nl]
+            ms = fs[gi: gi + nl]
             gi += nl
             with _On(lane):
-                dy = _branch_bwd(slots, acts, ys, mg, lg_grad, in_shape, dt)
+                if fused_on:
+                    dy = _branch_bwd_fused(slots, acts, ys, mg, ms, dl[1:], bp)
+                else:
+                    dy = _branch_bwd(slots, acts, ys, mg, lg_grad, in_shape, dt)
             if lane is not None:
                 dy.record_stream(main)
             grads.append(dy)
@@ -221,13 +247,39 @@
         add = mg[l - 1] if l > 0 else None
         a_kind, a_slope, y_arg = act, slope, (y_act if act != L.ACT_NONE else None)
         if act != L.ACT_NONE and L.lib().evt_conv1d_wants_plain_dy(C.byref(s.params(half, lin, 1.0, act, slope))):
-            dy_eff = torch.empty_like(dy)
-            L.check(L.lib().evt_dact_mul(dt, L.ptr(dy), L.ptr(y_act), int(act), C.c_float(slope), L.ptr(dy_eff),
-                                         C.c_int64(dy.numel()), L.stream_ptr()), "evt_dact_mul")
-            dy, y_arg, a_kind, a_slope = dy_eff, None, L.ACT_NONE, 1.0
+            dy, y_arg, a_kind, a_slope = HC._dact_mul(dy, y_act, act, slope, s.module), None, L.ACT_NONE, 1.0
         if add is not None and s.module.groups > 1:
             dy = HC._bwd_data(s, dy.contiguous(), y_arg, None, None, half, lin, 1.0, a_kind, a_slope)
             dy.add_(add)
         else:
             dy = HC._bwd_data(s, dy.contiguous(), y_arg, None, add, half, lin, 1.0, a_kind, a_slope)
     return dy
+
+
+def _branch_bwd_fused(slots, acts, ys, mg, ms, dfm, bp):
+    layers, fused = bp
+    dy, pre = mg[-1], False
+    for l in reversed(range(len(slots))):
+        s, (act, slope) = slots[l], acts[l]
+        half, lin, plain, (a_kind, a_slope) = layers[l]
+        y_act = ys[l][half:]
+        if plain and not pre:
+            dy = HC._dact_mul(dy, y_act, act, slope, s.module)
+        y_arg = y_act if a_kind != L.ACT_NONE else None
+        pre, dx = False, None
+        if l > 0 and fused[l - 1]:
+            below, gate = ys[l - 1], layers[l - 1][2]
+            dx = HC._bwd_data_post(s, dy.contiguous(), y_arg, None, half, lin, a_kind, a_slope, below[half:], acts[l - 1][1],
+                                   gate, below[:half], dfm, ms[l - 1])
+            if dx is None:
+                raise L.EvtError("evt_conv1d_bwd_data_post refused a layer evt_conv1d_bwd_data_post_ok accepted")
+            pre = gate
+        else:
+            add = mg[l - 1] if l > 0 else None
+            if add is not None and s.module.groups > 1:
+                dx = HC._bwd_data(s, dy.contiguous(), y_arg, None, None, half, lin, 1.0, a_kind, a_slope)
+                dx.add_(add)
+            else:
+                dx = HC._bwd_data(s, dy.contiguous(), y_arg, None, add, half, lin, 1.0, a_kind, a_slope)
+        dy = dx
+    return dy
diff --git a/easevoice_trainer_amd/hip/lib.py b/easevoice_trainer_amd/hip/lib.py
--- a/easevoice_trainer_amd/hip/lib.py
+++ b/easevoice_trainer_amd/hip/lib.py
@@ -73,7 +73,12 @@
 
 class Seg(C.Structure):
     _fields_ = [("a", C.c_void_p), ("b", C.c_void_p), ("da", C.c_void_p), ("n", C.c_int64),
-                ("scale", C.c_float), ("pad_", C.c_int32)]
+                ("scale", C.c_float), ("accum", C.c_int32)]
+
+
+class BwdPost(C.Structure):
+    _fields_ = [("act_y", C.c_void_p), ("fm_real", C.c_void_p), ("fm_dloss", C.c_void_p), ("fm_scale", C.c_float),
+                ("act_slope", C.c_float), ("gate", C.c_int32), ("pad_", C.c_int32)]
 
 
 class KlParams(C.Structure):
@@ -183,6 +188,7 @@
             raise EvtError(f"{path} serves half code {_lib.evt_half_dtype()}: not the {_half} build")
         _libs[_half] = _lib
         _lib.evt_conv1d_lout.restype = C.c_int32
+        _lib.evt_conv1d_bwd_data_post_ok.restype = C.c_int32
         _lib.evt_mel_workspace_floats.restype = C.c_int64
         _lib.evt_workspace_bytes.restype = C.c_int64
         _lib.evt_last_kernel_tag.restype = C.c_char_p
diff --git a/easevoice_trainer_amd/module/models.py b/easevoice_trainer_amd/module/models.py
--- a/easevoice_trainer_amd/module/models.py
+++ b/easevoice_trainer_amd/module/models.py
@@ -617,9 +617,11 @@
         xs = self._prepared(y.reshape(n, -1), y_hat.reshape(n, -1))
         if not y.is_cuda:
             return [d.forward_prepared(x)[0] for d, x in zip(self.discriminators, xs)]
+        from ..hip import conv as HC
         from ..hip.disc import _On, _branches
 
         bank = self.discriminators[0].convs[0]._slot.bank if self.discriminators[0].convs[0]._slot is not None else None
+        chain = HC.DISC_FUSED_BWD and HC.TRACE is None and bank is not None
         lanes, sides = _branches(y.device, len(self.discriminators)) if (bank is not None and bank.defer_n > 0) \
             else ([None] * len(self.discriminators), [])
         main = torch.cuda.current_stream(y.device) if sides else None
@@ -628,7 +630,10 @@
         outs = []
         for d, x, lane in zip(self.discriminators, xs, lanes):
             with _On(lane):
-                o = d.forward_prepared(x)[0]
+                if chain:
+                    o = HC.DiscChainFn.apply(x, bank.anchor, *d.plan()).view(x.size(0) // getattr(d, "period", 1), -1)
+                else:
+                    o = d.forward_prepared(x)[0]
             if lane is not None:
                 x.record_stream(lane)
                 o.record_stream(main)
diff --git a/include/evt.h b/include/evt.h
--- a/include/evt.h
+++ b/include/evt.h
@@ -84,6 +84,19 @@
 int evt_conv1d_bwd_data(const evt_conv1d_params* p, const void* dy, const void* y, const void* w_reg,
                         const void* w_alt, const void* x, const void* dx_add, void* dx, void* stream);
 
+typedef struct evt_bwd_post {
+  const void* act_y;
+  const void* fm_real;
+  const float* fm_dloss;
+  float fm_scale;
+  float act_slope;
+  int32_t gate;
+  int32_t pad_;
+} evt_bwd_post;
+int evt_conv1d_bwd_data_post(const evt_conv1d_params* p, const void* dy, const void* y, const void* w_reg,
+                             const void* w_alt, const void* dx_add, const evt_bwd_post* post, void* dx, void* stream);
+int32_t evt_conv1d_bwd_data_post_ok(const evt_conv1d_params* p);
+
 int evt_conv1d_bwd_weight(const evt_conv1d_params* p, const void* x, const void* dy, const void* y,
                           float* dw, float* dbias, void* stream);
 
@@ -181,7 +194,7 @@
 int evt_spec_to_mel(const float* spec, const float* basis, const int64_t* starts, float* out, int32_t B, int32_t F,
                     int32_t T, int32_t M, int32_t nfr, void* stream);
 
-typedef struct evt_seg { const void* a; const void* b; void* da; int64_t n; float scale; int32_t pad_; } evt_seg;
+typedef struct evt_seg { const void* a; const void* b; void* da; int64_t n; float scale; int32_t accum; } evt_seg;
 int evt_l1_multi_fwd(int32_t dtype, const evt_seg* segs, int32_t nseg, float* out, void* stream);
 int evt_l1_multi_bwd(int32_t dtype, const evt_seg* segs, int32_t nseg, const float* dloss, void* stream);
 int evt_lsgan_multi_fwd(int32_t dtype, const evt_seg* segs, int32_t nseg, float target, float* out, void* stream);
```

New measurement: 3492 audio-s/s, median of 6. About the same (+0.3%).
